# cerbos/cerbos

Measured on NVIDIA H100. Metric: checkresources_decisions_per_sec, higher is better.
Workload: dtype u64

## Files before the change

### cerbos_b200/csrc/cb_core.h

```cpp
#pragma once
#include <stdint.h>
#if !defined(__CUDACC_RTC__)
#include <math.h>
#endif

#include "cerbos_b200_format.h"

#if defined(__CUDACC__)
#define CB_HD __host__ __device__ __forceinline__
#define CB_HD_NOINLINE __host__ __device__ __noinline__
#else
#define CB_HD inline
#define CB_HD_NOINLINE
#endif

namespace cb {

struct alignas(16) U4 { uint32_t x, y, z, w; };

struct TableLayout {
    uint32_t off[32];
    uint32_t nV, nRP, nS, nP, nR, nAP, nT, n_slots, n_rows;
    uint32_t has_role_policies, has_parent_roles, has_principal_policies;
    uint32_t image_bytes;
    uint32_t uc_conds_off, uc_rows_off, uc_chain_off, n_uconds;
    uint32_t uc_n_rows;
    uint32_t uc_slots_off;
    uint32_t uc_deny_rows, uc_allow_rows;
    uint32_t theap_words;
    uint32_t uses_runtime;
};

struct TableView {
    const uint8_t *base;
    const TableLayout *L;
    template <typename T>
    CB_HD const T *sec(int id) const { return reinterpret_cast<const T *>(base + L->off[id]); }
    CB_HD const uint32_t *scope_parent() const { return sec<uint32_t>(CB_SEC_SCOPE_PARENT); }
    CB_HD const uint32_t *scope_flags() const { return sec<uint32_t>(CB_SEC_SCOPE_FLAGS); }
    CB_HD const uint32_t *res_block_map() const { return sec<uint32_t>(CB_SEC_RES_BLOCK_MAP); }
    CB_HD const uint8_t *res_exists() const { return sec<uint8_t>(CB_SEC_RES_EXISTS); }
    CB_HD const uint32_t *prin_block_map() const { return sec<uint32_t>(CB_SEC_PRIN_BLOCK_MAP); }
    CB_HD const uint8_t *prin_exists() const { return sec<uint8_t>(CB_SEC_PRIN_EXISTS); }
    CB_HD const uint32_t *prin_of_string() const { return sec<uint32_t>(CB_SEC_PRIN_OF_STRING); }
    CB_HD const cb_block *blocks() const { return sec<cb_block>(CB_SEC_BLOCKS); }
    CB_HD const cb_row *rows() const { return sec<cb_row>(CB_SEC_ROWS); }
    CB_HD const cb_cond *conds() const { return sec<cb_cond>(CB_SEC_CONDS); }
    CB_HD const cb_instr *code() const { return sec<cb_instr>(CB_SEC_CODE); }
    CB_HD const cb_const *consts() const { return sec<cb_const>(CB_SEC_CONSTS); }
    CB_HD const uint64_t *consts_v64() const { return sec<uint64_t>(CB_SEC_CONSTS_V64); }
    CB_HD const uint64_t *theap() const { return sec<uint64_t>(CB_SEC_THEAP); }
    CB_HD const uint32_t *str_off() const { return sec<uint32_t>(CB_SEC_STR_OFF); }
    CB_HD const uint8_t *str_bytes() const { return sec<uint8_t>(CB_SEC_STR_BYTES); }
    CB_HD const uint32_t *par_off() const { return sec<uint32_t>(CB_SEC_ROLE_PARENTS_OFF); }
    CB_HD const uint32_t *par_list() const { return sec<uint32_t>(CB_SEC_ROLE_PARENTS); }
    CB_HD const uint32_t *rp_off() const { return sec<uint32_t>(CB_SEC_ROLEPOL_OFF); }
    CB_HD const cb_rolepol_entry *rp_entries() const { return sec<cb_rolepol_entry>(CB_SEC_ROLEPOL_ENTRIES); }
    CB_HD const cb_rolepol_rule *rp_rules() const { return sec<cb_rolepol_rule>(CB_SEC_ROLEPOL_RULES); }
    CB_HD const uint32_t *rp_apats() const { return sec<uint32_t>(CB_SEC_ROLEPOL_APATS); }
    CB_HD const uint32_t *block_slots_off() const { return sec<uint32_t>(CB_SEC_BLOCK_SLOTS_OFF); }
    CB_HD const uint32_t *block_slots() const { return sec<uint32_t>(CB_SEC_BLOCK_SLOTS); }
    CB_HD const uint32_t *dr_off() const { return sec<uint32_t>(CB_SEC_DR_OFF); }
    CB_HD const uint32_t *dr_entries() const { return sec<uint32_t>(CB_SEC_DR_ENTRIES); }
    CB_HD const uint32_t *dr_parents() const { return sec<uint32_t>(CB_SEC_DR_PARENTS); }
    CB_HD const uint32_t *dr_name_str() const { return sec<uint32_t>(CB_SEC_DR_NAME_STR); }
    CB_HD const cb_cond *uconds() const { return reinterpret_cast<const cb_cond *>(base + L->uc_conds_off); }
    CB_HD const U4 *urows() const { return reinterpret_cast<const U4 *>(base + L->uc_rows_off); }
    CB_HD const uint32_t *uc_slots() const { return reinterpret_cast<const uint32_t *>(base + L->uc_slots_off); }
    CB_HD const U4 *uc_chain() const { return reinterpret_cast<const U4 *>(base + L->uc_chain_off); }
};

enum { CB_MAX_GATHER = 8 };
struct BatchView {
    const cb_hdr0 *hdr0;
    const cb_hdr1 *hdr1;
    const uint32_t *roles;
    const uint64_t *slots;
    const uint64_t *heap;
    const uint32_t *bstr_off;
    const uint8_t *bstr_bytes;
    const uint32_t *class_off, *class_pats, *aset_k;
    const uint64_t *aset_spread;
    const uint64_t *row_am;
    uint32_t n_rows;
    uint64_t stride;
    uint64_t first, count;
    uint32_t role_cols, n_asets, kc, n_pass, max_actions, kbytes, flags;
    uint32_t rcp, stride_pattern;
    int64_t now;
    const uint32_t *perm;
    uint32_t prefetch_slots;
    uint32_t *defer_list, *defer_count;
    uint32_t *count_dev;
    uint32_t *tile_counter;
    uint8_t *outs[CB_MAX_GATHER];
    uint32_t n_out;
    uint32_t *sig_flags[CB_MAX_GATHER];
    const uint32_t *wait_flags;
    uint32_t sig_rank, sig_step, wait_step;
    const uint32_t *strpred;
    const U4 *uc_rows_pk;
    uint32_t n_bstr;
    uint64_t heap_words;
};

#ifndef __CUDACC_RTC__
inline void finish_batch_view(BatchView &b) {
    b.perm = nullptr;
    b.prefetch_slots = 0;
    b.defer_list = nullptr; b.defer_count = nullptr; b.count_dev = nullptr; b.tile_counter = nullptr;
    b.n_out = 0;
    for (int i = 0; i < CB_MAX_GATHER; i++) { b.outs[i] = nullptr; b.sig_flags[i] = nullptr; }
    b.wait_flags = nullptr; b.sig_rank = 0; b.sig_step = 0; b.wait_step = 0;
    b.strpred = nullptr;
    b.uc_rows_pk = nullptr;
    b.rcp = 1;
    while (b.rcp < b.role_cols) b.rcp <<= 1;
    b.stride_pattern = 0;
    for (uint32_t j = 0; j * b.role_cols < 32; j++) b.stride_pattern |= 1u << (j * b.role_cols);
}
#endif

template <typename T>
CB_HD T ldg(const T *p) { return *p; }

CB_HD uint64_t ldcol64(const uint64_t *p) {
#if defined(__CUDA_ARCH__)
    uint64_t v;
    asm("ld.global.nc.L1::no_allocate.u64 %0, [%1];" : "=l"(v) : "l"(p));
    return v;
#else
    return *p;
#endif
}
CB_HD uint32_t ldcol32(const uint32_t *p) {
#if defined(__CUDA_ARCH__)
    uint32_t v;
    asm("ld.global.nc.L1::no_allocate.u32 %0, [%1];" : "=r"(v) : "l"(p));
    return v;
#else
    return *p;
#endif
}

CB_HD U4 ld16(const void *p) { return *reinterpret_cast<const U4 *>(p); }
CB_HD U4 ldcol128(const void *p) {
#if defined(__CUDA_ARCH__)
    U4 r;
    asm("ld.global.nc.L1::no_allocate.v4.u32 {%0, %1, %2, %3}, [%4];" : "=r"(r.x), "=r"(r.y), "=r"(r.z), "=r"(r.w) : "l"(p));
    return r;
#else
    return *reinterpret_cast<const U4 *>(p);
#endif
}
CB_HD cb_hdr0 load_hdr0(const cb_hdr0 *p) { U4 v = ldcol128(p); cb_hdr0 h; h.principal_id = v.x; h.kind_class = v.y; h.resource_scope = v.z; h.principal_scope = v.w; return h; }
CB_HD cb_hdr1 load_hdr1(const cb_hdr1 *p) {
    uint64_t v = ldcol64(reinterpret_cast<const uint64_t *>(p));
    cb_hdr1 h; h.resource_version = (uint16_t)(v & 0xFFFF); h.principal_version = (uint16_t)((v >> 16) & 0xFFFF); h.action_set_id = (uint32_t)(v >> 32); return h;
}
CB_HD cb_block load_block(const cb_block *p) { U4 v = ld16(p); cb_block b; b.row_start = v.x; b.n_rows = v.y; b.cond_base = v.z; b.n_conds = v.w; return b; }
CB_HD cb_row load_row(const cb_row *p) {
    U4 v = ld16(p);
    cb_row r; r.role = (uint16_t)(v.x & 0xFFFF); r.cond = (uint16_t)(v.x >> 16); r.drcond = (uint16_t)(v.y & 0xFFFF); r.respat = (uint16_t)(v.y >> 16);
    r.effect = (uint8_t)(v.z & 0xFF); r.flags = (uint8_t)((v.z >> 8) & 0xFF); r.n_pats = (uint16_t)(v.z >> 16); r.pat_start = v.w; return r;
}
CB_HD cb_rolepol_entry load_rp_entry(const cb_rolepol_entry *p) { U4 v = ld16(p); cb_rolepol_entry e; e.role = v.x; e.rule_start = v.y; e.n_rules = v.z; e.pad = v.w; return e; }
CB_HD cb_rolepol_rule load_rp_rule(const cb_rolepol_rule *p) { U4 v = ld16(p); cb_rolepol_rule e; e.respat = v.x; e.cond = v.y; e.apat_start = v.z; e.n_apats = v.w; return e; }

CB_HD double u2d(uint64_t u) {
#if defined(__CUDA_ARCH__)
    return __longlong_as_double((long long)u);
#else
    double d; __builtin_memcpy(&d, &u, 8); return d;
#endif
}
CB_HD uint64_t d2u(double d) {
#if defined(__CUDA_ARCH__)
    return (uint64_t)__double_as_longlong(d);
#else
    uint64_t u; __builtin_memcpy(&u, &d, 8); return u;
#endif
}

#if !defined(CB_LEAN_ONLY) || defined(CB_SPEC_PROGRAMS)
struct Val {
    uint32_t tag;
    uint64_t u;
};
static constexpr uint64_t kHeapBatch = 1ull << 63;
static constexpr uint64_t kHeapScratch = 1ull << 62;
static constexpr uint64_t kStrDyn = 1ull << 47;
static constexpr uint64_t kV64ScratchBit = 1ull << 46;
enum { CB_SCRATCH_WORDS = 192, CB_T_SKIP = 15 };

CB_HD Val mk(uint32_t tag, uint64_t u) { Val v; v.tag = tag; v.u = u; return v; }
CB_HD Val mk_err() { return mk(CB_T_ERR, 0); }
CB_HD Val mk_bool(bool b) { return mk(CB_T_BOOL, b ? 1u : 0u); }
CB_HD Val mk_int(int64_t i) { return mk(CB_T_INT, (uint64_t)i); }
CB_HD Val mk_double(double d) { return mk(CB_T_DOUBLE, d != d ? (uint64_t)CB_V64_CANON_NAN : d2u(d)); }

enum { SLOT_VALUE = 0, SLOT_ABSENT = 1, SLOT_ERROR = 2 };

CB_HD Val decode_v64(uint64_t bits, int *state) {
    const uint32_t top = (uint32_t)(bits >> 48);
    const bool boxed = (top & 0xFFF0u) == 0xFFF0u && (top & 0xFu) != 0;
    const uint32_t vt = top & 0xFu;
    const uint64_t pay = bits & 0xFFFFFFFFFFFFull;
    const uint64_t kTagOf = (uint64_t)CB_T_NULL << 4 | (uint64_t)CB_T_BOOL << 8 | (uint64_t)CB_T_STRING << 12 | (uint64_t)CB_T_LIST << 16 |
                            (uint64_t)CB_T_MAP << 20 | (uint64_t)CB_T_INT << 32;
    const uint32_t tag = boxed ? (uint32_t)(kTagOf >> (4 * vt)) & 0xFu : (uint32_t)CB_T_DOUBLE;
    uint64_t off = pay & (CB_V64_HEAP_BATCH_BIT - 1);
    off = (pay & CB_V64_HEAP_BATCH_BIT) ? off | kHeapBatch : (off & kV64ScratchBit) ? (off & ~kV64ScratchBit) | kHeapScratch : off;
    const uint64_t u = !boxed                                  ? bits
                       : vt == CB_V64_BOOL                     ? (uint64_t)(pay != 0)
                       : vt == CB_V64_STRING                   ? pay
                       : (vt == CB_V64_LIST || vt == CB_V64_MAP) ? off
                       : vt == CB_V64_INT                      ? (uint64_t)((int64_t)(pay << 16) >> 16)
                                                               : 0ull;
    *state = !boxed || tag != CB_T_ERR ? SLOT_VALUE : vt == CB_V64_ABSENT ? SLOT_ABSENT : SLOT_ERROR;
    return mk(tag, u);
}
CB_HD Val decode_elem(uint64_t bits) { int s; return decode_v64(bits, &s); }

struct Ctx {
    const TableView *t;
    const BatchView *b;
    uint64_t req;
    uint32_t pid;
    uint32_t unsupported;
    Val vars[CB_MAX_VARS];
    uint64_t edr;
    uint32_t scr_used;
    uint64_t scratch[CB_SCRATCH_WORDS];
};

CB_HD const uint64_t *heap_ptr(const Ctx &c, uint64_t ref) {
    return (ref & kHeapBatch) ? c.b->heap + (ref & ~kHeapBatch) : (ref & kHeapScratch) ? c.scratch + (ref & 0xFFFFu) : c.t->theap() + ref;
}
CB_HD void str_get(const Ctx &c, uint64_t id, const uint8_t *&p, uint32_t &len) {
    if (id & kStrDyn) {
        p = reinterpret_cast<const uint8_t *>(c.scratch) + ((id >> 16) & 0xFFFFu);
        len = (uint32_t)(id & 0xFFFFu);
    } else if (id < c.t->L->nT) {
        uint32_t o = ldg(c.t->str_off() + id);
        p = c.t->str_bytes() + o;
        len = ldg(c.t->str_off() + id + 1) - o;
    } else {
        uint64_t j = id - c.t->L->nT;
        uint32_t o = ldg(c.b->bstr_off + j);
        p = c.b->bstr_bytes + o;
        len = ldg(c.b->bstr_off + j + 1) - o;
    }
}

CB_HD bool is_num(const Val &v) { return v.tag == CB_T_INT || v.tag == CB_T_UINT || v.tag == CB_T_DOUBLE; }

CB_HD int num_cmp(const Val &a, const Val &b) {
    if (a.tag == CB_T_DOUBLE || b.tag == CB_T_DOUBLE) {
        if (a.tag == CB_T_DOUBLE && b.tag == CB_T_DOUBLE) {
            double x = u2d(a.u), y = u2d(b.u);
            if (x != x || y != y) return 2;
            return x < y ? -1 : (x > y ? 1 : 0);
        }
        int sign = 1;
        Val dv = a, iv = b;
        if (a.tag != CB_T_DOUBLE) { dv = b; iv = a; sign = -1; }
        double d = u2d(dv.u);
        if (d != d) return 2;
        int r;
        if (iv.tag == CB_T_UINT) {
            if (d < 0) r = -1;
            else if (d > 18446744073709551615.0) r = 1;
            else { double y = (double)iv.u; r = d < y ? -1 : (d > y ? 1 : 0); }
        } else {
            if (d < -9223372036854775808.0) r = -1;
            else if (d > 9223372036854775807.0) r = 1;
            else { double y = (double)(int64_t)iv.u; r = d < y ? -1 : (d > y ? 1 : 0); }
        }
        return r * sign;
    }
    if (a.tag == b.tag) {
        if (a.tag == CB_T_INT) { int64_t x = (int64_t)a.u, y = (int64_t)b.u; return x < y ? -1 : (x > y ? 1 : 0); }
        return a.u < b.u ? -1 : (a.u > b.u ? 1 : 0);
    }
    if (a.tag == CB_T_INT) {
        int64_t x = (int64_t)a.u;
        if (x < 0) return -1;
        return (uint64_t)x < b.u ? -1 : ((uint64_t)x > b.u ? 1 : 0);
    }
    int64_t y = (int64_t)b.u;
    if (y < 0) return 1;
    return a.u < (uint64_t)y ? -1 : (a.u > (uint64_t)y ? 1 : 0);
}

CB_HD bool str_equal(const Ctx &c, uint64_t a, uint64_t b) {
    if (a == b) return true;
    if (!((a | b) & kStrDyn)) return false;
    const uint8_t *pa, *pb;
    uint32_t la, lb;
    str_get(c, a, pa, la);
    str_get(c, b, pb, lb);
    if (la != lb) return false;
    for (uint32_t i = 0; i < la; i++)
        if (ldg(pa + i) != ldg(pb + i)) return false;
    return true;
}
CB_HD bool scalar_equal(const Ctx &c, const Val &a, const Val &b) {
    if (is_num(a) && is_num(b)) return num_cmp(a, b) == 0;
    if (a.tag != b.tag) return false;
    if (a.tag == CB_T_NULL) return true;
    if (a.tag == CB_T_STRING || a.tag == CB_T_BYTES) return str_equal(c, a.u, b.u);
    return a.u == b.u;
}
CB_HD bool is_container(const Val &v) { return v.tag == CB_T_LIST || v.tag == CB_T_MAP; }

CB_HD bool map_find(const Ctx &c, const Val &m, const Val &key, Val *out) {
    if (is_container(key) || key.tag == CB_T_ERR) return false;
    const uint64_t *p = heap_ptr(c, m.u);
    uint64_t n = ldg(p);
    for (uint64_t i = 0; i < n; i++) {
        Val k = decode_elem(ldg(p + 1 + i));
        if (scalar_equal(c, k, key)) {
            if (out) *out = decode_elem(ldg(p + 1 + n + i));
            return true;
        }
    }
    return false;
}

template <int DEPTH>
struct Eq {
    static CB_HD bool eq(Ctx &c, const Val &a, const Val &b) {
        if (!is_container(a) || !is_container(b)) {
            if (is_container(a) != is_container(b)) return false;
            return scalar_equal(c, a, b);
        }
        if (a.tag != b.tag) return false;
        const uint64_t *pa = heap_ptr(c, a.u), *pb = heap_ptr(c, b.u);
        uint64_t n = ldg(pa);
        if (n != ldg(pb)) return false;
        if (a.tag == CB_T_LIST) {
            for (uint64_t i = 0; i < n; i++)
                if (!Eq<DEPTH - 1>::eq(c, decode_elem(ldg(pa + 1 + i)), decode_elem(ldg(pb + 1 + i)))) return false;
            return true;
        }
        for (uint64_t i = 0; i < n; i++) {
            Val ov;
            if (!map_find(c, b, decode_elem(ldg(pa + 1 + i)), &ov)) return false;
            if (!Eq<DEPTH - 1>::eq(c, decode_elem(ldg(pa + 1 + n + i)), ov)) return false;
        }
        return true;
    }
};
template <>
struct Eq<0> {
    static CB_HD bool eq(Ctx &c, const Val &a, const Val &b) {
        if (is_container(a) && is_container(b)) { c.unsupported = 1; return false; }
        if (is_container(a) != is_container(b)) return false;
        return scalar_equal(c, a, b);
    }
};
CB_HD_NOINLINE bool container_equal(Ctx &c, const Val &a, const Val &b) { return Eq<3>::eq(c, a, b); }
CB_HD bool val_equal(Ctx &c, const Val &a, const Val &b) {
    if (!is_container(a) || !is_container(b)) { if (is_container(a) != is_container(b)) return false; return scalar_equal(c, a, b); }
    return container_equal(c, a, b);
}

CB_HD int str_cmp(const Ctx &c, uint64_t ia, uint64_t ib) {
    const uint8_t *pa, *pb;
    uint32_t la, lb;
    str_get(c, ia, pa, la);
    str_get(c, ib, pb, lb);
    uint32_t m = la < lb ? la : lb;
    for (uint32_t i = 0; i < m; i++) {
        uint8_t x = ldg(pa + i), y = ldg(pb + i);
        if (x != y) return x < y ? -1 : 1;
    }
    return la < lb ? -1 : (la > lb ? 1 : 0);
}

CB_HD int val_order(const Ctx &c, const Val &a, const Val &b) {
    if (is_num(a) && is_num(b)) { int r = num_cmp(a, b); return r == 2 ? 3 : r; }
    if (a.tag != b.tag) return 3;
    switch (a.tag) {
    case CB_T_BOOL: return a.u < b.u ? -1 : (a.u > b.u ? 1 : 0);
    case CB_T_STRING: return a.u == b.u ? 0 : str_cmp(c, a.u, b.u);
    case CB_T_TS:
    case CB_T_DUR: { int64_t x = (int64_t)a.u, y = (int64_t)b.u; return x < y ? -1 : (x > y ? 1 : 0); }
    default: return 3;
    }
}

CB_HD_NOINLINE int spiffe_equal(Ctx &c, const Val &a, const Val &b);
CB_HD Val do_cmp(Ctx &c, int ci, const Val &a, const Val &b) {
    if (a.tag == CB_T_ERR || b.tag == CB_T_ERR) return mk_err();
    if (ci <= 1 && (a.tag == CB_T_SPIFFE_ID || a.tag == CB_T_SPIFFE_TD)) {
        const int r = spiffe_equal(c, a, b);
        return r == 2 ? mk_err() : mk_bool((r == 1) == (ci == 0));
    }
    if (ci == 0) return mk_bool(val_equal(c, a, b));
    if (ci == 1) return mk_bool(!val_equal(c, a, b));
    int r = val_order(c, a, b);
    if (r == 3) return mk_err();
    switch (ci) {
    case 2: return mk_bool(r < 0);
    case 3: return mk_bool(r <= 0);
    case 4: return mk_bool(r > 0);
    default: return mk_bool(r >= 0);
    }
}

CB_HD Val do_in(Ctx &c, const Val &x, const Val &cont) {
    if (x.tag == CB_T_ERR || cont.tag == CB_T_ERR) return mk_err();
    if (cont.tag == CB_T_LIST) {
        const uint64_t *p = heap_ptr(c, cont.u);
        uint64_t n = ldg(p);
// ... 2906 lines not shown
        uint32_t k = 0;
        for (uint32_t i = 0; i < s.len; i++) k += (ldg(s.p + i) & 0xC0) != 0x80;
        return d2u((double)k);
    }
    return (uint64_t)(CB_V64_BOX_BASE | CB_V64_ERROR) << 48;
}
template <typename Cols>
CB_HD uint64_t term_operand(const TableView t, const BatchView &b, const Cols &cols, uint32_t pid, uint32_t kind, uint32_t v, uint32_t aux) {
    if (kind == CB_OPK_CONST) return ldg(t.consts_v64() + v);
    if (kind == CB_OPK_PID) return ((uint64_t)(CB_V64_BOX_BASE | CB_V64_STRING) << 48) | pid;
    uint64_t x = cols.slot(v);
    if (kind == CB_OPK_SLOT) return x;
    return kind == CB_OPK_SLOT_ELEM ? elem_operand(t, b, x, aux) : size_operand(t, b, x);
}
CB_HD bool v64_bad(uint64_t x) { return ((uint32_t)(x >> 48) & 0xFFFEu) == (CB_V64_BOX_BASE | CB_V64_ABSENT); }
CB_HD int eq_tri(uint64_t x, uint64_t y, bool &slow) {
    const uint32_t tx = v64_tag(x), ty = v64_tag(y);
    if (v64_bad(x) || v64_bad(y)) return TRI_E;
    if (tx == 0 && ty == 0) return u2d(x) == u2d(y);
    if (tx <= CB_V64_STRING && ty <= CB_V64_STRING) return x == y;
    slow = true;
    return TRI_E;
}
CB_HD int ord_tri(uint32_t ci, uint64_t x, uint64_t y, bool &slow) {
    const uint32_t tx = v64_tag(x), ty = v64_tag(y);
    if (v64_bad(x) || v64_bad(y)) return TRI_E;
    if (tx == 0 && ty == 0) {
        const double dx = u2d(x), dy = u2d(y);
        if (dx != dx || dy != dy) return TRI_E;
        return ci == 2 ? dx < dy : ci == 3 ? dx <= dy : ci == 4 ? dx > dy : dx >= dy;
    }
    if (tx != ty) return TRI_E;
    slow = true;
    return TRI_E;
}
CB_HD int in_tri(const TableView t, const BatchView &b, uint64_t x, uint64_t y, bool elems_scalar, bool &slow) {
    if (v64_bad(x) || v64_bad(y)) return TRI_E;
    if (v64_tag(y) != CB_V64_LIST || v64_tag(x) > CB_V64_STRING) { slow = true; return TRI_E; }
    const uint64_t *p = list_ptr(t, b, y);
    const uint32_t ln = (uint32_t)ldg(p);
    bool found = false;
    for (uint32_t j = 0; j < ln; j++) {
        const uint64_t e = ldg(p + 1 + j);
        if (!elems_scalar) slow |= v64_tag(e) > CB_V64_STRING;
        found |= scalar_eq64(x, e);
    }
    return found;
}
template <typename... E>
CB_HD int in_const_tri(uint64_t x, bool &slow, E... elems) {
    if (v64_bad(x)) return TRI_E;
    if (v64_tag(x) > CB_V64_STRING) { slow = true; return TRI_E; }
    bool found = false;
    ((found |= scalar_eq64(x, (uint64_t)elems)), ...);
    return found ? TRI_T : TRI_F;
}
CB_HD int has_tri(uint64_t x) {
    const uint32_t tx = v64_tag(x);
    return tx == CB_V64_ERROR ? TRI_E : (tx != CB_V64_ABSENT);
}
CB_HD int cmp_tri(uint32_t ci, uint64_t x, uint64_t y, bool &slow) {
    const uint32_t tx = v64_tag(x), ty = v64_tag(y);
    if (v64_bad(x) || v64_bad(y)) return TRI_E;
    if (tx == 0 && ty == 0) {
        const double dx = u2d(x), dy = u2d(y);
        if (ci == 0) return dx == dy;
        if (dx != dx || dy != dy) return TRI_E;
        return ci == 2 ? dx < dy : ci == 3 ? dx <= dy : ci == 4 ? dx > dy : dx >= dy;
    }
    if (ci == 0 && tx <= CB_V64_STRING && ty <= CB_V64_STRING) return x == y;
    if (ci != 0 && tx != ty) return TRI_E;
    slow = true;
    return TRI_E;
}
CB_HD int str_tri(const TableView t, const BatchView &b, uint32_t op, uint64_t x, uint64_t y) {
    if (v64_tag(x) != CB_V64_STRING || v64_tag(y) != CB_V64_STRING) return TRI_E;
    const StrRef a = str_ref(t, b, x), c = str_ref(t, b, y);
    if (c.len > a.len) return TRI_F;
    if (op == CB_TERM_CONTAINS) {
        bool hit = false;
        for (uint32_t o = 0; o + c.len <= a.len; o++) {
            bool eq = true;
            for (uint32_t j = 0; j < c.len; j++) eq &= ldg(a.p + o + j) == ldg(c.p + j);
            hit |= eq;
        }
        return hit;
    }
    const uint8_t *ap = op == CB_TERM_STARTS ? a.p : a.p + (a.len - c.len);
    bool eq = true;
    for (uint32_t j = 0; j < c.len; j++) eq &= ldg(ap + j) == ldg(c.p + j);
    return eq;
}
template <typename Cols>
CB_HD int term_tri(const TableView t, const BatchView &b, const Cols &cols, uint32_t pid, const U4 w, bool &slow) {
    const uint32_t op = w.x & 0xFF, flags = (w.x >> 8) & 0xFF, xk = (w.x >> 16) & 0xFF, yk = w.x >> 24;
    int tri = TRI_E;
    switch (w.x & 0xFF) {
    case CB_TERM_EQ_SS: tri = eq_tri(cols.slot(w.y), cols.slot(w.z), slow); break;
    case CB_TERM_EQ_SC: tri = eq_tri(cols.slot(w.y), ldg(t.consts_v64() + w.z), slow); break;
    case CB_TERM_EQ_SP: tri = eq_tri(cols.slot(w.y), ((uint64_t)(CB_V64_BOX_BASE | CB_V64_STRING) << 48) | pid, slow); break;
    case CB_TERM_ORD_SS: tri = ord_tri(flags & CB_TERM_CI_MASK, cols.slot(w.y), cols.slot(w.z), slow); break;
    case CB_TERM_ORD_SC: tri = ord_tri(flags & CB_TERM_CI_MASK, cols.slot(w.y), ldg(t.consts_v64() + w.z), slow); break;
    case CB_TERM_IN_SC: tri = in_tri(t, b, cols.slot(w.y), ldg(t.consts_v64() + w.z), true, slow); break;
    case CB_TERM_IN_CS: tri = in_tri(t, b, ldg(t.consts_v64() + w.y), cols.slot(w.z), false, slow); break;
    case CB_TERM_IN_SS: tri = in_tri(t, b, cols.slot(w.y), cols.slot(w.z), false, slow); break;
    default: {
        const uint64_t x = term_operand(t, b, cols, pid, xk, w.y, w.w & 0xFFFF);
        const uint64_t y = op == CB_TERM_HAS ? 0 : term_operand(t, b, cols, pid, yk, w.z, w.w >> 16);
        const uint32_t tx = v64_tag(x), ty = v64_tag(y);
        if (op == CB_TERM_HAS) {
            tri = has_tri(x);
        } else if (op == CB_TERM_CMP) {
            tri = cmp_tri(flags & CB_TERM_CI_MASK, x, y, slow);
        } else if (v64_bad(x) || v64_bad(y)) {
            tri = TRI_E;
        } else if (op == CB_TERM_IN) {
            if (ty != CB_V64_LIST || tx > CB_V64_STRING) slow = true;
            else {
                const uint64_t *p = list_ptr(t, b, y);
                const uint32_t ln = (uint32_t)ldg(p);
                bool found = false;
                for (uint32_t j = 0; j < ln; j++) {
                    const uint64_t e = ldg(p + 1 + j);
                    slow |= v64_tag(e) > CB_V64_STRING;
                    found |= scalar_eq64(x, e);
                }
                tri = found;
            }
        } else if (op == CB_TERM_STARTS || op == CB_TERM_ENDS || op == CB_TERM_CONTAINS) {
            tri = str_tri(t, b, op, x, y);
        } else {
            if (tx != CB_V64_LIST || ty != CB_V64_LIST) tri = TRI_E;
            else {
                const uint64_t *pa = list_ptr(t, b, x), *pb = list_ptr(t, b, y);
                const uint32_t na = (uint32_t)ldg(pa), nb = (uint32_t)ldg(pb);
                bool any_hit = false, all_hit = true;
                for (uint32_t i2 = 0; i2 < na; i2++) {
                    const uint64_t ea = ldg(pa + 1 + i2);
                    slow |= v64_tag(ea) > CB_V64_STRING;
                    bool hit = false;
                    for (uint32_t j = 0; j < nb; j++) {
                        const uint64_t eb = ldg(pb + 1 + j);
                        slow |= v64_tag(eb) > CB_V64_STRING;
                        hit |= scalar_eq64(ea, eb);
                    }
                    any_hit |= hit;
                    all_hit &= hit;
                }
                tri = op == CB_TERM_INTERSECTS ? any_hit : all_hit;
            }
        }
    }
    }
    return tri;
}
template <typename Cols>
CB_HD int uc_term_tri(const TableView t, const BatchView &b, const Cols &cols, uint32_t pid, const U4 w, bool &slow) {
#ifdef CB_UC_STUB_TERMS
    return (int)(cols.slot(w.y) & 1u);
#endif
    return term_tri(t, b, cols, pid, w, slow);
}
template <typename Cols>
CB_HD uint64_t uc_term_operand(const TableView t, const BatchView &b, const Cols &cols, uint32_t pid, uint32_t kind, uint32_t v, uint32_t aux) {
#ifdef CB_UC_STUB_TERMS
    return ((uint64_t)(CB_V64_BOX_BASE | CB_V64_STRING) << 48) | (uint32_t)cols.slot(v);
#endif
    return term_operand(t, b, cols, pid, kind, v, aux);
}
enum { CB_LC = 8 };
CB_HD uint32_t list_bound(uint32_t own) {
#if defined(__CUDA_ARCH__)
    return __reduce_max_sync(__activemask(), own);
#else
    return own;
#endif
}
#ifndef CB_LIST_KEYS64
struct ListRegs {
    uint32_t st, len;
    uint32_t bound;
    uint32_t e[CB_LC];
};
static constexpr uint32_t kListPad = 0xFFFFFFFEu;
static constexpr uint32_t kListNoKey = 0xFFFFFFFFu;
static constexpr uint32_t kStringTop = CB_V64_BOX_BASE | CB_V64_STRING;
CB_HD uint32_t list_key(uint64_t w) { return (uint32_t)w; }
CB_HD bool list_elem_odd(uint64_t w) { return (uint32_t)(w >> 48) != kStringTop; }
static constexpr uint64_t kListBeyondHeap = 0ull;
#else
struct ListRegs {
    uint32_t st, len;
    uint32_t bound;
    uint64_t e[CB_LC];
};
static constexpr uint64_t kListPad = 0xFFFE000000000001ull;
CB_HD uint64_t norm_scalar(uint64_t v) { return v == 0x8000000000000000ull ? 0ull : v; }
CB_HD uint64_t list_key(uint64_t w) { return norm_scalar(w); }
CB_HD bool list_elem_odd(uint64_t w) { return v64_tag(w) > CB_V64_STRING || w == CB_V64_CANON_NAN; }
static constexpr uint64_t kListBeyondHeap = kListPad;
#endif
CB_HD ListRegs list_load(const TableView t, const BatchView &b, uint64_t x) {
    ListRegs L;
    L.st = v64_bad(x) ? 1u : v64_tag(x) == CB_V64_LIST ? 0u : 3u;
    L.len = 0;
#ifdef CB_UC_STUB_LISTS
    L.len = (uint32_t)x & 7u;
    L.bound = CB_LC;
    for (int j = 0; j < CB_LC; j++) L.e[j] = (uint32_t)x + j;
    return L;
#endif
    const uint64_t *p = nullptr;
    uint64_t room = 0;
    if (L.st == 0) {
        const uint64_t pay = x & 0xFFFFFFFFFFFFull;
        const bool in_batch = (pay & CB_V64_HEAP_BATCH_BIT) != 0;
        const uint64_t off = in_batch ? pay & (CB_V64_HEAP_BATCH_BIT - 1) : pay;
        p = (in_batch ? b.heap : t.theap()) + off;
        room = (in_batch ? b.heap_words : (uint64_t)t.L->theap_words) - off;
        L.len = (uint32_t)ldg(p);
    }
    L.bound = list_bound(L.len < CB_LC ? L.len : CB_LC);
    const uint32_t lim = room > (uint64_t)L.bound ? L.bound : room != 0 ? (uint32_t)room - 1u : 0u;
    bool odd = L.len > CB_LC;
#if defined(__CUDA_ARCH__)
#pragma unroll
#endif
    for (int j = 0; j < CB_LC; j++) {
        const uint64_t w = (uint32_t)j < lim ? ldg(p + 1 + j) : kListBeyondHeap;
        const bool in = (uint32_t)j < L.len;
        odd |= in && list_elem_odd(w);
        L.e[j] = in ? list_key(w) : kListPad;
    }
    if (L.st == 0) L.st = odd ? 2u : 0u;
    return L;
}
CB_HD uint64_t list_size(const TableView t, const BatchView &b, uint64_t x, const ListRegs &L) {
    if (L.st == 0 || L.st == 2) return d2u((double)L.len);
    return size_operand(t, b, x);
}
CB_HD uint64_t list_elem(const TableView t, const BatchView &b, uint64_t x, const ListRegs &L, uint32_t i) {
    if (L.st == 2) return elem_operand(t, b, x, i);
    if (L.st != 0 || i >= L.len) return (uint64_t)(CB_V64_BOX_BASE | CB_V64_ERROR) << 48;
#ifndef CB_LIST_KEYS64
    return ((uint64_t)kStringTop << 48) | L.e[i];
#else
    return L.e[i];
#endif
}
#ifndef CB_LIST_KEYS64
typedef uint32_t ListKey;
CB_HD ListKey list_probe_key(uint64_t x) { return (uint32_t)(x >> 48) == kStringTop ? (uint32_t)x : kListNoKey; }
#else
typedef uint64_t ListKey;
CB_HD ListKey list_probe_key(uint64_t x) { return norm_scalar(x); }
#endif
template <int P>
CB_HD uint32_t list_probe(const ListRegs &L, const ListKey (&k)[P]) {
    static_assert(P >= 1 && P <= 32, "one bit per key");
#if defined(CB_UC_STUB_LISTS) || defined(CB_UC_STUB_LIST_PROBES)
    return ((uint32_t)(L.e[0] ^ k[0]) ^ L.len) & (uint32_t)((1ull << P) - 1u);
#endif
    uint32_t h = 0;
#if defined(__CUDA_ARCH__)
#pragma unroll
#endif
    for (int p = 0; p < P; p++) {
        bool hit = false;
#if defined(__CUDA_ARCH__)
#pragma unroll
#endif
        for (int j = 0; j < CB_LC; j++) hit |= k[p] == L.e[j];
        h |= (uint32_t)hit << p;
    }
    return h;
}
CB_HD int list_in_tri(uint64_t x, uint32_t st, uint32_t hit, bool &slow) {
#ifdef CB_UC_STUB_LISTS
    return hit ? TRI_T : TRI_F;
#endif
    if (v64_bad(x) || st == 1) return TRI_E;
    if (st != 0 || v64_tag(x) > CB_V64_STRING || x == CB_V64_CANON_NAN) { slow = true; return TRI_E; }
    return hit ? TRI_T : TRI_F;
}
CB_HD int list_in_tri(uint64_t x, const ListRegs &L, bool &slow) {
#ifdef CB_UC_STUB_LISTS
    return (uint32_t)x == L.e[0] ? TRI_T : TRI_F;
#endif
    const ListKey k[1] = {list_probe_key(x)};
    return list_in_tri(x, L.st, list_probe(L, k), slow);
}
CB_HD uint32_t list_mask(const ListRegs &A, const ListRegs &B) {
    return list_probe(B, A.e) & (A.len < CB_LC ? (1u << A.len) - 1u : (1u << CB_LC) - 1u);
}
CB_HD int list_set_tri(bool subset, const ListRegs &A, const ListRegs &B, uint32_t m, bool &slow) {
#ifdef CB_UC_STUB_LISTS
    return (A.e[0] == B.e[subset] + m) ? TRI_T : TRI_F;
#endif
    if (A.st == 1 || B.st == 1) return TRI_E;
    if (A.st == 3 || B.st == 3) return TRI_E;
    if (A.st == 2 || B.st == 2) { slow = true; return TRI_E; }
    return (subset ? m == (1u << A.len) - 1u : m != 0u) ? TRI_T : TRI_F;
}
CB_HD int strpred_tri(const BatchView &b, uint64_t x, uint32_t p) {
#ifdef CB_UC_STUB_STRPRED
    return (int)((x >> p) & 1u);
#endif
    if (v64_bad(x)) return TRI_E;
    if (v64_tag(x) != CB_V64_STRING) return TRI_E;
    return (int)((ldg(b.strpred + (uint32_t)(x & 0xFFFFFFFFu)) >> p) & 1u);
}
CB_HD bool typed_str(uint64_t x) { return (uint32_t)(x >> 32) == (uint32_t)(CB_V64_BOX_BASE | CB_V64_STRING) << 16; }
CB_HD bool typed_num(uint64_t x) { const double d = u2d(x); return v64_tag(x) == 0 && d == d; }
CB_HD bool typed_bool(uint64_t x) { return (x >> 1) == (uint64_t)(CB_V64_BOX_BASE | CB_V64_BOOL) << 47; }
CB_HD bool typed_list(const ListRegs &L, uint32_t need) {
    bool ok = L.st == 0 && L.len >= need;
#ifdef CB_LIST_KEYS64
    for (int j = 0; j < CB_LC; j++) ok &= (uint32_t)j >= L.len || (uint32_t)(L.e[j] >> 48) == (CB_V64_BOX_BASE | CB_V64_STRING);
#endif
    return ok;
}
CB_HD bool uc_typed(bool guard) {
#ifdef CB_UC_STUB_FALLBACK
    return guard || true;
#endif
    return guard;
}
CB_HD uint32_t typed_id(uint64_t key) { return (uint32_t)key; }
CB_HD uint64_t typed_box(uint32_t id) { return ((uint64_t)(CB_V64_BOX_BASE | CB_V64_STRING) << 48) | id; }
CB_HD bool typed_ord(uint32_t ci, double dx, double dy) { return ci == 2 ? dx < dy : ci == 3 ? dx <= dy : ci == 4 ? dx > dy : dx >= dy; }
CB_HD bool typed_strpred(const BatchView &b, uint32_t id, uint32_t p) {
#ifdef CB_UC_STUB_STRPRED
    return ((id >> p) & 1u) != 0;
#endif
    return ((ldg(b.strpred + id) >> p) & 1u) != 0;
}
template <typename Cols>
CB_HD ListKey list_elem_key(const TableView t, const BatchView &b, const Cols &cols, uint32_t v, const ListRegs &L, uint32_t i) {
    if (L.st == 2) return list_probe_key(elem_operand(t, b, cols.slot(v), i));
    return list_probe_key(list_elem(t, b, 0ull, L, i));
}

struct OneCols {
    uint64_t x;
    CB_HD uint64_t slot(uint32_t) const { return x; }
};
CB_HD bool term_lit(int tri, uint32_t flags) { return (flags & CB_TERM_LIT_F) ? tri == TRI_F : tri == TRI_T; }
template <typename Cols>
CB_HD uint32_t flat_dnf_inline(const TableView t, const BatchView &b, const Cols &cols, uint32_t pid, uint32_t flat_off, uint32_t info) {
    const uint32_t nt = info & 0xFFFF;
    const cb_instr *terms = t.code() + flat_off;
    bool any = false, group = true, slow = false;
    for (uint32_t i = 0; i < nt; i++) {
        const U4 w = ld16(terms + 2 * i);
        const uint32_t flags = (w.x >> 8) & 0xFF;
        group &= term_lit(term_tri(t, b, cols, pid, w, slow), flags);
        if (flags & CB_TERM_GROUP_END) { any |= group; group = true; }
    }
    if (slow) return 4u;
    return (uint32_t)(any != (bool)((info >> 24) & 1));
}
template <typename Cols>
CB_HD uint32_t cond_eval(const TableView t, const BatchView &b, const Cols &cols, uint32_t pid, uint32_t gid) {
    U4 cd = ld16(t.conds() + gid);
    if (cd.w) return flat_dnf_inline(t, b, cols, pid, cd.z, cd.w);
    return 4u;
}

CB_HD uint32_t chain_start(const TableView t, uint32_t scope, uint32_t kind_flag, bool lenient) {
    if (scope == CB_SCOPE_NONE) return CB_NONE32;
    uint32_t s = scope & ~CB_SCOPE_INEXACT_BIT;
    if (s >= t.L->nS) return CB_NONE32;
    if (!(ldg(t.scope_flags() + s) & kind_flag)) {
        if (!lenient) return CB_NONE32;
        do { s = ldg(t.scope_parent() + s); } while (s != CB_NONE32 && !(ldg(t.scope_flags() + s) & kind_flag));
    }
    return s;
}
CB_HD uint32_t chain_next(const TableView t, uint32_t s, uint32_t kind_flag) {
    do { s = ldg(t.scope_parent() + s); } while (s != CB_NONE32 && !(ldg(t.scope_flags() + s) & kind_flag));
    return s;
}

CB_HD void prefetch_l1(const void *p) {
#if defined(__CUDA_ARCH__)
    asm volatile("prefetch.global.L1 [%0];" ::"l"(p));
#else
    (void)p;
#endif
}

CB_HD void prefetch_request(const BatchView &b, uint64_t n) {
    prefetch_l1(b.hdr0 + n);
    prefetch_l1(b.hdr1 + n);
    const uint32_t *pr = b.roles + n;
    for (uint32_t i = 0; i < b.role_cols; i++, pr += b.stride) prefetch_l1(pr);
    const uint64_t *ps = b.slots + n;
    for (uint32_t q = 0; q < b.prefetch_slots; q++, ps += b.stride) prefetch_l1(ps);
}

#ifndef CB_LEAN_ONLY
CB_HD uint32_t kind_count(const BatchView &b, uint32_t kc) {
    if (kc == CB_KIND_NONE) return 0;
    if (!(kc & CB_KIND_CLASS_CSR_BIT)) return 1;
    uint32_t c = kc & ~CB_KIND_CLASS_CSR_BIT;
    return ldg(b.class_off + c + 1) - ldg(b.class_off + c);
}
CB_HD uint32_t kind_pat_at(const BatchView &b, uint32_t kc, uint32_t j) {
    if (!(kc & CB_KIND_CLASS_CSR_BIT)) return kc;
    return ldg(b.class_pats + ldg(b.class_off + (kc & ~CB_KIND_CLASS_CSR_BIT)) + j);
}
CB_HD bool kind_has(const BatchView &b, uint32_t kc, uint32_t pat) {
    if (!(kc & CB_KIND_CLASS_CSR_BIT)) return kc == pat;
    for (uint32_t j = 0, n = kind_count(b, kc); j < n; j++)
        if (kind_pat_at(b, kc, j) == pat) return true;
    return false;
}

template <typename M>
CB_HD_NOINLINE M role_cols_slow(const uint8_t *base, const TableLayout *L, const BatchView *b, uint64_t n, uint32_t n_roles, uint32_t rscope, uint32_t role) {
    TableView t; t.base = base; t.L = L;
    M m = 0;
    for (uint32_t i = 0; i < n_roles; i++) m |= (M)role_in_pr(t, role, ldcol32(b->roles + (uint64_t)i * b->stride + n), rscope) << i;
    return m;
}
struct U2x64 { uint64_t a, b; };
CB_HD_NOINLINE U2x64 role_tab_parents(const uint8_t *base, const TableLayout *L, const BatchView *b, uint64_t n, uint32_t n_roles, uint32_t rscope, uint32_t RCP,
                                     uint64_t rp0, uint64_t rp1) {
    TableView t; t.base = base; t.L = L;
    for (uint32_t i = 0; i < n_roles; i++) {
        uint32_t r = ldcol32(b->roles + (uint64_t)i * b->stride + n);
        if (r >= t.L->nR) continue;
        uint64_t idx = (uint64_t)rscope * t.L->nR + r;
        for (uint32_t j = ldg(t.par_off() + idx), e = ldg(t.par_off() + idx + 1); j < e; j++) {
            uint32_t pq = ldg(t.par_list() + j) * RCP + i;
            if (pq < 64) rp0 |= 1ull << pq; else if (pq < 128) rp1 |= 1ull << (pq - 64);
        }
    }
    U2x64 r; r.a = rp0; r.b = rp1; return r;
}

#endif
CB_HD uint32_t row_role(const U4 &r) { return r.x & 0xFFFF; }
CB_HD uint32_t row_cond(const U4 &r) { return r.x >> 16; }
CB_HD uint32_t row_drcond(const U4 &r) { return r.y & 0xFFFF; }
CB_HD uint32_t row_respat(const U4 &r) { return r.y >> 16; }
CB_HD uint32_t row_effect(const U4 &r) { return r.z & 0xFF; }
#ifndef CB_LEAN_ONLY

CB_HD_NOINLINE bool exists_check(const uint8_t *base, const TableLayout *L, const BatchView *b, uint32_t kc, uint32_t pscope, uint32_t r0,
                                 uint32_t pv, uint32_t rv, bool lenient) {
    TableView t; t.base = base; t.L = L;
    bool p_exists = false, r_exists = false;
    if (pv != CB_NONE16)
        for (uint32_t s = chain_start(t, pscope, CB_SCOPE_FLAG_PRINCIPAL, lenient); s != CB_NONE32; s = chain_next(t, s, CB_SCOPE_FLAG_PRINCIPAL))
            p_exists |= ldg(t.prin_exists() + (uint64_t)pv * t.L->nS + s) != 0;
    for (uint32_t s = r0; s != CB_NONE32; s = chain_next(t, s, CB_SCOPE_FLAG_RESOURCE))
        for (uint32_t j = 0, nk = kind_count(*b, kc); j < nk; j++)
            r_exists |= (ldg(t.res_exists() + ((uint64_t)rv * t.L->nRP + kind_pat_at(*b, kc, j)) * t.L->nS + s) & CB_EXISTS_RESOURCE_KIND) != 0;
    return p_exists || r_exists;
}

CB_HD void prefetch_block_slots(const TableView t, const BatchView &b, uint32_t bid, uint64_t n) {
    for (uint32_t q = ldg(t.block_slots_off() + bid), e = ldg(t.block_slots_off() + bid + 1); q < e; q++)
        prefetch_l1(b.slots + (uint64_t)ldg(t.block_slots() + q) * b.stride + n);
}

CB_HD_NOINLINE uint64_t compute_edr(const uint8_t *base, const TableLayout *L, const BatchView *b, uint64_t n, uint32_t pid, uint32_t bid, uint32_t n_roles,
                                    uint32_t rscope, uint32_t *unsupported) {
    TableView t; t.base = base; t.L = L;
    uint64_t mask = 0;
    for (uint32_t e = ldg(t.dr_off() + bid), ee = ldg(t.dr_off() + bid + 1); e < ee; e++) {
        const U4 en = ld16(t.dr_entries() + 4 * (uint64_t)e);
        bool hit = false;
        for (uint32_t q = 0; q < en.w && !hit; q++) {
            const uint32_t pr = ldg(t.dr_parents() + en.z + q);
            if (pr == CB_ROLE_ANY) { hit = true; break; }
            for (uint32_t i = 0; i < n_roles && !hit; i++) hit = role_in_pr(t, pr, ldcol32(b->roles + (uint64_t)i * b->stride + n), rscope);
        }
        if (!hit) continue;
        bool sat = true;
        if (en.y) { const uint32_t r = cond_sat(base, L, b, n, pid, en.y - 1); *unsupported |= r & 2; sat = r & 1; }
        if (sat) mask |= 1ull << (en.x & 63);
    }
    return mask;
}

template <typename M>
struct PairMasks { M deny, allow; uint32_t unsupported; };

template <typename M>
CB_HD_NOINLINE PairMasks<M> principal_walk(const uint8_t *base, const TableLayout *L, const BatchView *b, uint64_t n, uint32_t pid, uint32_t kc, uint32_t pidx,
                                           uint32_t p0, uint32_t rv, M amask, const uint64_t *row_am) {
    TableView t; t.base = base; t.L = L;
    PairMasks<M> out; out.deny = 0; out.allow = 0; out.unsupported = 0;
    M alive = amask;
    for (uint32_t s = p0; s != CB_NONE32 && alive; s = chain_next(t, s, CB_SCOPE_FLAG_PRINCIPAL)) {
        uint32_t bid = ldg(t.prin_block_map() + ((uint64_t)rv * t.L->nP + pidx) * t.L->nS + s);
        if (bid == CB_NONE32) continue;
        U4 bl = ld16(t.blocks() + bid);
        M D = 0, A = 0;
        for (uint32_t ri = bl.x, re = bl.x + bl.y; ri < re; ri++) {
            M m = (M)ldg(reinterpret_cast<const M *>(row_am + ri)) & alive;
            if (!m) continue;
            U4 row = ld16(t.rows() + ri);
            if (!kind_has(*b, kc, row_respat(row))) continue;
            if (row_effect(row) == CB_EFFECT_DENY ? (m & ~D) == 0 : (m & ~A) == 0) continue;
            bool sat = true;
            if (row_drcond(row)) { uint32_t r = cond_sat(t.base, t.L, b, n, pid, bl.z + row_drcond(row) - 1); out.unsupported |= r & 2; sat = r & 1; }
            if (sat && row_cond(row)) { uint32_t r = cond_sat(t.base, t.L, b, n, pid, bl.z + row_cond(row) - 1); out.unsupported |= r & 2; sat = r & 1; }
            if (!sat) continue;
            if (row_effect(row) == CB_EFFECT_DENY) D |= m; else A |= m;
        }
        out.deny |= D;
        alive &= ~D;
        uint32_t perm = (ldg(t.scope_flags() + s) >> CB_SCOPE_PERM_SHIFT) & 3;
        if (perm == 1) { M a = A & alive; out.allow |= a; alive &= ~a; }
    }
    return out;
}

template <typename M>
CB_HD_NOINLINE PairMasks<M> rolepol_denies(const uint8_t *base, const TableLayout *L, const BatchView *b, uint64_t n, uint32_t pid, uint32_t kc, uint32_t n_roles,
                                           uint32_t rscope, uint32_t RCP, uint64_t rp0, uint64_t rp1, bool packed, uint32_t rv, uint32_t s,
                                           uint32_t ps, uint32_t aset, M amask, M alive, M D) {
    TableView t; t.base = base; t.L = L;
    PairMasks<M> out; out.allow = 0; out.unsupported = 0;
    const M role_all = (M)(((M)1 << n_roles) - 1);
    const uint32_t nAP = t.L->nAP ? t.L->nAP : 1;
    const uint64_t *spread = b->aset_spread + ((uint64_t)ps * b->n_asets + aset) * nAP;
    uint64_t ro = (uint64_t)rv * t.L->nS + s;
    for (uint32_t e = ldg(t.rp_off() + ro), ee = ldg(t.rp_off() + ro + 1); e < ee; e++) {
        U4 en = ld16(t.rp_entries() + e);
        M rmask;
        if (packed) { uint32_t pos = en.x * RCP; rmask = (M)(pos < 64 ? rp0 >> pos : rp1 >> (pos - 64)) & role_all; }
        else rmask = role_cols_slow<M>(t.base, t.L, b, n, n_roles, rscope, en.x);
        if (!rmask) continue;
        M matched = 0;
        for (uint32_t q = 0; q < en.z; q++) {
            U4 ru = ld16(t.rp_rules() + en.y + q);
            if (!kind_has(*b, kc, ru.x)) continue;
            M am = 0;
            for (uint32_t a = 0; a < ru.w; a++) am |= (M)ldg(spread + ldg(t.rp_apats() + ru.z + a));
            if (!am) continue;
            matched |= am;
            if (ru.y && ((am * rmask) & alive & ~D)) {
                uint32_t r = cond_sat(t.base, t.L, b, n, pid, ru.y - 1);
                out.unsupported |= r & 2;
                if (!(r & 1)) D |= (am * rmask) & alive;
            }
        }
        D |= ((amask & ~matched) * rmask) & alive;
    }
    out.deny = D;
    return out;
}

template <typename M>
CB_HD void eval_request(const TableView t, const BatchView &b, uint64_t n, uint8_t *bitmap, uint8_t *effects, uint32_t *status) {
    constexpr M kOne = 1;
    const U4 h0 = ldcol128(b.hdr0 + n);
    const uint64_t h1 = ldcol64(reinterpret_cast<const uint64_t *>(b.hdr1 + n));
    const uint32_t pid = h0.x, kc = h0.y, rscope = h0.z, pscope = h0.w;
    const uint32_t rv = (uint32_t)(h1 & 0xFFFF), pv = (uint32_t)((h1 >> 16) & 0xFFFF), aset = (uint32_t)(h1 >> 32);
    const uint32_t RC = b.role_cols;
    const uint32_t K = aset < b.n_asets ? ldg(b.aset_k + aset) : 0;
    uint32_t unsupported = 0;

    uint32_t RCP = 1;
    while (RCP < RC) RCP <<= 1;
    const bool packed = (uint64_t)t.L->nR * RCP <= 128;
    uint64_t rp0 = 0, rp1 = 0;
    uint32_t n_roles = 0;
    for (uint32_t i = 0; i < RC; i++) {
        uint32_t rr = ldcol32(b.roles + (uint64_t)i * b.stride + n);
        if (rr != CB_ROLE_PAD) n_roles = i + 1;
        if (rr < t.L->nR) {
            uint32_t pos = rr * RCP + i;
            if (pos < 64) rp0 |= 1ull << pos; else if (pos < 128) rp1 |= 1ull << (pos - 64);
        }
    }

    uint64_t acc = 0;
    const bool wide = b.kbytes > 8;
    uint8_t *out = effects ? nullptr : bitmap + n * b.kbytes;
    uint8_t *eff = effects ? effects + n * (uint64_t)b.max_actions : nullptr;
    if (wide) {
        if (eff) for (uint32_t q = 0; q < b.max_actions; q++) eff[q] = (uint8_t)(q < K ? CB_EFFECT_DENY : 0);
        else for (uint32_t q = 0; q < b.kbytes; q++) out[q] = 0;
    }

    const bool lenient = (b.flags & CB_BATCH_FLAG_LENIENT) != 0;
    uint32_t p0 = CB_NONE32, r0 = CB_NONE32;
    bool live = n_roles != 0 && K != 0 && rv != CB_NONE16;
    if (live) {
        if (t.L->has_principal_policies) p0 = chain_start(t, pscope, CB_SCOPE_FLAG_PRINCIPAL, lenient);
        r0 = chain_start(t, rscope, CB_SCOPE_FLAG_RESOURCE, lenient);
        if (pv != rv && !exists_check(t.base, t.L, &b, kc, pscope, r0, pv, rv, lenient)) live = false;
        if (p0 == CB_NONE32 && r0 == CB_NONE32) live = false;
    }

    if (live) {
        const uint32_t pidx = (t.L->has_principal_policies && pid < t.L->nT) ? ldg(t.prin_of_string() + pid) : CB_NONE32;
        const M role_all = (M)((kOne << n_roles) - 1);
        if (t.L->has_parent_roles && packed && rscope != CB_SCOPE_NONE && !(rscope & CB_SCOPE_INEXACT_BIT) && rscope < t.L->nS) {
            U2x64 r = role_tab_parents(t.base, t.L, &b, n, n_roles, rscope, RCP, rp0, rp1);
            rp0 = r.a; rp1 = r.b;
        }
        const uint32_t nk = kind_count(b, kc);

        for (uint32_t ps = 0; ps < b.n_pass; ps++) {
            const uint32_t kbase = ps * b.kc;
            if (kbase >= K) break;
            const uint32_t kn = K - kbase < b.kc ? K - kbase : b.kc;
            const uint64_t *row_am = b.row_am + ((uint64_t)ps * b.n_asets + aset) * b.n_rows;
            M amask = 0;
            for (uint32_t kk = 0; kk < kn; kk++) amask |= kOne << (kk * RC);

            M p_allow = 0, p_deny = 0;
            if (pidx != CB_NONE32 && p0 != CB_NONE32) {
                PairMasks<M> pm = principal_walk<M>(t.base, t.L, &b, n, pid, kc, pidx, p0, rv, amask, row_am);
                p_allow = pm.allow; p_deny = pm.deny; unsupported |= pm.unsupported;
            }

            const M undecided = amask & ~(p_allow | p_deny);
            M r_allow_pairs = 0;
            if (undecided && r0 != CB_NONE32) {
                M alive = undecided * role_all;
                for (uint32_t s = r0; s != CB_NONE32 && alive; s = chain_next(t, s, CB_SCOPE_FLAG_RESOURCE)) {
                    M D = 0, A = 0;
                    bool any_row = false;
                    for (uint32_t j = 0; j < nk; j++) {
                        uint64_t mi = ((uint64_t)rv * t.L->nRP + kind_pat_at(b, kc, j)) * t.L->nS + s;
                        if (t.L->has_role_policies) any_row |= (ldg(t.res_exists() + mi) & CB_EXISTS_ANY_ROW) != 0;
                        uint32_t bid = ldg(t.res_block_map() + mi);
                        if (bid == CB_NONE32) continue;
                        prefetch_block_slots(t, b, bid, n);
                        const U4 bl = ld16(t.blocks() + bid);
// ... 691 lines not shown
```

### cerbos_b200/csrc/cb_specialize.h

```cpp
#pragma once
#include <stdint.h>

#include <cstdio>
#include <cstring>
#include <map>
#include <string>
#include <vector>

#include "cerbos_b200_format.h"

namespace cbspec {

struct Limits {
    uint32_t max_shapes = 8;
    uint32_t max_items = 96;
};

inline std::string hex(uint32_t v) {
    char buf[16];
    snprintf(buf, sizeof buf, "0x%xu", v);
    return buf;
}
inline std::string hex64(uint64_t v) {
    char buf[32];
// ... 76 lines not shown
        const uint32_t bid = shape_blocks[sh][0];
        const uint32_t *bl = blocks + 4 * bid;
        s += "template <typename Cols>\nCB_HD void spec_shape_" + std::to_string(sh) + "(" + args_decl + ") {\n";
        if (bs_off[bid + 1] > bs_off[bid]) {
            s += "    if (!cols.staged()) {";
            for (uint32_t q = bs_off[bid]; q < bs_off[bid + 1]; q++) s += " cols.prefetch_slot(" + std::to_string(bs[q]) + "u);";
            s += " }\n";
        }
        s += "    bool slow = false;\n    uint32_t val = 1u;\n";
        for (uint32_t c = 0; c < bl[3]; c++) {
            const uint32_t *cd = conds + 4 * (bl[2] + c);
            const uint32_t nt = cd[3] & 0xFFFFu, negate = (cd[3] >> 24) & 1u;
            s += "    {   // condition " + std::to_string(c + 1) + "\n        bool any = false, group = true;\n";
            for (uint32_t i = 0; i < nt; i++) {
                const uint32_t *w = code + 2 * (cd[2] + 2 * i);
                const uint32_t flags = (w[0] >> 8) & 0xFFu;
                s += "        group &= term_lit(" + term_expr(w, consts, theap) + ", " + hex(flags) + ");\n";
                if (flags & CB_TERM_GROUP_END) s += "        any |= group; group = true;\n";
            }
            s += std::string("        val |= (uint32_t)(any != ") + (negate ? "true" : "false") + ") << " + std::to_string(c + 1) + ";\n    }\n";
        }
        s += "    defer |= slow;\n";
        for (uint32_t r = 0; r < bl[1]; r++) {
            const uint32_t *row = rows + 4 * (bl[0] + r);
            s += "    row_apply(ldg(reinterpret_cast<const uint32_t *>(ram + " + std::to_string(r) + ")), U4{" + hex(row[0]) + ", " + hex(row[1] & 0xFFFFu) + ", " +
                 hex(row[2] & 0xFFu) + ", 0u}, rp, RCP, role_all, alive, val, D, A);\n";
        }
        s += "}\n";
    }
    s += "struct SpecBlocks {\n    template <typename Cols>\n    CB_HD void operator()(const TableView t, const BatchView &b, const Cols &cols, uint32_t pid, uint32_t bid, "
         "uint64_t rp, uint32_t RCP, uint32_t role_all, uint32_t alive, const uint64_t *row_am, uint32_t &D, uint32_t &A, bool &defer) const {\n";
    s += "        const uint64_t *ram = row_am + ldg(reinterpret_cast<const uint32_t *>(t.blocks() + bid));   // + row_start\n";
    s += "        switch (bid) {\n";
    for (uint32_t sh = 0; sh < shape_blocks.size(); sh++) {
        s += "       ";
        for (uint32_t bid : shape_blocks[sh]) s += " case " + std::to_string(bid) + ":";
        s += "\n            spec_shape_" + std::to_string(sh) + "(t, b, cols, pid, rp, RCP, role_all, alive, ram, D, A, defer);\n            break;\n";
    }
    s += "        default: defer = true; break;\n        }\n    }\n};\n}  // namespace cb\n";
    return s;
}

struct Ins { uint32_t op, ia, ib, ic; };
struct Atoms {
    std::map<std::vector<uint32_t>, uint32_t> ids;
    std::vector<std::string> src;
    std::vector<bool> slot_used;
    std::vector<uint32_t> only_slot;
    std::vector<bool> reads_pid;
};

inline bool is_jump(uint32_t op) {
    return op == CB_OP_JF_KEEP || op == CB_OP_JT_KEEP || op == CB_OP_JMP || op == CB_OP_TERN || op == CB_OP_LOOP_INIT || op == CB_OP_LOOP_NEXT || op == CB_OP_LOOP_PRED;
}

inline std::string atom_source(const std::vector<Ins> &P, uint32_t lo, uint32_t hi, const uint32_t *consts , uint32_t n_consts, uint32_t n_slots,
                               std::vector<bool> &slot_used, uint32_t *only_slot = nullptr, bool *reads_pid = nullptr) {
    std::vector<uint32_t> my_slots;
    bool my_pid = false;
    const uint32_t n = hi - lo;
    const int kUnset = -1000;
    std::vector<int> depth(n + 1, kUnset), ldep(n + 1, kUnset);
    std::vector<bool> target(n + 1, false);
    bool bad = false;
    auto set = [&](uint32_t k, int d, int l) {
        if (k > n) { bad = true; return; }
        if (depth[k] == kUnset) { depth[k] = d; ldep[k] = l; }
        else if (depth[k] != d || ldep[k] != l) bad = true;
    };
    auto rel = [&](uint32_t abs) -> uint32_t { if (abs < lo || abs > hi) { bad = true; return 0; } return abs - lo; };
    set(0, 0, 0);
    for (uint32_t k = 0; k < n && !bad; k++) {
        if (depth[k] == kUnset) { bad = true; break; }
        const Ins &I = P[lo + k];
        const int d = depth[k], l = ldep[k];
        int nd = d;
        bool falls = true;
        switch (I.op) {
        case CB_OP_CONST: case CB_OP_SLOT: case CB_OP_HAS_SLOT: case CB_OP_PID: case CB_OP_NOW: case CB_OP_VAR:
        case CB_OP_CMP_SLOT_CONST: case CB_OP_CMP_SLOT_SLOT: case CB_OP_CMP_SLOT_PID: case CB_OP_IN_SLOT_CONST: case CB_OP_IN_CONST_SLOT:
            nd = d + 1; break;
        case CB_OP_SELECT: case CB_OP_HAS: case CB_OP_NEG: case CB_OP_NOT: case CB_OP_SIZE: case CB_OP_NOERR: case CB_OP_INT: case CB_OP_UINT:
        case CB_OP_DOUBLE: case CB_OP_TIMESTAMP: case CB_OP_DURATION: case CB_OP_DYN: case CB_OP_IN_IP_RANGE: case CB_OP_HIER_SIZE: case CB_OP_TS_GET:
        case CB_OP_MATCHES:
            if (d < 1) bad = true;
            break;
        case CB_OP_INDEX: case CB_OP_EQ: case CB_OP_NE: case CB_OP_LT: case CB_OP_LE: case CB_OP_GT: case CB_OP_GE:
        case CB_OP_ADD: case CB_OP_SUB: case CB_OP_MUL: case CB_OP_DIV: case CB_OP_MOD: case CB_OP_IN:
        case CB_OP_STARTS_WITH: case CB_OP_ENDS_WITH: case CB_OP_CONTAINS: case CB_OP_AND: case CB_OP_OR:
        case CB_OP_HAS_INTERSECTION: case CB_OP_IS_SUBSET: case CB_OP_HIER_REL: case CB_OP_IN_SPLIT:
            if (d < 2) bad = true;
            nd = d - 1; break;
        case CB_OP_HIER_CA: nd = d - (I.ia == 0 ? 1 : 2); if (nd < 1) bad = true; break;
        case CB_OP_FN:
            if (I.ib < 1 || I.ib > (I.ia == CB_FN_FORMAT ? (uint32_t)CB_MAX_STACK : 4u) || d < (int)I.ib) bad = true;
            nd = d - ((int)I.ib - 1); break;
        case CB_OP_JF_KEEP: case CB_OP_JT_KEEP: if (d < 1) bad = true; set(rel(I.ic), d, l); target[rel(I.ic)] = true; break;
        case CB_OP_JMP: set(rel(I.ic), d, l); target[rel(I.ic)] = true; falls = false; break;
        case CB_OP_TERN:
            if (d < 1) bad = true;
            nd = d - 1;
            set(rel(I.ic), d - 1, l); target[rel(I.ic)] = true;
            set(rel(I.ib), d, l); target[rel(I.ib)] = true;
            break;
        case CB_OP_LOOP_INIT:
            if (d < 1 || (I.ib & 0xFF) >= CB_LOOP_MAP || l >= CB_MAX_LOOP_DEPTH) bad = true;
            set(rel(I.ic), d, l); target[rel(I.ic)] = true;
            set(k + 1, d - 1, l + 1);
            falls = false;
            break;
        case CB_OP_LOOP_NEXT:
            if (d < 1 || (I.ib & 0xFF) >= CB_LOOP_MAP || l < 1) bad = true;
            set(rel(I.ic), d - 1, l); target[rel(I.ic)] = true;
            set(k + 1, d, l - 1);
            falls = false;
            break;
        default: bad = true; break;
        }
        if (nd > CB_MAX_STACK) bad = true;
        if (falls && !bad) set(k + 1, nd, l);
    }
    if (bad || depth[n] != 1 || ldep[n] != 0) return "";
    auto S = [](int i) { return "s" + std::to_string(i); };
    auto lab = [](uint32_t k) { return "P" + std::to_string(k); };
    auto cst = [&](uint32_t k) -> std::string {
        if (k >= n_consts) { bad = true; return "mk_err()"; }
        const uint32_t *w = consts + 4 * k;
        return "mk(" + hex(w[0]) + ", " + hex64((uint64_t)w[2] | (uint64_t)w[3] << 32) + ")";
    };
    auto slot = [&](uint32_t v) -> std::string {
        if (v >= n_slots) { bad = true; return "0ull"; }
        slot_used[v] = true;
        bool seen = false;
        for (uint32_t q : my_slots) seen |= q == v;
        if (!seen) my_slots.push_back(v);
        return "cols.slot(" + std::to_string(v) + "u)";
    };
    int maxd = 1;
    for (uint32_t k = 0; k <= n; k++) if (depth[k] > maxd) maxd = depth[k];
    std::string s = "    Val";
    for (int i = 0; i < maxd; i++) s += std::string(i ? ", " : " ") + S(i);
    s += ";\n    Loop L0, L1; int st_; (void)st_; (void)L0; (void)L1;\n";
    for (uint32_t k = 0; k < n; k++) {
        const Ins &I = P[lo + k];
        const int d = depth[k], l = ldep[k];
        if (target[k]) s += lab(k) + ":;\n";
        const std::string a = S(d - 1), a2 = S(d - 2), top = S(d);
        s += "    ";
        switch (I.op) {
        case CB_OP_CONST: s += top + " = " + cst(I.ic) + ";"; break;
        case CB_OP_SLOT: s += top + " = decode_v64(" + slot(I.ic) + ", &st_);"; break;
        case CB_OP_HAS_SLOT: s += "decode_v64(" + slot(I.ic) + ", &st_); " + top + " = op_has_slot(st_);"; break;
        case CB_OP_PID: my_pid = true; s += top + " = mk(CB_T_STRING, c.pid);"; break;
        case CB_OP_NOW: s += top + " = mk(CB_T_TS, (uint64_t)c.b->now);"; break;
        case CB_OP_VAR: if (I.ia >= CB_MAX_VARS) bad = true; s += top + " = c.vars[" + std::to_string(I.ia) + "];"; break;
        case CB_OP_SELECT: s += a + " = op_select(c, " + a + ", " + hex(I.ic) + ");"; break;
        case CB_OP_HAS: s += a + " = op_has(c, " + a + ", " + hex(I.ic) + ");"; break;
        case CB_OP_INDEX: s += a2 + " = do_index(c, " + a2 + ", " + a + ");"; break;
        case CB_OP_EQ: case CB_OP_NE: case CB_OP_LT: case CB_OP_LE: case CB_OP_GT: case CB_OP_GE:
            s += a2 + " = do_cmp(c, " + std::to_string(I.op - CB_OP_EQ) + ", " + a2 + ", " + a + ");"; break;
        case CB_OP_ADD: case CB_OP_SUB: case CB_OP_MUL: case CB_OP_DIV: case CB_OP_MOD:
            s += a2 + " = do_arith(c, " + std::to_string(I.op) + ", " + a2 + ", " + a + ");"; break;
        case CB_OP_NEG: s += a + " = op_neg(" + a + ");"; break;
        case CB_OP_NOT: s += a + " = op_not(" + a + ");"; break;
        case CB_OP_IN: s += a2 + " = do_in(c, " + a2 + ", " + a + ");"; break;
        case CB_OP_SIZE: s += a + " = op_size(c, " + a + ");"; break;
        case CB_OP_STARTS_WITH: case CB_OP_ENDS_WITH: case CB_OP_CONTAINS:
            s += a2 + " = do_str2(c, " + std::to_string(I.op) + ", " + a2 + ", " + a + ");"; break;
        case CB_OP_JF_KEEP: s += "if (" + a + ".tag == CB_T_BOOL && " + a + ".u == 0) goto " + lab(I.ic - lo) + ";"; break;
        case CB_OP_JT_KEEP: s += "if (" + a + ".tag == CB_T_BOOL && " + a + ".u == 1) goto " + lab(I.ic - lo) + ";"; break;
        case CB_OP_AND: s += a2 + " = and_or(false, " + a2 + ", " + a + ");"; break;
        case CB_OP_OR: s += a2 + " = and_or(true, " + a2 + ", " + a + ");"; break;
        case CB_OP_JMP: s += "goto " + lab(I.ic - lo) + ";"; break;
        case CB_OP_TERN:
            s += "if (" + a + ".tag == CB_T_BOOL) { if (!" + a + ".u) goto " + lab(I.ic - lo) + "; } else { " + a + " = mk_err(); goto " + lab(I.ib - lo) + "; }";
            break;
        case CB_OP_HAS_INTERSECTION: s += a2 + " = do_set_pred(c, false, " + a2 + ", " + a + ");"; break;
        case CB_OP_IS_SUBSET: s += a2 + " = do_set_pred(c, true, " + a2 + ", " + a + ");"; break;
        case CB_OP_LOOP_INIT:
            s += "{ const Val r_ = " + a + "; if (!qloop_init(c, L" + std::to_string(l) + ", r_, " + std::to_string(I.ib & 0xFF) + ", " + (((I.ib >> 8) & 1) ? "true" : "false") +
                 ", " + std::to_string(I.ia) + ", &" + a + ")) goto " + lab(I.ic - lo) + "; }";
            break;
        case CB_OP_LOOP_NEXT:
            s += "{ const Val r_ = " + a + "; if (!qloop_next(c, L" + std::to_string(l - 1) + ", r_, " + std::to_string(I.ib & 0xFF) + ", " + (((I.ib >> 8) & 1) ? "true" : "false") +
                 ", " + std::to_string(I.ia) + ", &" + a + ")) goto " + lab(I.ic - lo) + "; }";
            break;
        case CB_OP_NOERR: s += a + " = mk_bool(" + a + ".tag != CB_T_ERR);"; break;
        case CB_OP_INT: s += a + " = conv_int(c, " + a + ");"; break;
        case CB_OP_UINT: s += a + " = conv_uint(c, " + a + ");"; break;
        case CB_OP_DOUBLE: s += a + " = op_double(c, " + a + ");"; break;
        case CB_OP_TIMESTAMP: s += a + " = op_timestamp(c, " + a + ");"; break;
        case CB_OP_DURATION: s += a + " = op_duration(c, " + a + ");"; break;
        case CB_OP_DYN: s += ";"; break;
        case CB_OP_CMP_SLOT_CONST: s += top + " = do_cmp(c, " + std::to_string(I.ia) + ", decode_v64(" + slot(I.ib) + ", &st_), " + cst(I.ic) + ");"; break;
        case CB_OP_CMP_SLOT_SLOT: s += "{ const Val x_ = decode_v64(" + slot(I.ib) + ", &st_); " + top + " = do_cmp(c, " + std::to_string(I.ia) + ", x_, decode_v64(" + slot(I.ic) + ", &st_)); }"; break;
        case CB_OP_CMP_SLOT_PID: my_pid = true; s += top + " = do_cmp(c, " + std::to_string(I.ia) + ", decode_v64(" + slot(I.ib) + ", &st_), mk(CB_T_STRING, c.pid));"; break;
        case CB_OP_IN_SLOT_CONST: s += top + " = do_in(c, decode_v64(" + slot(I.ib) + ", &st_), " + cst(I.ic) + ");"; break;
        case CB_OP_IN_CONST_SLOT: s += top + " = do_in(c, " + cst(I.ic) + ", decode_v64(" + slot(I.ib) + ", &st_));"; break;
        case CB_OP_IN_IP_RANGE: s += a + " = " + a + ".tag == CB_T_ERR ? mk_err() : do_in_ip_range(c, " + a + ", c.t->theap() + " + hex(I.ic) + ");"; break;
        case CB_OP_HIER_REL: s += a2 + " = op_hier_rel(c, " + hex(I.ia) + ", " + hex(I.ib) + ", " + hex(I.ic) + ", " + a2 + ", " + a + ");"; break;
        case CB_OP_TS_GET: s += a + " = op_ts_get(c, " + a + ", " + hex(I.ia) + ", " + hex(I.ib) + ", " + hex(I.ic) + ");"; break;
        case CB_OP_IN_SPLIT: s += a2 + " = op_in_split(c, " + a2 + ", " + a + ", " + hex(I.ib) + ");"; break;
        case CB_OP_HIER_SIZE: s += a + " = op_hier_size(c, " + a + ", " + hex(I.ib) + ");"; break;
        case CB_OP_HIER_CA:
            if (I.ia == 0) s += a2 + " = op_hier_ca2(c, " + a2 + ", " + a + ", " + hex(I.ib) + ", " + hex(I.ic) + ");";
            else s += S(d - 3) + " = op_hier_ca3(c, " + S(d - 3) + ", " + a2 + ", " + a + ", " + hex(I.ib) + ", " + hex(I.ic) + ");";
            break;
        case CB_OP_FN: {
            const int base = d - (int)I.ib;
            s += "{ Val a_[" + std::to_string(I.ib) + "] = {";
            for (uint32_t q = 0; q < I.ib; q++) s += std::string(q ? ", " : "") + S(base + (int)q);
            s += "}; " + S(base) + " = op_fn(c, " + hex(I.ia) + ", " + hex(I.ib) + ", a_); }";
            break;
        }
        case CB_OP_MATCHES: s += a + " = op_matches(c, " + a + ", " + hex(I.ic) + ");"; break;
        default: bad = true; break;
        }
        s += "\n";
    }
    if (target[n]) s += lab(n) + ":;\n";
    s += "    return cond_true(s0);\n";
    if (only_slot) *only_slot = my_slots.size() == 1 ? my_slots[0] : CB_NONE32;
    if (reads_pid) *reads_pid = my_pid;
    return bad ? std::string() : s;
}

inline std::string translate_program(const uint32_t *code_words, uint32_t code_off, uint32_t code_len, const uint32_t *consts, uint32_t n_consts, uint32_t n_slots, Atoms &at) {
    if (code_len == 0 || code_len > 4096) return "";
    std::vector<Ins> P(code_len);
    for (uint32_t i = 0; i < code_len; i++) {
        const uint32_t w0 = code_words[2 * (code_off + i)], w1 = code_words[2 * (code_off + i) + 1];
        P[i] = Ins{w0 & 0xFFu, (w0 >> 8) & 0xFFu, w0 >> 16, w1};
    }
    std::vector<std::string> st;
    uint32_t i = 0;
    bool ret = false;
    while (i < code_len && !ret) {
        const Ins &I = P[i];
        auto cond_level = [&](uint32_t op) { return op == CB_OP_AND || op == CB_OP_OR || op == CB_OP_COND_NOT || op == CB_OP_RET; };
        switch (I.op) {
        case CB_OP_RET: ret = true; continue;
        case CB_OP_AND: case CB_OP_OR: {
            if (st.size() < 2) return "";
            const std::string b = st.back(); st.pop_back();
            st.back() = "(" + st.back() + (I.op == CB_OP_AND ? " & " : " | ") + b + ")";
            i++;
            continue;
        }
        case CB_OP_COND_NOT: if (st.empty()) return ""; st.back() = "!" + st.back(); i++; continue;
        case CB_OP_JF_KEEP: case CB_OP_JT_KEEP:
            if (st.empty() || I.ic <= i || I.ic > code_len) return "";
            i++;
            continue;
        default: break;
        }
        uint32_t e = i;
        while (e < code_len && P[e].op != CB_OP_TO_COND) e++;
        bool literal = false;
        if (I.op == CB_OP_CONST && i + 1 < code_len) {
            const uint32_t nx = P[i + 1].op;
            if (cond_level(nx)) literal = true;
            if ((nx == CB_OP_JF_KEEP || nx == CB_OP_JT_KEEP) && (e >= code_len || P[i + 1].ic > e)) literal = true;
        }
        if (literal) {
            if (I.ic >= n_consts || consts[4 * I.ic] != CB_T_BOOL) return "";
            st.push_back(consts[4 * I.ic + 2] ? "true" : "false");
            i++;
            continue;
        }
        if (e >= code_len) return "";
        std::vector<uint32_t> key;
        for (uint32_t k = i; k < e; k++) {
            const Ins &J = P[k];
            const bool j = is_jump(J.op);
            key.push_back(J.op | J.ia << 8 | (J.op == CB_OP_TERN ? (J.ib - i) : J.ib) << 16);
            key.push_back(j ? J.ic - i : J.ic);
        }
        auto it = at.ids.find(key);
        if (it == at.ids.end()) {
            if (at.slot_used.size() < n_slots) at.slot_used.resize(n_slots, false);
            uint32_t one = CB_NONE32;
            bool pid = false;
            const std::string body = atom_source(P, i, e, consts, n_consts, n_slots, at.slot_used, &one, &pid);
            if (body.empty()) return "";
            const uint32_t id = (uint32_t)at.src.size();
            at.only_slot.push_back(one);
            at.reads_pid.push_back(pid);
            at.src.push_back("template <typename Cols>\nCB_HD bool uc_atom_" + std::to_string(id) + "(Ctx &c, const Cols &cols) {\n" + body + "}\n");
            it = at.ids.emplace(key, id).first;
        }
        st.push_back("a" + std::to_string(it->second));
        i = e + 1;
    }
    if (!ret || st.size() != 1) return "";
    return st[0];
}

struct UcLimits {
    uint32_t max_terms = 512;
};
struct UcSource {
    std::string src;
    uint32_t n_strpred = 0;
    uint32_t n_atoms = 0;
};
inline UcSource generate_uc(const uint8_t *uc_image, const uint32_t *off, uint32_t uc_conds_off, uint32_t n_uconds, uint32_t n_slots, uint32_t n_consts = 0,
                            const UcLimits lim = UcLimits()) {
    UcSource out;
    if (n_uconds == 0 || n_uconds > 127) return out;
    const uint32_t *const_words = reinterpret_cast<const uint32_t *>(uc_image + off[CB_SEC_CONSTS]);
    Atoms atoms;
    std::vector<std::string> formula(n_uconds + 1);
    const uint32_t *uconds = reinterpret_cast<const uint32_t *>(uc_image + uc_conds_off);
    const uint32_t scope_rows = uconds[0], deny_rows = uconds[1], allow_rows = uconds[2];
    const uint32_t *code = reinterpret_cast<const uint32_t *>(uc_image + off[CB_SEC_CODE]);
    const uint64_t *consts = reinterpret_cast<const uint64_t *>(uc_image + off[CB_SEC_CONSTS_V64]);
    const uint64_t *theap = reinterpret_cast<const uint64_t *>(uc_image + off[CB_SEC_THEAP]);
    const uint32_t kUseMask = ~((uint32_t)(CB_TERM_LIT_F | CB_TERM_GROUP_END) << 8);
    std::map<std::vector<uint32_t>, uint32_t> term_ids;
    std::vector<std::vector<uint32_t>> terms;
    const uint32_t ns = n_slots ? n_slots : 1;
    std::vector<bool> slot_used(ns, false), slot_list(ns, false);
    auto is_slot_kind = [](uint32_t kind) { return kind == CB_OPK_SLOT || kind == CB_OPK_SLOT_ELEM || kind == CB_OPK_SLOT_SIZE; };
    auto use_slot = [&](uint32_t kind, uint32_t v) { if (is_slot_kind(kind) && v < ns) slot_used[v] = true; };
    auto v64_tag = [](uint64_t b) { const uint32_t top = (uint32_t)(b >> 48); return (top & 0xFFF0u) == 0xFFF0u ? (top & 0xFu) : 0u; };
    for (uint32_t u = 1; u <= n_uconds; u++) {
        const uint32_t *cd = uconds + 4 * u;
        if (cd[3] == 0 || ((cd[3] >> 16) & 0xFF) != CB_FLAT_DNF) {
            formula[u] = translate_program(code, cd[0], cd[1], const_words, n_consts, ns, atoms);
            if (formula[u].empty()) return out;
            continue;
        }
        for (uint32_t i = 0, nt = cd[3] & 0xFFFFu; i < nt; i++) {
            const uint32_t *w = code + 2 * (cd[2] + 2 * i);
            std::vector<uint32_t> key = {w[0] & kUseMask, w[1], w[2], w[3]};
            if (term_ids.emplace(key, (uint32_t)terms.size()).second) terms.push_back(key);
        }
    }
    if (terms.size() > lim.max_terms) return out;
    std::vector<char> form(terms.size(), 'G');
    std::vector<uint32_t> pred_of(terms.size(), 0);
    std::vector<uint32_t> pred_terms;
    for (uint32_t q = 0; q < terms.size(); q++) {
        const uint32_t *w = terms[q].data();
        const uint32_t op = w[0] & 0xFF, xk = (w[0] >> 16) & 0xFF, yk = w[0] >> 24;
        switch (op) {
        case CB_TERM_EQ_SS: case CB_TERM_ORD_SS: use_slot(CB_OPK_SLOT, w[1]); use_slot(CB_OPK_SLOT, w[2]); break;
        case CB_TERM_EQ_SC: case CB_TERM_EQ_SP: case CB_TERM_ORD_SC: case CB_TERM_IN_SC: use_slot(CB_OPK_SLOT, w[1]); break;
        case CB_TERM_IN_SS: use_slot(CB_OPK_SLOT, w[1]); use_slot(CB_OPK_SLOT, w[2]); if (w[2] < ns) { slot_list[w[2]] = true; form[q] = 'L'; } break;
        case CB_TERM_IN_CS: use_slot(CB_OPK_SLOT, w[2]); if (w[2] < ns) { slot_list[w[2]] = true; form[q] = 'L'; } break;
        default:
            use_slot(xk, w[1]);
            if (op != CB_TERM_HAS) use_slot(yk, w[2]);
            if (xk == CB_OPK_SLOT_SIZE && w[1] < ns) slot_list[w[1]] = true;
            if (op != CB_TERM_HAS && yk == CB_OPK_SLOT_SIZE && w[2] < ns) slot_list[w[2]] = true;
            if (op == CB_TERM_IN && yk == CB_OPK_SLOT && w[2] < ns) { slot_list[w[2]] = true; form[q] = 'L'; }
            if ((op == CB_TERM_INTERSECTS || op == CB_TERM_SUBSET) && xk == CB_OPK_SLOT && yk == CB_OPK_SLOT && w[1] < ns && w[2] < ns) {
                slot_list[w[1]] = slot_list[w[2]] = true;
                form[q] = 'L';
            }
            if ((op == CB_TERM_STARTS || op == CB_TERM_ENDS || op == CB_TERM_CONTAINS) && xk == CB_OPK_SLOT && yk == CB_OPK_CONST &&
                v64_tag(consts[w[2]]) == CB_V64_STRING && pred_terms.size() < 32) {
                form[q] = 'P';
                pred_of[q] = (uint32_t)pred_terms.size();
                pred_terms.push_back(q);
            }
            break;
        }
    }
    std::vector<int> atom_pred(atoms.src.size(), -1);
    uint32_t n_pred_bits = (uint32_t)pred_terms.size();
    for (uint32_t a = 0; a < atoms.src.size(); a++)
        if (atoms.only_slot[a] != CB_NONE32 && !atoms.reads_pid[a] && n_pred_bits + 2 <= 32) { atom_pred[a] = (int)n_pred_bits; n_pred_bits += 2; }
    std::map<std::pair<uint32_t, uint32_t>, bool> masks;
    std::vector<std::pair<uint32_t, uint32_t>> mask_of(terms.size());
    for (int pass = 0; pass < 2; pass++)
        for (uint32_t q = 0; q < terms.size(); q++) {
            const uint32_t *w = terms[q].data();
            const uint32_t op = w[0] & 0xFF;
            if (form[q] != 'L' || (op != CB_TERM_SUBSET && op != CB_TERM_INTERSECTS) || (op == CB_TERM_SUBSET) != (pass == 0)) continue;
            std::pair<uint32_t, uint32_t> k(w[1], w[2]);
            if (op == CB_TERM_INTERSECTS && !masks.count(k) && masks.count({w[2], w[1]})) k = {w[2], w[1]};
            masks[k] = true;
            mask_of[q] = k;
        }
    auto sl = [](uint32_t v) { return "cols.slot(" + std::to_string(v) + "u)"; };
    auto operand = [&](uint32_t kind, uint32_t v, uint32_t aux) -> std::string {
        if (kind == CB_OPK_CONST) return hex64(consts[v]);
        if (kind == CB_OPK_PID) return "(((uint64_t)(CB_V64_BOX_BASE | CB_V64_STRING) << 48) | pid)";
        if (v >= ns) return "";
        if (kind == CB_OPK_SLOT) return sl(v);
        const std::string l = "cols.l" + std::to_string(v);
        if (kind == CB_OPK_SLOT_SIZE && slot_list[v]) return "list_size(t, b, " + sl(v) + ", " + l + ")";
        if (kind == CB_OPK_SLOT_ELEM && slot_list[v] && aux < 8) return "list_elem(t, b, " + sl(v) + ", " + l + ", " + std::to_string(aux) + "u)";
        return "";
    };
    struct Probe {
        uint32_t kind, v, aux;
        std::string value;
    };
    auto probe_operand = [&](uint32_t q) -> Probe {
        const uint32_t *w = terms[q].data();
        const uint32_t op = w[0] & 0xFF, xk = (w[0] >> 16) & 0xFF;
        if (op == CB_TERM_IN_CS) return Probe{CB_OPK_CONST, w[1], 0, hex64(consts[w[1]])};
        if (op == CB_TERM_IN_SS) return Probe{CB_OPK_SLOT, w[1], 0, sl(w[1])};
        const std::string x = operand(xk, w[1], w[3] & 0xFFFFu);
        if (!x.empty()) return Probe{xk, w[1], w[3] & 0xFFFFu, x};
        return Probe{CB_NONE32, 0, 0, "uc_term_operand(t, b, cols, pid, " + hex(xk) + ", " + hex(w[1]) + ", " + hex(w[3] & 0xFFFFu) + ")"};
    };
    std::map<uint32_t, std::vector<Probe>> probes;
    std::vector<uint32_t> probe_of(terms.size(), CB_NONE32);
    for (uint32_t q = 0; q < terms.size(); q++) {
        const uint32_t op = terms[q][0] & 0xFF;
        if (form[q] != 'L' || (op != CB_TERM_IN_CS && op != CB_TERM_IN_SS && op != CB_TERM_IN)) continue;
        std::vector<Probe> &ps = probes[terms[q][2]];
        const Probe x = probe_operand(q);
        uint32_t p = 0;
        while (p < ps.size() && ps[p].value != x.value) p++;
        if (p == ps.size() && p < 32) ps.push_back(x);
        if (p < ps.size()) probe_of[q] = p;
    }
    auto term_code = [&](uint32_t q) -> std::string {
        const uint32_t *w = terms[q].data();
        const uint32_t op = w[0] & 0xFF, flags = (w[0] >> 8) & 0xFF, xk = (w[0] >> 16) & 0xFF, yk = w[0] >> 24;
        const bool kinds = op <= CB_TERM_SUBSET;
        const std::string x = kinds ? operand(xk, w[1], w[3] & 0xFFFFu) : "", y = kinds && op != CB_TERM_HAS ? operand(yk, w[2], w[3] >> 16) : "";
        if (form[q] == 'P') return "strpred_tri(b, " + sl(w[1]) + ", " + std::to_string(pred_of[q]) + "u)";
        if (form[q] == 'L') {
            if (op == CB_TERM_IN_CS || op == CB_TERM_IN_SS || op == CB_TERM_IN) {
                const std::string v = std::to_string(w[2]);
                if (probe_of[q] == CB_NONE32) return "list_in_tri(" + probe_operand(q).value + ", cols.l" + v + ", slow)";
                const std::string xp = "x" + v + "_" + std::to_string(probe_of[q]);
                return "list_in_tri(" + xp + ", cols.l" + v + ".st, h" + v + " & " + hex(1u << probe_of[q]) + ", slow)";
            }
            const std::string a = std::to_string(mask_of[q].first), bb = std::to_string(mask_of[q].second);
            return std::string("list_set_tri(") + (op == CB_TERM_SUBSET ? "true" : "false") + ", cols.l" + a + ", cols.l" + bb + ", m" + a + "_" + bb + ", slow)";
        }
        if (w[1] < ns && w[2] < ns) {
            if (op == CB_TERM_EQ_SS) return "eq_tri(" + sl(w[1]) + ", " + sl(w[2]) + ", slow)";
            if (op == CB_TERM_ORD_SS) return "ord_tri(" + hex(flags & CB_TERM_CI_MASK) + ", " + sl(w[1]) + ", " + sl(w[2]) + ", slow)";
        }
        if (op == CB_TERM_EQ_SP && w[1] < ns) return "eq_tri(" + sl(w[1]) + ", " + operand(CB_OPK_PID, 0, 0) + ", slow)";
        if (op == CB_TERM_HAS && !x.empty()) return "has_tri(" + x + ")";
        if (op == CB_TERM_CMP && !x.empty() && !y.empty()) return "cmp_tri(" + hex(flags & CB_TERM_CI_MASK) + ", " + x + ", " + y + ", slow)";
        if ((op == CB_TERM_STARTS || op == CB_TERM_ENDS || op == CB_TERM_CONTAINS) && !x.empty() && !y.empty())
            return "str_tri(t, b, " + std::to_string(op) + "u, " + x + ", " + y + ")";
        const std::string e = term_expr(w, consts, theap);
        return e.compare(0, 9, "term_tri(") == 0 ? "uc_" + e : e;
    };
    const uint32_t kMaxRegSlots = 16;
    const bool have_atoms = !atoms.src.empty();
    atoms.slot_used.resize(ns, false);
    uint32_t n_reg = 0;
    for (uint32_t v = 0; v < ns; v++) n_reg += slot_used[v] || slot_list[v];
    if (n_reg > kMaxRegSlots)
        for (uint32_t v = 0; v < ns; v++) if (!slot_list[v]) slot_used[v] = false;
    std::vector<char> ty(ns, 0);
    std::vector<uint32_t> list_need(ns, 0);
    bool typed = n_reg > 0 && n_reg <= kMaxRegSlots;
    auto want = [&](uint32_t v, char k) {
        if (v >= ns || !k) { typed = false; return; }
        if (ty[v] && ty[v] != k) typed = false;
        ty[v] = k;
    };
    auto const_type = [&](uint64_t c) -> char {
        const uint32_t tag = v64_tag(c);
        double d;
        memcpy(&d, &c, sizeof d);
        if (tag == 0) return d == d ? 'N' : 0;
        if (tag == CB_V64_STRING) return (uint32_t)(c >> 32) == (uint32_t)(CB_V64_BOX_BASE | CB_V64_STRING) << 16 ? 'S' : 0;
        if (tag == CB_V64_BOOL) return (c >> 1) == (uint64_t)(CB_V64_BOX_BASE | CB_V64_BOOL) << 47 ? 'B' : 0;
        return 0;
    };
    auto operand_type = [&](uint32_t kind, uint32_t v, uint32_t aux) -> char {
        if (kind == CB_OPK_CONST) return const_type(consts[v]);
        if (kind == CB_OPK_PID) return 'S';
        if (v >= ns || !slot_list[v] || (kind == CB_OPK_SLOT_ELEM && aux >= 8)) return kind == CB_OPK_SLOT ? 0 : 'X';
        if (kind == CB_OPK_SLOT_SIZE) return 'N';
        if (kind == CB_OPK_SLOT_ELEM) { list_need[v] = aux + 1 > list_need[v] ? aux + 1 : list_need[v]; return 'S'; }
        return 0;
    };
    auto in_const_type = [&](uint32_t q) -> char {
        const uint64_t *p = theap + (consts[terms[q][2]] & 0xFFFFFFFFFFFFull);
        if (p[0] == 0 || p[0] > 16) return 0;
        char k = const_type(p[1]);
        for (uint32_t j = 1; j < (uint32_t)p[0]; j++) k = const_type(p[1 + j]) == k ? k : 0;
        return k == 'S' || k == 'N' ? k : 0;
    };
    for (uint32_t q = 0; q < terms.size() && typed; q++) {
        const uint32_t *w = terms[q].data();
        const uint32_t op = w[0] & 0xFF, xk = (w[0] >> 16) & 0xFF, yk = w[0] >> 24;
        switch (op) {
        case CB_TERM_EQ_SS: case CB_TERM_ORD_SS: break;
        case CB_TERM_EQ_SC: want(w[1], const_type(consts[w[2]])); break;
        case CB_TERM_ORD_SC: want(w[1], const_type(consts[w[2]]) == 'N' ? 'N' : 0); break;
        case CB_TERM_EQ_SP: want(w[1], 'S'); break;
        case CB_TERM_IN_SC: want(w[1], in_const_type(q)); break;
        case CB_TERM_IN_SS: want(w[1], 'S'); want(w[2], 'L'); break;
        case CB_TERM_IN_CS: want(w[2], 'L'); break;
        default: {
            if (op == CB_TERM_HAS) { if (xk != CB_OPK_SLOT) typed = false; break; }
            const char tx = operand_type(xk, w[1], w[3] & 0xFFFFu), tyy = operand_type(yk, w[2], w[3] >> 16);
            if (tx == 'X' || tyy == 'X') { typed = false; break; }
            if (form[q] == 'L') {
                if (op == CB_TERM_IN) { if (xk == CB_OPK_SLOT) want(w[1], 'S'); want(w[2], 'L'); }
                else { want(w[1], 'L'); want(w[2], 'L'); }
                break;
            }
            if (op == CB_TERM_STARTS || op == CB_TERM_ENDS || op == CB_TERM_CONTAINS) {
                if (xk == CB_OPK_SLOT) want(w[1], 'S');
                if (yk == CB_OPK_SLOT) want(w[2], 'S');
                break;
            }
            if (xk == CB_OPK_SLOT && yk != CB_OPK_SLOT) want(w[1], tyy);
            if (yk == CB_OPK_SLOT && xk != CB_OPK_SLOT) want(w[2], tx);
            break;
        }
        }
    }
    for (uint32_t v = 0; v < ns && typed; v++) {
        if (slot_list[v]) want(v, 'L');
        if ((slot_used[v] || slot_list[v]) && (!ty[v] || atoms.slot_used[v])) typed = false;
    }
    auto typed_operand = [&](uint32_t kind, uint32_t v, uint32_t aux, char &k) -> std::string {
        const std::string V = std::to_string(v);
        if (kind == CB_OPK_CONST) {
            const uint64_t c = consts[v];
            k = const_type(c);
            if (k == 'S') return hex((uint32_t)c);
            if (k == 'N') return "u2d(" + hex64(c) + ")";
            if (k == 'B') return c & 1u ? "true" : "false";
            return "";
        }
        if (kind == CB_OPK_PID) { k = 'S'; return "pid"; }
        if (kind == CB_OPK_SLOT_SIZE) { k = 'N'; return "(double)cols.l" + V + ".len"; }
        if (kind == CB_OPK_SLOT_ELEM) { k = 'S'; return "typed_id(cols.l" + V + ".e[" + std::to_string(aux) + "])"; }
        k = v < ns && (ty[v] == 'S' || ty[v] == 'N' || ty[v] == 'B') ? ty[v] : 0;
        return k == 'S' ? "typed_id(cols.k" + V + ")" : k == 'N' ? "cols.d" + V : k == 'B' ? "cols.b" + V : "";
    };
    auto typed_term = [&](uint32_t q) -> std::string {
        const uint32_t *w = terms[q].data();
        const uint32_t op = w[0] & 0xFF, flags = (w[0] >> 8) & 0xFF, xk = (w[0] >> 16) & 0xFF, yk = w[0] >> 24, ci = flags & CB_TERM_CI_MASK;
        if (form[q] == 'P') return "typed_strpred(b, typed_id(cols.k" + std::to_string(w[1]) + "), " + std::to_string(pred_of[q]) + "u)";
        if (form[q] == 'L') {
            if (op == CB_TERM_IN_CS || op == CB_TERM_IN_SS || op == CB_TERM_IN) {
                if (probe_of[q] == CB_NONE32) return "";
                if (op == CB_TERM_IN_CS && const_type(consts[w[1]]) == 0) return "";
                if (op == CB_TERM_IN && xk == CB_OPK_CONST && const_type(consts[w[1]]) == 0) return "";
                return "(h" + std::to_string(w[2]) + " & " + hex(1u << probe_of[q]) + ") != 0u";
            }
            const std::string a = std::to_string(mask_of[q].first), bb = std::to_string(mask_of[q].second);
            return op == CB_TERM_SUBSET ? "m" + a + "_" + bb + " == (1u << cols.l" + a + ".len) - 1u" : "m" + a + "_" + bb + " != 0u";
        }
        char kx = 0, ky = 0;
        std::string x, y;
        switch (op) {
        case CB_TERM_EQ_SS: case CB_TERM_ORD_SS:
            x = typed_operand(CB_OPK_SLOT, w[1], 0, kx); y = typed_operand(CB_OPK_SLOT, w[2], 0, ky);
            if (!kx || kx != ky) return "";
            if (op == CB_TERM_EQ_SS) return x + " == " + y;
            return kx == 'N' ? "typed_ord(" + hex(ci) + ", " + x + ", " + y + ")" : "";
        case CB_TERM_EQ_SC: case CB_TERM_ORD_SC:
            x = typed_operand(CB_OPK_SLOT, w[1], 0, kx); y = typed_operand(CB_OPK_CONST, w[2], 0, ky);
            if (!kx || kx != ky) return "";
            if (op == CB_TERM_EQ_SC) return x + " == " + y;
            return kx == 'N' ? "typed_ord(" + hex(ci) + ", " + x + ", " + y + ")" : "";
        case CB_TERM_EQ_SP: return "typed_id(cols.k" + std::to_string(w[1]) + ") == pid";
        case CB_TERM_IN_SC: {
            const uint64_t *p = theap + (consts[w[2]] & 0xFFFFFFFFFFFFull);
            x = typed_operand(CB_OPK_SLOT, w[1], 0, kx);
            if (!kx || kx != in_const_type(q)) return "";
            std::string e;
            for (uint32_t j = 0; j < (uint32_t)p[0]; j++)
                e += std::string(j ? " | " : "") + "(" + x + " == " + (kx == 'S' ? hex((uint32_t)p[1 + j]) : "u2d(" + hex64(p[1 + j]) + ")") + ")";
            return e;
        }
        case CB_TERM_HAS: return "true";
        case CB_TERM_CMP:
            x = typed_operand(xk, w[1], w[3] & 0xFFFFu, kx); y = typed_operand(yk, w[2], w[3] >> 16, ky);
            if (!kx || !ky) return "";
            if (ci == 0) return kx == ky ? x + " == " + y : "false";
            return kx == 'N' && ky == 'N' ? "typed_ord(" + hex(ci) + ", " + x + ", " + y + ")" : "";
        case CB_TERM_STARTS: case CB_TERM_ENDS: case CB_TERM_CONTAINS:
            x = typed_operand(xk, w[1], w[3] & 0xFFFFu, kx); y = typed_operand(yk, w[2], w[3] >> 16, ky);
            if (kx != 'S' || ky != 'S') return "";
            return "str_tri(t, b, " + std::to_string(op) + "u, typed_box(" + x + "), typed_box(" + y + ")) == TRI_T";
        default: return "";
        }
    };
    std::vector<std::string> tterm(terms.size());
    for (uint32_t q = 0; q < terms.size() && typed; q++) {
        tterm[q] = typed_term(q);
        typed = !tterm[q].empty();
    }
    auto probe_key = [&](const Probe &x) -> std::string {
        const std::string V = std::to_string(x.v);
        if (x.kind == CB_OPK_CONST || x.kind == CB_OPK_PID) return "list_probe_key(" + x.value + ")";
        if (x.kind == CB_OPK_SLOT) return x.v < ns && ty[x.v] == 'S' ? "cols.k" + V : "";
        if (x.kind == CB_OPK_SLOT_ELEM) return "list_elem_key(t, b, cols, " + V + "u, cols.l" + V + ", " + std::to_string(x.aux) + "u)";
        return "";
    };
    for (const auto &pl : probes)
        for (const Probe &x : pl.second) typed &= !probe_key(x).empty();
    std::string s;
    s += "// generated by cb_specialize.h (generate_uc) from the loaded table: every distinct condition, straight-line\n";
    s += "namespace cb {\n";
    for (const std::string &a : atoms.src) s += a;
    auto reg = [&](uint32_t v) { return slot_used[v] || slot_list[v]; };
    s += "struct SpecRegs {\n    CachedCols g;\n";
    for (uint32_t v = 0; v < ns; v++)
        if (reg(v)) s += "    uint64_t s" + std::to_string(v) + ";\n";
    if (typed) {
        s += "    bool typed;   // every slot below holds the type its terms compare it as (SpecConds::load)\n";
        for (uint32_t v = 0; v < ns; v++) {
            const std::string V = std::to_string(v);
            if (ty[v] == 'S') s += "    ListKey k" + V + ";   // string: its probe key (the id when typed)\n";
            if (ty[v] == 'N') s += "    double d" + V + ";\n";
            if (ty[v] == 'B') s += "    bool b" + V + ";\n";
        }
    }
    for (uint32_t v = 0; v < ns; v++)
        if (slot_list[v]) s += "    ListRegs l" + std::to_string(v) + ";\n";
    s += "    CB_HD uint64_t slot(uint32_t v) const {\n        switch (v) {\n";
    for (uint32_t v = 0; v < ns && !typed; v++)
        if (reg(v)) s += "        case " + std::to_string(v) + "u: return s" + std::to_string(v) + ";\n";
    s += "        default: return v < " + std::to_string(ns) + "u ? g.slot(v) : (uint64_t)(CB_V64_BOX_BASE | CB_V64_ERROR) << 48;\n        }\n    }\n};\n";
    s += "struct SpecConds {\n    static constexpr uint32_t n_strpred = " + std::to_string(n_pred_bits) + "u;\n";
    s += std::string("    static constexpr int kForm = ") + (n_uconds <= 31 ? "CB_UC_FORM_MASK32" : n_uconds <= 63 ? "CB_UC_FORM_MASK64" : "CB_UC_FORM_INDEX") + ";   // how the rows name their conditions\n";
    s += "    static constexpr uint32_t kScopeRows = " + std::to_string(scope_rows) + "u;   // rows the walk visits per scope (cb::uc_walk)\n";
    s += "    static constexpr uint32_t kDenyRows = " + std::to_string(deny_rows) + "u, kAllowRows = " + std::to_string(allow_rows) +
         "u;   // segment slots (0 / 0: row ranges)\n";
    s += std::string("    static constexpr bool kPrograms = ") + (have_atoms ? "true" : "false") + ";   // leaf programs: needs the value helpers of cb_core.h\n";
    s += "    template <typename Cols>\n    CB_HD SpecRegs load(const TableView t, const BatchView &b, const Cols &c) const {\n        SpecRegs r;\n        r.g.b = c.b; r.g.n = c.n;\n";
    for (uint32_t v = 0; v < ns; v++)
        if (reg(v)) s += "        r.s" + std::to_string(v) + " = c.slot(" + std::to_string(v) + "u);\n";
    if (typed) {
        std::string guard;
        for (uint32_t v = 0; v < ns; v++) {
            const std::string V = std::to_string(v);
            if (!reg(v)) continue;
            if (ty[v] == 'L') s += "        r.l" + V + " = list_load(t, b, r.s" + V + ");\n";
            if (ty[v] == 'S') s += "        r.k" + V + " = list_probe_key(r.s" + V + ");\n";
            if (ty[v] == 'N') s += "        r.d" + V + " = u2d(r.s" + V + ");\n";
            if (ty[v] == 'B') s += "        r.b" + V + " = (r.s" + V + " & 1u) != 0;\n";
            guard += std::string(guard.empty() ? "" : " & ") + (ty[v] == 'L' ? "typed_list(r.l" + V + ", " + std::to_string(list_need[v]) + "u)"
                                                                 : std::string(ty[v] == 'S' ? "typed_str" : ty[v] == 'N' ? "typed_num" : "typed_bool") + "(r.s" + V + ")");
        }
        s += "        r.typed = " + guard + ";\n";
    } else {
        for (uint32_t v = 0; v < ns; v++)
            if (slot_list[v]) s += "        r.l" + std::to_string(v) + " = list_load(t, b, r.s" + std::to_string(v) + ");\n";
    }
    s += "        return r;\n    }\n";
    s += "    // the predicate word of one string (pre-pass over the string dictionary; bit p = predicate p holds)\n";
    s += "    CB_HD uint32_t strpred(const TableView t, const BatchView &b, uint32_t id) const {\n";
    s += "        OneCols cols; cols.x = ((uint64_t)(CB_V64_BOX_BASE | CB_V64_STRING) << 48) | id;\n        bool slow = false; uint32_t bits = 0u; const uint32_t pid = 0u;\n";
    for (uint32_t p = 0; p < pred_terms.size(); p++) {
        const uint32_t *w = terms[pred_terms[p]].data();
        s += "        bits |= (uint32_t)(term_tri(t, b, cols, pid, U4{" + hex(w[0]) + ", 0x0u, " + hex(w[2]) + ", " + hex(w[3]) + "}, slow) == TRI_T) << " + std::to_string(p) + ";\n";
    }
    {
        bool any = false;
        for (int p : atom_pred) any |= p >= 0;
        if (any) {
            s += "        Ctx c; c.t = &t; c.b = &b; c.req = 0; c.pid = 0; c.edr = 0;\n";
            for (uint32_t a = 0; a < atoms.src.size(); a++)
                if (atom_pred[a] >= 0)
                    s += "        c.unsupported = 0; c.scr_used = 0; bits |= (uint32_t)uc_atom_" + std::to_string(a) + "(c, cols) << " + std::to_string(atom_pred[a]) +
                         "; bits |= (uint32_t)(c.unsupported != 0) << " + std::to_string(atom_pred[a] + 1) + ";\n";
        }
    }
    s += "        (void)slow; (void)pid;\n        return bits;\n    }\n";
    s += "    CB_HD CondWord operator()(const TableView t, const BatchView &b, const SpecRegs &cols, uint32_t pid, uint64_t n, bool &slow) const {\n";
    const std::string in = typed ? "            " : "        ";
    for (const auto &pl : probes) {
        const std::string v = std::to_string(pl.first);
        std::string keys;
        for (uint32_t p = 0; p < pl.second.size(); p++) {
            const std::string xp = "x" + v + "_" + std::to_string(p);
            if (!typed) s += "        const uint64_t " + xp + " = " + pl.second[p].value + ";\n";
            keys += std::string(p ? ", " : "") + (typed ? probe_key(pl.second[p]) : "list_probe_key(" + xp + ")");
        }
        s += "        const ListKey k" + v + "[" + std::to_string(pl.second.size()) + "] = {" + keys + "};\n";
        s += "        const uint32_t h" + v + " = list_probe(cols.l" + v + ", k" + v + ");   // bit p: x" + v + "_p is an element of slot " + v + "\n";
    }
    for (const auto &m : masks) {
        const std::string a = std::to_string(m.first.first), bb = std::to_string(m.first.second);
        s += "        const uint32_t m" + a + "_" + bb + " = list_mask(cols.l" + a + ", cols.l" + bb + ");   // elements of slot " + a + " in slot " + bb + "\n";
    }
    std::string tri;
    if (typed)
        for (const auto &pl : probes)
            for (uint32_t p = 0; p < pl.second.size(); p++)
                tri += in + "const uint64_t x" + std::to_string(pl.first) + "_" + std::to_string(p) + " = " + pl.second[p].value + ";\n";
    for (int list_terms = 1; list_terms >= 0; list_terms--)
        for (uint32_t q = 0; q < terms.size(); q++)
            if ((form[q] == 'L') == (list_terms == 1)) tri += in + "const int q" + std::to_string(q) + " = " + term_code(q) + ";\n";
    std::string atom_src;
    if (have_atoms) {
        atom_src += "        Ctx c; c.t = &t; c.b = &b; c.req = n; c.pid = pid; c.unsupported = 0; c.edr = 0; c.scr_used = 0;\n";
        for (uint32_t a = 0; a < atoms.src.size(); a++) {
            const std::string A = std::to_string(a);
            if (atom_pred[a] >= 0) {
                const std::string P = std::to_string(atom_pred[a]), V = sl(atoms.only_slot[a]);
                atom_src += "        bool a" + A + ";\n        {\n            const uint64_t x = " + V + ";\n            const uint32_t w = v64_tag(x) == CB_V64_STRING && !v64_bad(x) ? ldg(b.strpred + (uint32_t)(x & 0xFFFFFFFFu)) >> " + P + " : 2u;\n";
                atom_src += "            if (w & 2u) { c.scr_used = 0; a" + A + " = uc_atom_" + A + "(c, cols); } else a" + A + " = (w & 1u) != 0;\n        }\n";
            } else {
                atom_src += "        c.scr_used = 0; const bool a" + A + " = uc_atom_" + A + "(c, cols);\n";
            }
        }
        atom_src += "        slow |= c.unsupported != 0;   // a value the device forms cannot hold: the general kernel reports it\n";
    } else atom_src += "        (void)n;\n";
    std::string typed_src;
    std::vector<std::string> cond_src(n_uconds + 1);
    if (typed) {
        typed_src += "        if (uc_typed(cols.typed)) {   // every term a plain boolean: no error, no deferral\n";
        for (uint32_t q = 0; q < terms.size(); q++) typed_src += "            const bool t" + std::to_string(q) + " = " + tterm[q] + ";\n";
    }
    for (uint32_t u = 1; u <= n_uconds; u++) {
        const uint32_t *cd = uconds + 4 * u;
        const std::string word = u < 64 ? "val.lo" : "val.hi", sh = std::to_string(u & 63u);
        if (!formula[u].empty()) {
            cond_src[u] = "        " + word + " |= (uint64_t)(" + formula[u] + ") << " + sh + ";   // distinct condition " + std::to_string(u) + " (program)\n";
            continue;
        }
        const uint32_t nt = cd[3] & 0xFFFFu, negate = (cd[3] >> 24) & 1u;
        std::string &c = cond_src[u];
        c += in + "{   // distinct condition " + std::to_string(u) + "\n" + in + "    bool any = false, group = true;\n";
        std::string any, group;
        for (uint32_t i = 0; i < nt; i++) {
            const uint32_t *w = code + 2 * (cd[2] + 2 * i);
            const uint32_t flags = (w[0] >> 8) & 0xFFu;
            const uint32_t q = term_ids[{w[0] & kUseMask, w[1], w[2], w[3]}];
            c += in + "    group &= term_lit(q" + std::to_string(q) + ", " + hex(flags) + ");\n";
            group += std::string(group.empty() ? "" : " & ") + (flags & CB_TERM_LIT_F ? "!t" : "t") + std::to_string(q);
            if (flags & CB_TERM_GROUP_END) {
                c += in + "    any |= group; group = true;\n";
                any += std::string(any.empty() ? "" : " | ") + "(" + group + ")";
                group.clear();
            }
        }
        c += in + "    " + word + std::string(" |= (uint64_t)(any != ") + (negate ? "true" : "false") + ") << " + sh + ";\n" + in + "}\n";
        if (any.empty()) any = "false";
        typed_src += "            " + word + " |= (uint64_t)(" + (negate ? "!(" + any + ")" : any) + ") << " + sh + ";   // condition " + std::to_string(u) + "\n";
    }
    if (typed) {
        s += atom_src + "        CondWord val; val.lo = 1ull; val.hi = 0ull;\n" + typed_src + "        } else {   // the tri-state terms on the slot words, reloaded (cols.slot)\n" + tri;
        for (uint32_t u = 1; u <= n_uconds; u++) if (formula[u].empty()) s += cond_src[u];
        s += "        }\n";
        for (uint32_t u = 1; u <= n_uconds; u++) if (!formula[u].empty()) s += cond_src[u];
    } else {
        s += tri + atom_src + "        CondWord val; val.lo = 1ull; val.hi = 0ull;\n";
        for (uint32_t u = 1; u <= n_uconds; u++) s += cond_src[u];
    }
    s += "        return val;\n    }\n};\n}  // namespace cb\n";
    out.src = s;
    out.n_strpred = n_pred_bits;
    out.n_atoms = (uint32_t)atoms.src.size();
    return out;
}

}
```

### cerbos_b200/csrc/cerbos_b200.cu

```cuda
#include <cuda_runtime.h>
#include <dlfcn.h>
#include <sys/stat.h>
#include <unistd.h>

#include <atomic>
#include <cstdarg>
#include <cstdio>
#include <cstdlib>
#include <cstring>
#include <map>
#include <mutex>
#include <new>
#include <string>
#include <thread>
#include <vector>

#include "cb_core.h"
#include "cb_kernels.h"
#include "cb_specialize.h"
#include "cb_uc.h"
#include "cb_encode.h"
#include "cb_narrow.h"
#include "cb_host.h"
#include "cb_embed.inc"
// ... 24 lines not shown
    __shared__ __align__(8) uint64_t mbar_tab, mbar_col[4];
    cbk::check_tiles_body<cb::GenericBlocks>(td, bv, bitmap, effects, status, n_slots, smem_image, &mbar_tab, mbar_col);
}

__global__ void __launch_bounds__(kThreads, 2) check_meta_kernel(const __grid_constant__ TableDesc td, const __grid_constant__ cb::BatchView bv, uint8_t *effects,
                                                             uint32_t *action_meta, cb_request_meta *req_meta, uint32_t *status) {
    const uint64_t count = bv.count_dev ? (uint64_t)*bv.count_dev : bv.count;
    for (uint64_t i = (uint64_t)blockIdx.x * kThreads + threadIdx.x; i < count; i += (uint64_t)gridDim.x * kThreads)
        cb::eval_request_meta(td.base, &td.lay, &bv, bv.first + (bv.perm ? bv.perm[i] : i), effects, action_meta, req_meta, status);
    if (bv.count_dev) {
        __shared__ uint32_t last;
        __syncthreads();
        if (threadIdx.x == 0) {
            __threadfence();
            last = atomicAdd(bv.count_dev + 1, 1u) == gridDim.x - 1;
            if (blockIdx.x == 0) bv.count_dev[3] += (uint32_t)count;
        }
        __syncthreads();
        if (last && threadIdx.x == 0) { bv.count_dev[0] = 0; bv.count_dev[1] = 0; }
    }
}

constexpr uint32_t kMaxNarrowSlots = 64;
struct WidenParams {
    const uint32_t *pid; const uint16_t *hdr16; const uint8_t *versions; const uint8_t *roles;
    const void *slot_src[kMaxNarrowSlots];
    uint8_t slot_class[kMaxNarrowSlots];
    cb_hdr0 *hdr0; cb_hdr1 *hdr1; uint32_t *roles_out; uint64_t *slots_out;
    uint64_t first, count, stride;
    uint32_t role_cols, n_slots;
    uint32_t slot_base[kMaxNarrowSlots], slot_base2[kMaxNarrowSlots];
    const uint16_t *pid16; uint32_t pid_base;
    uint32_t hdr_const_mask, hdr_w; uint16_t hdr_const[4];
    uint32_t versions_const; uint8_t versions_value[2];
};
__device__ __forceinline__ uint64_t widen_special(uint32_t code) {
    return (uint64_t)(CB_V64_BOX_BASE | (code == 0 ? CB_V64_ABSENT : code == 1 ? CB_V64_ERROR : CB_V64_NULL)) << 48;
}
__global__ void __launch_bounds__(kThreads) widen_kernel(const __grid_constant__ WidenParams p) {
    for (uint64_t i = (uint64_t)blockIdx.x * kThreads + threadIdx.x; i < p.count; i += (uint64_t)gridDim.x * kThreads) {
        const uint64_t n = p.first + i;
        uint32_t f16[4];
        if (p.hdr_const_mask == 0) {
            const uint2 h = reinterpret_cast<const uint2 *>(p.hdr16)[n];
            f16[0] = h.x & 0xFFFF; f16[1] = h.x >> 16; f16[2] = h.y & 0xFFFF; f16[3] = h.y >> 16;
        } else {
            const uint16_t *hp = p.hdr16 + n * p.hdr_w;
            uint32_t q = 0;
            for (uint32_t f = 0; f < 4; f++) f16[f] = (p.hdr_const_mask >> f) & 1u ? p.hdr_const[f] : hp[q++];
        }
        const uint32_t k16 = f16[0], rs16 = f16[1], ps16 = f16[2], aset = f16[3];
        cb_hdr0 h0;
        h0.principal_id = p.pid16 ? p.pid_base + p.pid16[n] : p.pid[n];
        h0.kind_class = k16 == 0xFFFF ? CB_KIND_NONE : (k16 & 0x8000) ? ((k16 & 0x7FFF) | CB_KIND_CLASS_CSR_BIT) : k16;
        h0.resource_scope = rs16 == 0xFFFF ? CB_SCOPE_NONE : (rs16 & 0x8000) ? ((rs16 & 0x7FFF) | CB_SCOPE_INEXACT_BIT) : rs16;
        h0.principal_scope = ps16 == 0xFFFF ? CB_SCOPE_NONE : (ps16 & 0x8000) ? ((ps16 & 0x7FFF) | CB_SCOPE_INEXACT_BIT) : ps16;
        p.hdr0[n] = h0;
        const uint32_t rv = p.versions_const ? p.versions_value[0] : p.versions[2 * n], pv = p.versions_const ? p.versions_value[1] : p.versions[2 * n + 1];
        cb_hdr1 h1;
        h1.resource_version = (uint16_t)(rv == 0xFF ? CB_NONE16 : rv); h1.principal_version = (uint16_t)(pv == 0xFF ? CB_NONE16 : pv); h1.action_set_id = aset;
        p.hdr1[n] = h1;
        for (uint32_t c = 0; c < p.role_cols; c++) {
            const uint32_t r = p.roles[(uint64_t)c * p.stride + n];
            p.roles_out[(uint64_t)c * p.stride + n] = r == 0xFF ? CB_ROLE_PAD : r == 0xFE ? CB_ROLE_UNKNOWN : r;
        }
        for (uint32_t v = 0; v < p.n_slots; v++) {
            uint64_t out;
            switch (p.slot_class[v]) {
            case CGPU_SLOT_U32_ID: {
                const uint32_t w = static_cast<const uint32_t *>(p.slot_src[v])[n];
                if (w < 0xFFFFFFF0u) out = ((uint64_t)(CB_V64_BOX_BASE | CB_V64_STRING) << 48) | w;
                else if (w >= 0xFFFFFFFDu) out = widen_special(0xFFFFFFFFu - w);
                else out = ((uint64_t)(CB_V64_BOX_BASE | CB_V64_BOOL) << 48) | (w == 0xFFFFFFFBu ? 1u : 0u);
                break;
            }
            case CGPU_SLOT_U32_HEAP: {
                const uint32_t w = static_cast<const uint32_t *>(p.slot_src[v])[n];
                if (w >= 0xFFFFFFFDu) out = widen_special(0xFFFFFFFFu - w);
                else out = ((uint64_t)(CB_V64_BOX_BASE | ((w & 0x80000000u) ? CB_V64_MAP : CB_V64_LIST)) << 48) | CB_V64_HEAP_BATCH_BIT | (w & 0x7FFFFFFFu);
                break;
            }
            case CGPU_SLOT_F32: {
                const uint32_t w = static_cast<const uint32_t *>(p.slot_src[v])[n];
                if ((w & 0x7FC00000u) == 0x7FC00000u && (w & 0x3FFFFFu)) out = widen_special((w & 3u) - 1u);
                else if (w == 0x7FC00000u) out = CB_V64_CANON_NAN;
                else out = (uint64_t)__double_as_longlong((double)__uint_as_float(w));
                break;
            }
            case CGPU_SLOT_U8: {
                const uint32_t w = static_cast<const uint8_t *>(p.slot_src[v])[n];
                out = w <= 1 ? (((uint64_t)(CB_V64_BOX_BASE | CB_V64_BOOL) << 48) | w) : widen_special(w == 3 ? 0u : w == 4 ? 1u : 2u);
                break;
            }
            case CGPU_SLOT_U16_ID: {
                const uint32_t w = static_cast<const uint16_t *>(p.slot_src[v])[n];
                if (w < 0xFFF0u) out = ((uint64_t)(CB_V64_BOX_BASE | CB_V64_STRING) << 48) | (uint64_t)(w < 0x8000u ? p.slot_base[v] + w : p.slot_base2[v] + (w - 0x8000u));
                else if (w >= 0xFFFDu) out = widen_special(0xFFFFu - w);
                else out = ((uint64_t)(CB_V64_BOX_BASE | CB_V64_BOOL) << 48) | (w == 0xFFFBu ? 1u : 0u);
                break;
            }
            case CGPU_SLOT_U8_NUM: {
                const uint32_t w = static_cast<const uint8_t *>(p.slot_src[v])[n];
                out = w >= 0xFDu ? widen_special(0xFFu - w) : (uint64_t)__double_as_longlong((double)w);
                break;
            }
            default: out = static_cast<const uint64_t *>(p.slot_src[v])[n]; break;
            }
            p.slots_out[(uint64_t)v * p.stride + n] = out;
        }
    }
}
__global__ void __launch_bounds__(kThreads) widen_heap_kernel(const uint32_t *src, uint64_t *dst, uint64_t n) {
    for (uint64_t i = (uint64_t)blockIdx.x * kThreads + threadIdx.x; i < n; i += (uint64_t)gridDim.x * kThreads) {
        const uint32_t w = src[i];
        dst[i] = (w & 0x80000000u) ? (((uint64_t)(CB_V64_BOX_BASE | CB_V64_STRING) << 48) | (w & 0x7FFFFFFFu)) : (uint64_t)w;
    }
}

__global__ void __launch_bounds__(kThreads) widen_heap16_kernel(const uint16_t *src, uint64_t *dst, uint64_t n, uint32_t base, uint32_t base2) {
    for (uint64_t i = (uint64_t)blockIdx.x * kThreads + threadIdx.x; i < n; i += (uint64_t)gridDim.x * kThreads) {
        const uint32_t w = src[i];
        dst[i] = (w & 0x8000u) ? (((uint64_t)(CB_V64_BOX_BASE | CB_V64_STRING) << 48) | (uint64_t)(((w & 0x4000u) ? base2 : base) + (w & 0x3FFFu))) : (uint64_t)w;
    }
}

template <bool kStaged>
__global__ void __launch_bounds__(kThreads, CB_MIN_BLOCKS) check_uc(const __grid_constant__ TableDesc td, const __grid_constant__ cb::BatchView bv, uint8_t *bitmap,
                                                                  uint8_t *effects, uint32_t *status, const uint32_t) {
    extern __shared__ __align__(128) uint8_t smem_image[];
    __shared__ __align__(8) uint64_t mbar;
    (void)status;
    cbk::check_uc_body<cb::GenericConds, cb::CachedCols, kStaged>(td, bv, bitmap, effects, smem_image, &mbar);
}
template <bool kStaged>
__global__ void __launch_bounds__(kThreads, CB_MIN_BLOCKS) check_uc_meta(const __grid_constant__ TableDesc td, const __grid_constant__ cb::BatchView bv, uint8_t *effects,
                                                                       uint32_t *action_meta, cb_request_meta *req_meta, const cb::U4 *side) {
    extern __shared__ __align__(128) uint8_t smem_image[];
    __shared__ __align__(8) uint64_t mbar;
    cbk::check_uc_body<cb::GenericConds, cb::CachedCols, kStaged>(td, bv, nullptr, effects, smem_image, &mbar, cbk::UcMeta{action_meta, req_meta, side});
}

struct SignalParams { uint32_t *flags[cb::CB_MAX_GATHER]; const uint32_t *wait_flags; uint32_t n_ranks, my_rank, step, wait_step; };
__global__ void __launch_bounds__(kThreads) uc_merge_rows(const __grid_constant__ TableDesc td, const __grid_constant__ cb::BatchView bv, cb::U4 *out, const uint32_t n_pk) {
    const uint32_t j = blockIdx.x * kThreads + threadIdx.x;
    if (j >= n_pk) return;
    cb::TableView tv;
    tv.base = td.base; tv.L = &td.lay;
    const uint32_t n_u = td.lay.uc_n_rows;
    cb::UcRowsGlobal g; g.urows = tv.urows(); g.row_am = bv.row_am; g.RCP = bv.rcp; g.nR = td.lay.nR;
    out[j] = g.aset(tv, bv, j / n_u).merged(tv, j % n_u);
}

__global__ void gather_signal(const __grid_constant__ SignalParams p) {
    asm volatile("griddepcontrol.wait;" ::: "memory");
    __threadfence_system();
    if (threadIdx.x < p.n_ranks) asm volatile("red.release.sys.global.max.u32 [%0], %1;" ::"l"(p.flags[threadIdx.x] + p.my_rank), "r"(p.step) : "memory");
    if (p.wait_step) cbk::gather_wait_flags(p.wait_flags, p.n_ranks, p.wait_step);
}
__global__ void gather_wait(const uint32_t *flags, uint32_t n_ranks, uint32_t step) {
    if (threadIdx.x < n_ranks) {
        uint32_t v;
        do {
            asm volatile("ld.acquire.sys.global.u32 %0, [%1];" : "=r"(v) : "l"(flags + threadIdx.x) : "memory");
        } while ((int32_t)(v - step) < 0);
    }
}

constexpr uint32_t kClusterChunk = 2048;
constexpr uint32_t kMaxBuckets = 4096;

struct ClusterParams {
    const cb_hdr0 *hdr0;
    const cb_hdr1 *hdr1;
    uint64_t first;
    uint32_t count, window, nb;
    uint32_t nV, nRP, nS;
    uint16_t *keys;
    uint32_t *hist;
    uint32_t *perm;
};

__device__ __forceinline__ uint32_t cluster_key(const ClusterParams &p, uint64_t n) {
    const cb::U4 h0 = cb::ldcol128(p.hdr0 + n);
    const uint64_t h1 = cb::ldcol64(reinterpret_cast<const uint64_t *>(p.hdr1 + n));
    uint32_t kc = h0.y & ~CB_KIND_CLASS_CSR_BIT, rs = h0.z & ~CB_SCOPE_INEXACT_BIT, rv = (uint32_t)(h1 & 0xFFFF);
    kc = kc < p.nRP ? kc : p.nRP;
    rs = rs < p.nS ? rs : p.nS;
    rv = rv < p.nV ? rv : p.nV;
    return ((rv * (p.nRP + 1) + kc) * (p.nS + 1) + rs) & (p.nb - 1);
}

__global__ void __launch_bounds__(kThreads) cluster_count(const __grid_constant__ ClusterParams p) {
    __shared__ uint32_t hist[kMaxBuckets];
    for (uint32_t j = threadIdx.x; j < p.nb; j += kThreads) hist[j] = 0;
    __syncthreads();
    const uint32_t c0 = blockIdx.x * kClusterChunk;
    for (uint32_t q = 0; q < kClusterChunk / kThreads; q++) {
        const uint32_t i = c0 + q * kThreads + threadIdx.x;
        if (i < p.count) {
            const uint32_t k = cluster_key(p, p.first + i);
            p.keys[i] = (uint16_t)k;
            atomicAdd(&hist[k], 1u);
        }
    }
    __syncthreads();
    uint32_t *g = p.hist + (uint64_t)(c0 / p.window) * p.nb;
    for (uint32_t j = threadIdx.x; j < p.nb; j += kThreads)
        if (hist[j]) atomicAdd(g + j, hist[j]);
}

__global__ void __launch_bounds__(kThreads) cluster_scan(const __grid_constant__ ClusterParams p) {
    __shared__ uint32_t part[kThreads];
    uint32_t *g = p.hist + (uint64_t)blockIdx.x * p.nb;
    const uint32_t per = (p.nb + kThreads - 1) / kThreads;
    const uint32_t j0 = threadIdx.x * per;
    uint32_t sum = 0;
    for (uint32_t j = j0; j < j0 + per && j < p.nb; j++) sum += g[j];
    part[threadIdx.x] = sum;
    __syncthreads();
    for (uint32_t d = 1; d < kThreads; d <<= 1) {
        uint32_t v = threadIdx.x >= d ? part[threadIdx.x - d] : 0;
        __syncthreads();
        part[threadIdx.x] += v;
        __syncthreads();
    }
    uint32_t run = part[threadIdx.x] - sum;
    for (uint32_t j = j0; j < j0 + per && j < p.nb; j++) { uint32_t c = g[j]; g[j] = run; run += c; }
}

__global__ void __launch_bounds__(kThreads) cluster_scatter(const __grid_constant__ ClusterParams p) {
    __shared__ uint32_t hist[kMaxBuckets];
    for (uint32_t j = threadIdx.x; j < p.nb; j += kThreads) hist[j] = 0;
    __syncthreads();
    const uint32_t c0 = blockIdx.x * kClusterChunk;
    uint32_t key[kClusterChunk / kThreads], rank[kClusterChunk / kThreads];
#pragma unroll
    for (uint32_t q = 0; q < kClusterChunk / kThreads; q++) {
        const uint32_t i = c0 + q * kThreads + threadIdx.x;
        key[q] = 0; rank[q] = 0;
        if (i < p.count) { key[q] = p.keys[i]; rank[q] = atomicAdd(&hist[key[q]], 1u); }
    }
    __syncthreads();
    uint32_t *g = p.hist + (uint64_t)(c0 / p.window) * p.nb;
    for (uint32_t j = threadIdx.x; j < p.nb; j += kThreads)
        if (hist[j]) hist[j] = atomicAdd(g + j, hist[j]);
    __syncthreads();
    const uint32_t wbase = (c0 / p.window) * p.window;
#pragma unroll
    for (uint32_t q = 0; q < kClusterChunk / kThreads; q++) {
        const uint32_t i = c0 + q * kThreads + threadIdx.x;
        if (i < p.count) p.perm[wbase + hist[key[q]] + rank[q]] = i;
    }
}

thread_local std::string g_err;

int fail(int code, const char *fmt, ...) {
    char buf[512];
    va_list ap;
    va_start(ap, fmt);
    vsnprintf(buf, sizeof(buf), fmt, ap);
    va_end(ap);
    g_err = buf;
    return code;
}
#define CUDA_TRY(expr)                                                                                   \
    do {                                                                                                 \
        cudaError_t e__ = (expr);                                                                        \
        if (e__ != cudaSuccess) return fail(CGPU_ERR_CUDA, "%s failed: %s", #expr, cudaGetErrorString(e__)); \
    } while (0)

struct Slot {
    cudaStream_t stream = nullptr;
    cudaStream_t h2d = nullptr, d2h = nullptr;
    std::vector<cudaEvent_t> ev;
    void *dev = nullptr;
    size_t dev_cap = 0;
    uint32_t *h_status = nullptr;
    uint32_t *d_status = nullptr;
    bool busy = false;
};

enum class Kernel : uint8_t {
    General, GeneralGlobal,
    Lean, LeanGlobal, LeanTiles,
    Uc, UcGlobal,
    SpecTiles, SpecDirect,
    SpecUc, SpecUcGlobal,
    UcMeta, UcMetaGlobal, SpecUcMeta, SpecUcMetaGlobal,
};
constexpr int kKernels = (int)Kernel::SpecUcMetaGlobal + 1;

struct LaunchPlan {
    Kernel kernel = Kernel::General;
    uint32_t smem = 0;
    uint32_t last_arg = 0;
    bool stage = false;
    bool lean = false;
    bool uc = false;
    bool uc_staged = false;
    bool col_tiles = false;
    bool cluster = false;
    bool spec = false;
    bool strpred = false;
    bool merge_rows = false;
    bool serialise = false;
};

template <class T> struct LaneBuf {
    T *ptr = nullptr;
    size_t cap = 0;
    cudaError_t fit(size_t n, size_t min_cap, cudaStream_t stream) {
        if (cap >= n) return cudaSuccess;
        size_t c = min_cap;
        while (c < n) c <<= 1;
        T *fresh = nullptr;
        const cudaError_t e = cudaMallocAsync(reinterpret_cast<void **>(&fresh), c * sizeof(T), stream);
        if (e != cudaSuccess) return e;
        T *old = ptr;
        ptr = fresh;
        cap = c;
        return old ? cudaFreeAsync(old, stream) : cudaSuccess;
    }
};

}

struct cgpu_ctx {
    int device = 0;
    int sm_count = 0;
    uint32_t *d_status = nullptr;
    std::atomic<uint64_t> launches{0};
    std::mutex mu;
    std::vector<Slot> slots;
    LaunchPlan last_plan;
    uint32_t last_grid = 0, last_window = 0, last_buckets = 0;
    int force_no_stage = 0;
    int force_general = 0;
    int cluster_mode = -1;
    int force_no_tiles = 0;
    int force_no_jit = 0;
    struct DeferLane {
        uint32_t seq = 0;
        uint32_t *cells = nullptr;
        struct Bufs {
            LaneBuf<uint32_t> list;
            LaneBuf<uint32_t> strpred;
            LaneBuf<cb::U4> pk;
        } q[4];
    };
    std::map<cudaStream_t, DeferLane> defer_lanes;
    std::mutex defer_mu;
    cudaStream_t copy_stream = nullptr;
    cudaEvent_t copy_ev[16] = {};
    uint32_t copy_seq = 0;
    struct SliceUse { const void *ptr; cudaEvent_t done; uint8_t *stage; size_t stage_bytes; };
    std::vector<SliceUse> slice_uses;
    std::mutex copy_mu;
    std::vector<cgpu_ctx *> peers;
    int uc_mode = -1;
    bool profiling = false;
    cudaEvent_t ev0 = nullptr, ev1 = nullptr;
    double prof_ms = 0;
    uint64_t prof_n = 0;
    bool prof_pending = false;
};

struct cgpu_encoder { cbenc::Encoder enc; };
struct cgpu_encoded {
    cbenc::Columns cols;
    void *pinned = nullptr;
    size_t pinned_cap = 0;
    const void *ptrs[CGPU_N_COLUMNS] = {};
    size_t bytes[CGPU_N_COLUMNS] = {};
    uint32_t flags = 0;
    uint32_t n_slots = 0, role_cols = 1;
};
struct cgpu_narrowed {
    cbnarrow::Narrowed nb;
    const cgpu_encoded *enc = nullptr;
    void *pinned = nullptr;
    bool pinned_is_malloc = false;
    size_t pinned_cap = 0;
    const void *pid = nullptr, *hdr16 = nullptr, *versions = nullptr, *roles = nullptr, *heap = nullptr;
    std::vector<const void *> slot_ptrs;
    size_t heap_bytes = 0;
    const void *cols[CGPU_N_COLUMNS] = {};
    size_t col_bytes[CGPU_N_COLUMNS] = {};
};

struct cgpu_table {
    cgpu_ctx *ctx = nullptr;
    std::atomic<int> refs{1};
    uint8_t *d_image = nullptr;
    TableDesc desc{};
    uint32_t meta[CB_META_WORDS]{};
    mutable std::atomic<uint64_t> occ[kKernels]{};
    std::vector<uint8_t> host_image;
    std::mutex spec_mu;
    std::atomic<int> spec_state{0};
    cudaLibrary_t spec_lib = nullptr;
    cudaKernel_t spec_tiles = nullptr, spec_direct = nullptr, spec_uc = nullptr, spec_uc_global = nullptr, spec_strpred = nullptr;
    cudaKernel_t spec_uc_meta = nullptr, spec_uc_meta_global = nullptr;
    uint32_t spec_n_strpred = 0;
    std::string spec_note;
    uint64_t sec_len[cbhost::kMaxSec]{};
    std::vector<cgpu_table *> peer_tables;
    cbuc::Image uc;
    uint8_t *d_uc_image = nullptr;
    TableDesc uc_desc{};
    cbuc::MetaSide uc_meta;
    cb::U4 *d_uc_meta = nullptr;
    std::thread spec_thread;
    std::mutex join_mu;
};

namespace {

int invalid(const std::string &why) { return why.empty() ? CGPU_OK : fail(CGPU_ERR_INVALID, "%s", why.c_str()); }

struct Nvrtc {
    void *h = nullptr;
    int (*create)(void **, const char *, const char *, int, const char *const *, const char *const *) = nullptr;
    int (*compile)(void *, int, const char *const *) = nullptr;
    int (*log_size)(void *, size_t *) = nullptr;
    int (*log)(void *, char *) = nullptr;
    int (*cubin_size)(void *, size_t *) = nullptr;
    int (*cubin)(void *, char *) = nullptr;
    int (*destroy)(void **) = nullptr;
    bool ok = false;
};
Nvrtc &nvrtc() {
    static Nvrtc n;
    static std::once_flag once;
    std::call_once(once, [] {
        for (const char *name : {"libnvrtc.so.12", "libnvrtc.so"}) {
            n.h = dlopen(name, RTLD_NOW | RTLD_LOCAL);
            if (n.h) break;
        }
        if (!n.h) return;
        n.create = reinterpret_cast<decltype(n.create)>(dlsym(n.h, "nvrtcCreateProgram"));
        n.compile = reinterpret_cast<decltype(n.compile)>(dlsym(n.h, "nvrtcCompileProgram"));
        n.log_size = reinterpret_cast<decltype(n.log_size)>(dlsym(n.h, "nvrtcGetProgramLogSize"));
        n.log = reinterpret_cast<decltype(n.log)>(dlsym(n.h, "nvrtcGetProgramLog"));
        n.cubin_size = reinterpret_cast<decltype(n.cubin_size)>(dlsym(n.h, "nvrtcGetCUBINSize"));
        n.cubin = reinterpret_cast<decltype(n.cubin)>(dlsym(n.h, "nvrtcGetCUBIN"));
        n.destroy = reinterpret_cast<decltype(n.destroy)>(dlsym(n.h, "nvrtcDestroyProgram"));
        n.ok = n.create && n.compile && n.log_size && n.log && n.cubin_size && n.cubin && n.destroy;
    });
    return n;
}

const char kSpecPrelude[] =
    "#define CB_LEAN_ONLY 1\n"
    "#ifndef CB_SPEC_MIN_BLOCKS\n#define CB_SPEC_MIN_BLOCKS 5\n#endif\n"
    "typedef unsigned char uint8_t; typedef unsigned short uint16_t; typedef unsigned int uint32_t; typedef unsigned long long uint64_t;\n"
    "typedef signed char int8_t; typedef short int16_t; typedef int int32_t; typedef long long int64_t; typedef unsigned long long uintptr_t;\n";
const char kSpecKernels[] =
    "\nextern \"C\" __global__ void __launch_bounds__(256, CB_SPEC_MIN_BLOCKS) cb_spec_tiles(const __grid_constant__ cbk::TableDesc td, const __grid_constant__ cb::BatchView bv,\n"
    "        uint8_t *bitmap, uint8_t *effects, uint32_t *status, const uint32_t n_slots) {\n"
    "    extern __shared__ __align__(128) uint8_t smem_image[];\n"
    "    __shared__ __align__(8) uint64_t mbar_tab, mbar_col[4];\n"
    "    cbk::check_tiles_body<cb::SpecBlocks>(td, bv, bitmap, effects, status, n_slots, smem_image, &mbar_tab, mbar_col);\n"
    "}\n"
    "extern \"C\" __global__ void __launch_bounds__(256, CB_SPEC_MIN_BLOCKS) cb_spec_direct(const __grid_constant__ cbk::TableDesc td, const __grid_constant__ cb::BatchView bv,\n"
    "        uint8_t *bitmap, uint8_t *effects, uint32_t *status, const uint32_t stage_rt) {\n"
    "    extern __shared__ __align__(128) uint8_t smem_image[];\n"
    "    __shared__ __align__(8) uint64_t mbar;\n"
    "    cbk::check_body<true, 1, cb::SpecBlocks>(td, bv, bitmap, effects, status, stage_rt, smem_image, &mbar);\n"
    "}\n";
const char kSpecUcStaged[] =
    "\nextern \"C\" __global__ void __launch_bounds__(256, CB_SPEC_UC_MIN_BLOCKS) cb_spec_uc(const __grid_constant__ cbk::TableDesc td, const __grid_constant__ cb::BatchView bv,\n"
    "        uint8_t *bitmap, uint8_t *effects, uint32_t *status, const uint32_t) {\n"
    "    extern __shared__ __align__(128) uint8_t smem_image[];\n"
    "    __shared__ __align__(8) uint64_t mbar;\n"
    "    cbk::check_uc_body<cb::SpecConds, cb::GlobalCols, true>(td, bv, bitmap, effects, smem_image, &mbar);\n"
    "}\n";
const char kSpecUcGlobal[] =
    "\nextern \"C\" __global__ void __launch_bounds__(256, CB_SPEC_UC_MIN_BLOCKS) cb_spec_uc_global(const __grid_constant__ cbk::TableDesc td, const __grid_constant__ cb::BatchView bv,\n"
    "        uint8_t *bitmap, uint8_t *effects, uint32_t *status, const uint32_t) {\n"
    "    cbk::check_uc_body<cb::SpecConds, cb::GlobalCols, false>(td, bv, bitmap, effects, nullptr, nullptr);\n"
    "}\n";
const char kSpecUcMetaStaged[] =
    "\nextern \"C\" __global__ void __launch_bounds__(256, CB_SPEC_UC_MIN_BLOCKS) cb_spec_uc_meta(const __grid_constant__ cbk::TableDesc td, const __grid_constant__ cb::BatchView bv,\n"
    "        uint8_t *effects, uint32_t *action_meta, cb_request_meta *req_meta, const cb::U4 *side) {\n"
    "    extern __shared__ __align__(128) uint8_t smem_image[];\n"
    "    __shared__ __align__(8) uint64_t mbar;\n"
    "    cbk::check_uc_body<cb::SpecConds, cb::GlobalCols, true>(td, bv, nullptr, effects, smem_image, &mbar, cbk::UcMeta{action_meta, req_meta, side});\n"
    "}\n";
const char kSpecUcMetaGlobal[] =
    "\nextern \"C\" __global__ void __launch_bounds__(256, CB_SPEC_UC_MIN_BLOCKS) cb_spec_uc_meta_global(const __grid_constant__ cbk::TableDesc td, const __grid_constant__ cb::BatchView bv,\n"
    "        uint8_t *effects, uint32_t *action_meta, cb_request_meta *req_meta, const cb::U4 *side) {\n"
    "    cbk::check_uc_body<cb::SpecConds, cb::GlobalCols, false>(td, bv, nullptr, effects, nullptr, nullptr, cbk::UcMeta{action_meta, req_meta, side});\n"
    "}\n";
const char kSpecUcStrpred[] =
    "\nextern \"C\" __global__ void __launch_bounds__(256) cb_spec_strpred(const __grid_constant__ cbk::TableDesc td, const __grid_constant__ cb::BatchView bv, uint32_t *out, const uint32_t n) {\n"
    "    const uint32_t id = blockIdx.x * 256u + threadIdx.x;\n"
    "    cb::TableView tv; tv.base = td.base; tv.L = &td.lay;\n"
    "    if (id < n) out[id] = cb::SpecConds().strpred(tv, bv, id);\n"
    "}\n";

uint64_t fnv1a(const void *p, size_t n, uint64_t h = 1469598103934665603ull) {
    const uint8_t *b = static_cast<const uint8_t *>(p);
    for (size_t i = 0; i < n; i++) { h ^= b[i]; h *= 1099511628211ull; }
    return h;
}
std::string cache_path(uint64_t key) {
    const char *d = getenv("CERBOS_B200_CACHE_DIR");
    std::string dir;
    if (d) { if (!d[0]) return ""; dir = d; }
    else { const char *home = getenv("HOME"); if (!home || !home[0]) return ""; dir = std::string(home) + "/.cache/cerbos_b200"; }
    char name[64];
    snprintf(name, sizeof name, "/spec_%016llx.cubin", (unsigned long long)key);
    return dir + name;
}
bool cache_read(const std::string &path, std::vector<char> *out) {
    if (path.empty()) return false;
    FILE *f = fopen(path.c_str(), "rb");
    if (!f) return false;
    fseek(f, 0, SEEK_END);
    const long n = ftell(f);
    fseek(f, 0, SEEK_SET);
    bool ok = n > 0;
    if (ok) { out->resize((size_t)n); ok = fread(out->data(), 1, (size_t)n, f) == (size_t)n; }
    fclose(f);
    return ok;
}
void cache_write(const std::string &path, const std::vector<char> &data) {
    if (path.empty()) return;
    const std::string dir = path.substr(0, path.rfind('/'));
    for (size_t i = 1; i <= dir.size(); i++)
        if (i == dir.size() || dir[i] == '/') mkdir(dir.substr(0, i).c_str(), 0755);
    const std::string tmp = path + ".tmp" + std::to_string((unsigned long long)getpid());
    FILE *f = fopen(tmp.c_str(), "wb");
    if (!f) return;
    const bool ok = fwrite(data.data(), 1, data.size(), f) == data.size();
    fclose(f);
    if (ok) rename(tmp.c_str(), path.c_str()); else remove(tmp.c_str());
}

enum SpecForm { SPEC_NONE = 0, SPEC_SHAPES = 1, SPEC_UC = 2 };
constexpr uint32_t kUcMaxSmem = 72 * 1024;

uint64_t uc_smem_bytes(const cbuc::Image &uc, uint64_t n_pk) { return (((uint64_t)uc.lay.image_bytes + 127) & ~127ull) + 16 * n_pk; }
bool uc_stageable(const cbuc::Image &uc, uint64_t n_pk = 1) { return uc_smem_bytes(uc, n_pk) <= kUcMaxSmem; }

SpecForm spec_generate(const uint8_t *image, const cb::TableLayout &lay, const uint32_t *meta, const cbuc::Image &uc, std::string *gen, std::string *why, uint32_t *n_strpred,
                       uint32_t *n_atoms = nullptr) {
    *n_strpred = 0;
    if (n_atoms) *n_atoms = 0;
    if (!cbhost::lean_table(lay, meta)) {
        *why = "table is not lean-eligible (principal / role policies, parent roles or resource globs): general kernel only";
        return SPEC_NONE;
    }
    if (lay.image_bytes <= kMaxStageBytes) {
        *gen = cbspec::generate(image, lay.off, meta);
        if (!gen->empty()) return SPEC_SHAPES;
    }
    if (uc.ok) {
        cbspec::UcSource us = cbspec::generate_uc(uc.bytes.data(), uc.lay.off, uc.lay.uc_conds_off, uc.n_uconds, lay.n_slots, meta[CB_META_N_CONSTS]);
        *gen = us.src;
        *n_strpred = us.n_strpred;
        if (n_atoms) *n_atoms = us.n_atoms;
        if (!gen->empty()) return SPEC_UC;
    }
    *why = "table does not qualify (too many block shapes and: more than 127 distinct conditions, or a condition program the translator does not take -- "
           "list / map literals, collecting comprehensions, runtime.effectiveDerivedRoles)";
    return SPEC_NONE;
}

SpecForm spec_compile(const uint8_t *image, const cb::TableLayout &lay, const uint32_t *meta, const cbuc::Image &uc, std::vector<char> *cubin, std::string *why, uint32_t *n_strpred) {
    std::string gen;
    uint32_t n_atoms = 0;
    const SpecForm form = spec_generate(image, lay, meta, uc, &gen, why, n_strpred, &n_atoms);
    if (form == SPEC_NONE) return SPEC_NONE;
    std::string src = kSpecPrelude;
    if (n_atoms) src += "#define CB_SPEC_PROGRAMS 1\n";
    for (const char *const *p = kEmbedFormat; *p; p++) src += *p;
    for (const char *const *p = kEmbedCore; *p; p++) src += *p;
    src += gen;
    for (const char *const *p = kEmbedKernels; *p; p++) src += *p;
    if (form == SPEC_UC) {
        if (uc_stageable(uc)) { src += kSpecUcStaged; src += kSpecUcMetaStaged; }
        src += kSpecUcGlobal;
        src += kSpecUcMetaGlobal;
        src += kSpecUcStrpred;
    } else src += kSpecKernels;
    const char *mb = getenv("CERBOS_B200_SPEC_BLOCKS");
    const std::string mbopt = std::string("-DCB_SPEC_MIN_BLOCKS=") + (mb && mb[0] >= '1' && mb[0] <= '8' && !mb[1] ? mb : "5");
    const char *ub = getenv("CERBOS_B200_SPEC_UC_BLOCKS");
    const std::string ubopt = std::string("-DCB_SPEC_UC_MIN_BLOCKS=") + (ub && ub[0] >= '1' && ub[0] <= '8' && !ub[1] ? ub : n_atoms ? "2" : "3");
    if (const char *dump = getenv("CERBOS_B200_SPEC_DUMP")) {
        if (FILE *f = fopen(dump, "w")) { fwrite(src.data(), 1, src.size(), f); fclose(f); }
    }
    std::vector<std::string> defs;
    if (const char *xd = getenv("CERBOS_B200_SPEC_DEFS")) {
        std::string cur;
        for (const char *c = xd;; c++) {
            if (*c == ' ' || *c == 0) { if (!cur.empty()) defs.push_back(cur); cur.clear(); if (!*c) break; }
            else cur += *c;
        }
    }
    uint64_t key = fnv1a(ubopt.data(), ubopt.size(), fnv1a(mbopt.data(), mbopt.size(), fnv1a(src.data(), src.size())));
    for (const std::string &d : defs) key = fnv1a(d.data(), d.size(), key);
    const std::string cpath = cache_path(key);
    if (cache_read(cpath, cubin)) return form;
    Nvrtc &n = nvrtc();
    if (!n.ok) { *why = "libnvrtc not available"; return SPEC_NONE; }
    void *prog = nullptr;
    if (n.create(&prog, src.c_str(), "cerbos_b200_spec.cu", 0, nullptr, nullptr) != 0) { *why = "nvrtcCreateProgram failed"; return SPEC_NONE; }
    std::vector<const char *> opts = {"--gpu-architecture=sm_90a", "-std=c++17", "-lineinfo", mbopt.c_str(), ubopt.c_str()};
    for (const std::string &d : defs) opts.push_back(d.c_str());
    if (n_atoms) opts.push_back("--device-int128");
    const int rc = n.compile(prog, (int)opts.size(), opts.data());
    if (rc != 0) {
        size_t ls = 0;
        n.log_size(prog, &ls);
        std::string log(ls, '\0');
        if (ls) n.log(prog, &log[0]);
        n.destroy(&prog);
        *why = "NVRTC compile failed: " + log.substr(0, 600);
        return SPEC_NONE;
    }
    size_t cs = 0;
    n.cubin_size(prog, &cs);
    cubin->resize(cs);
    n.cubin(prog, cubin->data());
    n.destroy(&prog);
    cache_write(cpath, *cubin);
    return form;
}

bool ensure_spec(cgpu_ctx *ctx, cgpu_table *t) {
    int st = t->spec_state.load(std::memory_order_acquire);
    if (st != 0) return st > 0;
    std::lock_guard<std::mutex> g(t->spec_mu);
    st = t->spec_state.load(std::memory_order_acquire);
    if (st != 0) return st > 0;
    auto give_up = [&](const std::string &why) { t->spec_note = why; t->spec_state.store(-1, std::memory_order_release); return false; };
    if (ctx->force_no_jit) return give_up("disabled (CERBOS_B200_NO_JIT)");
    std::vector<char> cubin;
    std::string why;
    const SpecForm form = spec_compile(t->host_image.data(), t->desc.lay, t->meta, t->uc, &cubin, &why, &t->spec_n_strpred);
    if (form == SPEC_NONE) return give_up(why);
    if (cudaLibraryLoadData(&t->spec_lib, cubin.data(), nullptr, nullptr, 0, nullptr, nullptr, 0) != cudaSuccess) { cudaGetLastError(); return give_up("cudaLibraryLoadData failed"); }
    bool got = form == SPEC_UC ? (!uc_stageable(t->uc) || (cudaLibraryGetKernel(&t->spec_uc, t->spec_lib, "cb_spec_uc") == cudaSuccess &&
                                                            cudaLibraryGetKernel(&t->spec_uc_meta, t->spec_lib, "cb_spec_uc_meta") == cudaSuccess)) &&
                                     cudaLibraryGetKernel(&t->spec_uc_global, t->spec_lib, "cb_spec_uc_global") == cudaSuccess &&
                                     cudaLibraryGetKernel(&t->spec_uc_meta_global, t->spec_lib, "cb_spec_uc_meta_global") == cudaSuccess &&
                                     cudaLibraryGetKernel(&t->spec_strpred, t->spec_lib, "cb_spec_strpred") == cudaSuccess
                               : cudaLibraryGetKernel(&t->spec_tiles, t->spec_lib, "cb_spec_tiles") == cudaSuccess &&
                                     cudaLibraryGetKernel(&t->spec_direct, t->spec_lib, "cb_spec_direct") == cudaSuccess;
    if (!got) {
        cudaGetLastError();
        cudaLibraryUnload(t->spec_lib);
        t->spec_lib = nullptr;
        t->spec_tiles = t->spec_direct = t->spec_uc = t->spec_uc_global = t->spec_strpred = nullptr;
        t->spec_uc_meta = t->spec_uc_meta_global = nullptr;
        return give_up("cudaLibraryGetKernel failed");
    }
    t->spec_note = "ok";
    t->spec_state.store(1, std::memory_order_release);
    return true;
}

constexpr uint64_t kClusterMinRequests = 32768;
constexpr uint64_t kClusterWindowBytes = 12u << 20;

int launch_cluster(cgpu_ctx *ctx, const cgpu_table *t, const cb::BatchView &bv, uint32_t **perm_out, cudaStream_t stream) {
    const cb::TableLayout &lay = t->desc.lay;
    ClusterParams p{};
    p.hdr0 = bv.hdr0; p.hdr1 = bv.hdr1; p.first = bv.first; p.count = (uint32_t)bv.count;
    p.nV = lay.nV; p.nRP = lay.nRP; p.nS = lay.nS;
    const uint64_t nkeys = (uint64_t)(lay.nV + 1) * (lay.nRP + 1) * (lay.nS + 1);
    p.nb = 32;
    while (p.nb < nkeys && p.nb < kMaxBuckets) p.nb <<= 1;
    const uint64_t per_req = 24 + 4ull * bv.role_cols + 8ull * lay.n_slots + 16;
    uint64_t w = kClusterChunk;
    while (w * 2 * per_req <= kClusterWindowBytes) w <<= 1;
    while (w < 64ull * p.nb && w < (1ull << 22)) w <<= 1;
    p.window = (uint32_t)w;
    const uint32_t n_win = (uint32_t)((bv.count + w - 1) / w);
    const uint32_t n_chunks = (uint32_t)((bv.count + kClusterChunk - 1) / kClusterChunk);
    const size_t perm_bytes = ((size_t)bv.count * 4 + 255) & ~(size_t)255, keys_bytes = ((size_t)bv.count * 2 + 255) & ~(size_t)255;
    const size_t hist_bytes = (size_t)n_win * p.nb * 4;
    uint8_t *scratch = nullptr;
    CUDA_TRY(cudaMallocAsync(reinterpret_cast<void **>(&scratch), perm_bytes + keys_bytes + hist_bytes, stream));
    p.perm = reinterpret_cast<uint32_t *>(scratch);
    p.keys = reinterpret_cast<uint16_t *>(scratch + perm_bytes);
    p.hist = reinterpret_cast<uint32_t *>(scratch + perm_bytes + keys_bytes);
    CUDA_TRY(cudaMemsetAsync(p.hist, 0, hist_bytes, stream));
    cluster_count<<<n_chunks, kThreads, 0, stream>>>(p);
    cluster_scan<<<n_win, kThreads, 0, stream>>>(p);
    cluster_scatter<<<n_chunks, kThreads, 0, stream>>>(p);
    CUDA_TRY(cudaGetLastError());
    ctx->launches.fetch_add(3, std::memory_order_relaxed);
    ctx->last_window = p.window; ctx->last_buckets = p.nb;
    *perm_out = p.perm;
    return CGPU_OK;
}

int acquire_defer(cgpu_ctx *ctx, cudaStream_t stream, uint64_t count, uint32_t **list, uint32_t **cell, size_t n_strpred, uint32_t **strpred,
                  size_t n_pk, cb::U4 **pk) {
    std::lock_guard<std::mutex> g(ctx->defer_mu);
    cgpu_ctx::DeferLane &ln = ctx->defer_lanes[stream];
    if (!ln.cells) {
        CUDA_TRY(cudaMalloc(reinterpret_cast<void **>(&ln.cells), 4 * 16));
        CUDA_TRY(cudaMemset(ln.cells, 0, 4 * 16));
    }
    const uint32_t q = ln.seq++ & 3;
    cgpu_ctx::DeferLane::Bufs &b = ln.q[q];
    CUDA_TRY(b.list.fit(count, 1024, stream));
    if (n_strpred) CUDA_TRY(b.strpred.fit(n_strpred, 4096, stream));
    if (n_pk) CUDA_TRY(b.pk.fit(n_pk, 4096, stream));
    *list = b.list.ptr;
    *cell = ln.cells + 4 * q;
    *strpred = n_strpred ? b.strpred.ptr : nullptr;
    *pk = n_pk ? b.pk.ptr : nullptr;
    return CGPU_OK;
}

LaunchPlan plan_launch(const cgpu_ctx &ctx, const cgpu_table &t, const cb::BatchView &bv) {
    const cb::TableLayout &lay = t.desc.lay;
    LaunchPlan p;
    p.stage = !ctx.force_no_stage && lay.image_bytes <= kMaxStageBytes;
    const bool spec_ready = t.spec_state.load(std::memory_order_acquire) == 1;
    const bool uc_spec_ready = spec_ready && t.spec_uc_global != nullptr;
    const bool mostly_programs = t.uc.ok && !uc_spec_ready && 2 * (uint64_t)t.uc.n_gids_flat < t.uc.n_gids;
    p.lean = !ctx.force_general && !mostly_programs && cbhost::lean_eligible(lay, t.meta, bv);
    const uint64_t n_pk = (uint64_t)bv.n_asets * t.uc.lay.uc_n_rows;
    p.uc = p.lean && cbhost::uc_eligible(lay, t.uc, bv) && (uc_spec_ready || !t.uc.needs_spec()) && t.d_uc_image &&
           (ctx.uc_mode == 1 || (ctx.uc_mode != 0 && ctx.cluster_mode != 1 && t.meta[CB_META_BLOCK_SHAPES] > 1));
    p.cluster = !p.uc && bv.count < (1ull << 32) &&
                (ctx.cluster_mode == 1 || (ctx.cluster_mode != 0 && bv.count >= kClusterMinRequests && t.meta[CB_META_BLOCK_SHAPES] > 1));
    const uint32_t tile_bytes = cb::tile_cols_bytes(bv.role_cols, lay.n_slots);
    const uint64_t small_tabs = (uint64_t)bv.n_asets * lay.n_rows * 8 + (((uint64_t)bv.n_asets + 1) & ~1ull) * 4 + 16 + 2 * kThreads;
    const uint32_t tiles_smem = ((lay.image_bytes + 127u) & ~127u) + 2 * tile_bytes + (uint32_t)(small_tabs < 65536 ? small_tabs : 65536);
    auto al16 = [](const void *ptr) { return (reinterpret_cast<uintptr_t>(ptr) & 15) == 0; };
    p.col_tiles = !p.uc && p.lean && p.stage && !p.cluster && !ctx.force_no_tiles && tiles_smem <= kMaxTilesSmem && bv.stride % 4 == 0 &&
                  bv.first % 4 == 0 && al16(bv.hdr0) && al16(bv.hdr1) && al16(bv.roles) && al16(bv.slots);
    p.uc_staged = p.uc && !ctx.force_no_stage && uc_stageable(t.uc, n_pk) && (!uc_spec_ready || t.spec_uc != nullptr);
    p.spec = p.uc ? uc_spec_ready : p.lean && p.stage && bv.count < (1ull << 32) && spec_ready && t.spec_tiles != nullptr;
    p.kernel = p.uc        ? (p.spec ? (p.uc_staged ? Kernel::SpecUc : Kernel::SpecUcGlobal) : p.uc_staged ? Kernel::Uc : Kernel::UcGlobal)
             : p.spec      ? (p.col_tiles ? Kernel::SpecTiles : Kernel::SpecDirect)
             : p.col_tiles ? Kernel::LeanTiles
             : p.lean      ? (p.stage ? Kernel::Lean : Kernel::LeanGlobal)
                           : (p.stage ? Kernel::General : Kernel::GeneralGlobal);
    p.smem = p.uc ? (p.uc_staged ? (uint32_t)uc_smem_bytes(t.uc, n_pk) : 0) : p.col_tiles ? tiles_smem : p.stage ? lay.image_bytes : 0;
    p.last_arg = p.col_tiles ? lay.n_slots : p.stage ? 1u : 0u;
    p.serialise = p.spec && !p.uc && !ctx.profiling;
    p.strpred = p.uc && p.spec && t.spec_n_strpred;
    p.merge_rows = p.uc && !p.uc_staged && n_pk <= (1u << 19);
    return p;
}

const void *kernel_fn(const cgpu_table &t, Kernel k) {
    switch (k) {
    case Kernel::General:
    case Kernel::GeneralGlobal: return (const void *)check_kernel<false, 2>;
    case Kernel::Lean: return (const void *)check_kernel<true, 1>;
    case Kernel::LeanGlobal: return (const void *)check_kernel<true, 0>;
    case Kernel::LeanTiles: return (const void *)check_kernel_tiles;
    case Kernel::Uc: return (const void *)check_uc<true>;
    case Kernel::UcGlobal: return (const void *)check_uc<false>;
    case Kernel::SpecTiles: return (const void *)t.spec_tiles;
    case Kernel::SpecDirect: return (const void *)t.spec_direct;
    case Kernel::SpecUc: return (const void *)t.spec_uc;
    case Kernel::SpecUcGlobal: return (const void *)t.spec_uc_global;
    case Kernel::UcMeta: return (const void *)check_uc_meta<true>;
    case Kernel::UcMetaGlobal: return (const void *)check_uc_meta<false>;
    case Kernel::SpecUcMeta: return (const void *)t.spec_uc_meta;
    case Kernel::SpecUcMetaGlobal: return (const void *)t.spec_uc_meta_global;
    }
    return nullptr;
}
Kernel meta_kernel(Kernel k) {
    return k == Kernel::Uc ? Kernel::UcMeta : k == Kernel::UcGlobal ? Kernel::UcMetaGlobal : k == Kernel::SpecUc ? Kernel::SpecUcMeta : Kernel::SpecUcMetaGlobal;
}

struct MetaDev {
    uint32_t *action_meta;
    cb_request_meta *req_meta;
};

int resident_ctas(const cgpu_table &t, Kernel k, uint32_t smem) {
    std::atomic<uint64_t> &entry = t.occ[(int)k];
    const uint64_t e = entry.load(std::memory_order_relaxed);
    if ((uint32_t)e != 0 && (uint32_t)(e >> 32) == smem) return (int)(uint32_t)e;
    const void *fn = kernel_fn(t, k);
    int occ = 0;
    if (cudaFuncSetAttribute(fn, cudaFuncAttributeMaxDynamicSharedMemorySize, (int)kMaxStageBytes) != cudaSuccess ||
        cudaOccupancyMaxActiveBlocksPerMultiprocessor(&occ, fn, kThreads, smem) != cudaSuccess) {
        if (k < Kernel::SpecTiles || k == Kernel::UcMeta || k == Kernel::UcMetaGlobal) return fail(CGPU_ERR_CUDA, "kernel attribute / occupancy query failed: %s", cudaGetErrorString(cudaGetLastError()));
        cudaGetLastError();
        occ = CB_MIN_BLOCKS;
    }
    if (occ < 1) occ = 1;
    entry.store((uint64_t)smem << 32 | (uint32_t)occ, std::memory_order_relaxed);
    return occ;
}

cudaError_t launch_serialised(const void *fn, uint32_t grid, uint32_t block, uint32_t smem, cudaStream_t stream, void **args) {
    cudaLaunchConfig_t cfg = {};
    cfg.gridDim = dim3(grid); cfg.blockDim = dim3(block); cfg.dynamicSmemBytes = smem; cfg.stream = stream;
    cudaLaunchAttribute pdl[1];
    pdl[0].id = cudaLaunchAttributeProgrammaticStreamSerialization;
    pdl[0].val.programmaticStreamSerializationAllowed = 1;
    cfg.attrs = pdl; cfg.numAttrs = 1;
    return cudaLaunchKernelExC(&cfg, fn, args);
}

int launch_check(cgpu_ctx *ctx, const cgpu_table *t, const LaunchPlan &plan_in, const cb::BatchView &bv, uint8_t *d_bitmap, uint8_t *d_effects,
                 uint32_t *d_status, cudaStream_t stream, const MetaDev *md = nullptr) {
    LaunchPlan plan = plan_in;
    if (md) plan.kernel = meta_kernel(plan.kernel);
    const cb::TableLayout &lay = t->desc.lay;
    const uint64_t tiles = (bv.count + kThreads - 1) / kThreads;
    const int occ = resident_ctas(*t, plan.kernel, plan.smem);
    if (occ < 0) return occ;
    const uint64_t max_ctas = (uint64_t)ctx->sm_count * (uint64_t)occ;
    uint32_t grid = (uint32_t)(tiles < max_ctas ? tiles : max_ctas);
    if (grid == 0) grid = 1;
    TableDesc td = plan.uc ? t->uc_desc : t->desc;
    cb::BatchView bvv = bv;
    bvv.perm = nullptr;
    bvv.prefetch_slots = lay.n_slots <= 8 ? lay.n_slots : 0;
    uint32_t *perm = nullptr;
    if (plan.cluster) {
        int rc = launch_cluster(ctx, t, bv, &perm, stream);
        if (rc != CGPU_OK) return rc;
        bvv.perm = perm;
    }
    uint32_t last_arg = plan.last_arg;
    uint32_t *defer = nullptr;
    if (plan.lean) {
        uint32_t *cell = nullptr, *strpred = nullptr;
        cb::U4 *pk = nullptr;
        const uint32_t n_str = lay.nT + bv.n_bstr;
        const uint64_t n_pk = (uint64_t)bv.n_asets * t->uc.lay.uc_n_rows;
        int rc = acquire_defer(ctx, stream, bv.count, &defer, &cell, plan.strpred ? (size_t)n_str + 1 : 0, &strpred, plan.merge_rows ? (size_t)n_pk : 0, &pk);
        if (rc != CGPU_OK) return rc;
        if (plan.merge_rows) {
            uc_merge_rows<<<(unsigned)((n_pk + kThreads - 1) / kThreads), kThreads, 0, stream>>>(t->uc_desc, bvv, pk, (uint32_t)n_pk);
            CUDA_TRY(cudaGetLastError());
            ctx->launches.fetch_add(1, std::memory_order_relaxed);
            bvv.uc_rows_pk = pk;
        }
        bvv.defer_count = cell;
        bvv.tile_counter = plan.col_tiles ? cell + 2 : nullptr;
        bvv.defer_list = defer;
        if (plan.strpred && n_str) {
            TableDesc ptd = t->uc_desc;
            uint32_t n_arg = n_str;
            void *pargs[] = {&ptd, &bvv, &strpred, &n_arg};
            CUDA_TRY(cudaLaunchKernel((const void *)t->spec_strpred, dim3((n_str + 255) / 256), dim3(256), pargs, 0, stream));
            ctx->launches.fetch_add(1, std::memory_order_relaxed);
        }
        bvv.strpred = strpred;
    }
    const void *fn = kernel_fn(*t, plan.kernel);
    void *args[] = {&td, &bvv, &d_bitmap, &d_effects, &d_status, &last_arg};
    uint32_t *d_am = md ? md->action_meta : nullptr;
    cb_request_meta *d_rm = md ? md->req_meta : nullptr;
    const cb::U4 *d_side = t->d_uc_meta;
    void *margs[] = {&td, &bvv, &d_effects, &d_am, &d_rm, &d_side};
    if (ctx->profiling) {
        if (ctx->prof_pending && cudaEventSynchronize(ctx->ev1) == cudaSuccess) {
            float ms = 0;
            if (cudaEventElapsedTime(&ms, ctx->ev0, ctx->ev1) == cudaSuccess) { ctx->prof_ms += ms; ctx->prof_n++; }
            ctx->prof_pending = false;
        }
        CUDA_TRY(cudaEventRecord(ctx->ev0, stream));
    }
    if (plan.serialise) {
        CUDA_TRY(launch_serialised(fn, grid, kThreads, plan.smem, stream, args));
    } else {
        CUDA_TRY(cudaLaunchKernel(fn, dim3(grid), dim3(kThreads), md ? margs : args, plan.smem, stream));
    }
    CUDA_TRY(cudaGetLastError());
    if (ctx->profiling) { CUDA_TRY(cudaEventRecord(ctx->ev1, stream)); ctx->prof_pending = true; }
    if (md) {
        cb::BatchView dv = bv;
        dv.perm = defer;
        dv.count_dev = bvv.defer_count;
        const uint64_t gmax = (uint64_t)ctx->sm_count * 4;
        check_meta_kernel<<<(unsigned)(tiles < gmax ? tiles : gmax), kThreads, 0, stream>>>(t->desc, dv, d_effects, d_am, d_rm, d_status);
        CUDA_TRY(cudaGetLastError());
        ctx->launches.fetch_add(1, std::memory_order_relaxed);
    } else if (plan.lean) {
        cb::BatchView dv = bv;
        dv.perm = defer;
        dv.count_dev = bvv.defer_count;
        dv.prefetch_slots = 0;
        const Kernel gk = plan.stage ? Kernel::General : Kernel::GeneralGlobal;
        const uint32_t gsmem = plan.stage ? lay.image_bytes : 0;
        const int gocc = resident_ctas(*t, gk, gsmem);
        if (gocc < 0) return gocc;
        const uint64_t gmax = (uint64_t)ctx->sm_count;
        const uint32_t ggrid = (uint32_t)(tiles < gmax ? tiles : gmax);
        uint32_t stage_arg = plan.stage ? 1u : 0u;
        TableDesc gtd = t->desc;
        void *gargs[] = {&gtd, &dv, &d_bitmap, &d_effects, &d_status, &stage_arg};
        CUDA_TRY(launch_serialised(kernel_fn(*t, gk), ggrid ? ggrid : 1, kThreads, gsmem, stream, gargs));
        CUDA_TRY(cudaGetLastError());
        ctx->launches.fetch_add(1, std::memory_order_relaxed);
    }
    if (perm) CUDA_TRY(cudaFreeAsync(perm, stream));
    ctx->launches.fetch_add(1, std::memory_order_relaxed);
    ctx->last_plan = plan;
    ctx->last_grid = grid;
    return CGPU_OK;
}

}

extern "C" {

const char *cgpu_last_error(void) { return g_err.c_str(); }

int cgpu_init(const int *device_ids, int n_devices, cgpu_ctx **out) {
    if (!out) return fail(CGPU_ERR_INVALID, "cgpu_init: out is null");
    *out = nullptr;
    if (n_devices < 1 || !device_ids) return fail(CGPU_ERR_INVALID, "cgpu_init: at least one device; got %d", n_devices);
    if (n_devices > 1) {
        for (int i = 0; i < n_devices; i++)
            for (int j = 0; j < i; j++)
                if (device_ids[i] == device_ids[j]) return fail(CGPU_ERR_INVALID, "cgpu_init: device %d listed twice", device_ids[i]);
        cgpu_ctx *head = nullptr;
        int rc = cgpu_init(device_ids, 1, &head);
        if (rc != CGPU_OK) return rc;
        for (int i = 1; i < n_devices; i++) {
            cgpu_ctx *c = nullptr;
            rc = cgpu_init(device_ids + i, 1, &c);
            if (rc != CGPU_OK) { const std::string why = g_err; cgpu_shutdown(head); return fail(rc, "%s", why.c_str()); }
            head->peers.push_back(c);
        }
        *out = head;
        return CGPU_OK;
    }
    int count = 0;
    cudaError_t e = cudaGetDeviceCount(&count);
    if (e != cudaSuccess || count == 0) return fail(CGPU_ERR_NO_DEVICE, "no CUDA device available (%s); cerbos_b200 has no CPU fallback", e == cudaSuccess ? "device count 0" : cudaGetErrorString(e));
    if (device_ids[0] < 0 || device_ids[0] >= count) return fail(CGPU_ERR_INVALID, "cgpu_init: device %d out of range (0..%d)", device_ids[0], count - 1);
    cgpu_ctx *ctx = new (std::nothrow) cgpu_ctx();
    if (!ctx) return fail(CGPU_ERR_INVALID, "out of memory");
    ctx->device = device_ids[0];
    {
        cudaDeviceProp prop;
        cudaError_t ie = cudaSetDevice(ctx->device);
        if (ie == cudaSuccess) ie = cudaGetDeviceProperties(&prop, ctx->device);
        if (ie == cudaSuccess) { ctx->sm_count = prop.multiProcessorCount; ie = cudaMalloc(&ctx->d_status, sizeof(uint32_t)); }
        if (ie == cudaSuccess) ie = cudaMemset(ctx->d_status, 0, sizeof(uint32_t));
        if (ie != cudaSuccess) {
            if (ctx->d_status) cudaFree(ctx->d_status);
            delete ctx;
            return fail(CGPU_ERR_CUDA, "cgpu_init: %s", cudaGetErrorString(ie));
        }
    }
    const char *ns = getenv("CERBOS_B200_NO_STAGE");
    ctx->force_no_stage = ns && ns[0] == '1';
    const char *fg = getenv("CERBOS_B200_FORCE_GENERAL");
    ctx->force_general = fg && fg[0] == '1';
    const char *nj = getenv("CERBOS_B200_NO_JIT");
    ctx->force_no_jit = nj && nj[0] == '1';
    const char *nt = getenv("CERBOS_B200_NO_TILES");
    ctx->force_no_tiles = nt && nt[0] == '1';
    const char *um = getenv("CERBOS_B200_UC");
    ctx->uc_mode = um && (um[0] == '0' || um[0] == '1') ? um[0] - '0' : -1;
    const char *cm = getenv("CERBOS_B200_CLUSTER");
    ctx->cluster_mode = cm && (cm[0] == '0' || cm[0] == '1') ? cm[0] - '0' : -1;
    cudaMemPool_t pool;
    if (cudaDeviceGetDefaultMemPool(&pool, ctx->device) == cudaSuccess) {
        uint64_t keep = ~0ull;
        cudaMemPoolSetAttribute(pool, cudaMemPoolAttrReleaseThreshold, &keep);
    }
    ctx->slots.resize(4);
    *out = ctx;
    return CGPU_OK;
}

void cgpu_shutdown(cgpu_ctx *ctx) {
    if (!ctx) return;
    for (cgpu_ctx *p : ctx->peers) cgpu_shutdown(p);
    ctx->peers.clear();
    cudaSetDevice(ctx->device);
    cudaDeviceSynchronize();
    for (auto &s : ctx->slots) {
        if (s.stream) cudaStreamDestroy(s.stream);
        if (s.h2d) cudaStreamDestroy(s.h2d);
        if (s.d2h) cudaStreamDestroy(s.d2h);
        for (auto e : s.ev) cudaEventDestroy(e);
        if (s.dev) cudaFree(s.dev);
        if (s.h_status) cudaFreeHost(s.h_status);
        if (s.d_status) cudaFree(s.d_status);
    }
    if (ctx->d_status) cudaFree(ctx->d_status);
    for (auto &kv : ctx->defer_lanes) {
        for (auto &b : kv.second.q) { cudaFree(b.list.ptr); cudaFree(b.strpred.ptr); cudaFree(b.pk.ptr); }
        if (kv.second.cells) cudaFree(kv.second.cells);
    }
    if (ctx->copy_stream) cudaStreamDestroy(ctx->copy_stream);
    for (auto e : ctx->copy_ev) if (e) cudaEventDestroy(e);
    for (auto &u : ctx->slice_uses) { if (u.done) cudaEventDestroy(u.done); if (u.stage) cudaFree(u.stage); }
    if (ctx->ev0) cudaEventDestroy(ctx->ev0);
    if (ctx->ev1) cudaEventDestroy(ctx->ev1);
    delete ctx;
}

int cgpu_table_load(cgpu_ctx *ctx, const void *blob, size_t len, cgpu_table **out) {
    if (!ctx || !out) return fail(CGPU_ERR_INVALID, "cgpu_table_load: null argument");
    *out = nullptr;
    cgpu_table *t = new (std::nothrow) cgpu_table();
    if (!t) return fail(CGPU_ERR_INVALID, "out of memory");
    t->ctx = ctx;
    int rc = invalid(cbhost::parse_blob(blob, len, &t->desc.lay, t->meta, t->sec_len));
    if (rc != CGPU_OK) { delete t; return rc; }
    t->uc = cbuc::build(static_cast<const uint8_t *>(blob), t->desc.lay.off, t->sec_len, t->meta, t->desc.lay);
    cudaError_t e = cudaSetDevice(ctx->device);
    if (e == cudaSuccess) e = cudaMalloc(reinterpret_cast<void **>(&t->d_image), t->desc.lay.image_bytes);
    if (e == cudaSuccess) e = cudaMemcpy(t->d_image, blob, t->desc.lay.image_bytes, cudaMemcpyHostToDevice);
    if (e == cudaSuccess && t->uc.ok) {
        e = cudaMalloc(reinterpret_cast<void **>(&t->d_uc_image), t->uc.bytes.size());
        if (e == cudaSuccess) e = cudaMemcpy(t->d_uc_image, t->uc.bytes.data(), t->uc.bytes.size(), cudaMemcpyHostToDevice);
        t->uc_meta = cbuc::build_meta(static_cast<const uint8_t *>(blob), t->desc.lay.off, t->sec_len, t->meta, t->desc.lay, t->uc);
        if (e == cudaSuccess && t->uc_meta.ok) {
            e = cudaMalloc(reinterpret_cast<void **>(&t->d_uc_meta), t->uc_meta.words.size() * 4);
            if (e == cudaSuccess) e = cudaMemcpy(t->d_uc_meta, t->uc_meta.words.data(), t->uc_meta.words.size() * 4, cudaMemcpyHostToDevice);
        }
    }
    if (e != cudaSuccess) {
        if (t->d_image) cudaFree(t->d_image);
        if (t->d_uc_image) cudaFree(t->d_uc_image);
        if (t->d_uc_meta) cudaFree(t->d_uc_meta);
        delete t;
        return fail(CGPU_ERR_CUDA, "table upload failed: %s", cudaGetErrorString(e));
    }
    t->desc.base = t->d_image;
    t->uc_desc.base = t->d_uc_image;
    t->uc_desc.lay = t->uc.lay;
    t->host_image.assign(static_cast<const uint8_t *>(blob), static_cast<const uint8_t *>(blob) + t->desc.lay.image_bytes);
    t->spec_thread = std::thread([ctx, t] {
        cudaSetDevice(ctx->device);
        ensure_spec(ctx, t);
    });
    for (cgpu_ctx *p : ctx->peers) {
        cgpu_table *pt = nullptr;
        rc = cgpu_table_load(p, blob, len, &pt);
        if (rc != CGPU_OK) { const std::string why = g_err; cgpu_table_release(t); return fail(rc, "%s", why.c_str()); }
        t->peer_tables.push_back(pt);
    }
    *out = t;
    return CGPU_OK;
}

void cgpu_table_retain(cgpu_table *t) { if (t) t->refs.fetch_add(1); }
int cgpu_device_count(const cgpu_ctx *ctx) { return ctx ? 1 + (int)ctx->peers.size() : 0; }

void cgpu_table_release(cgpu_table *t) {
    if (!t) return;
    if (t->refs.fetch_sub(1) == 1) {
        for (cgpu_table *pt : t->peer_tables) cgpu_table_release(pt);
        t->peer_tables.clear();
        { std::lock_guard<std::mutex> g(t->join_mu); if (t->spec_thread.joinable()) t->spec_thread.join(); }
        cudaSetDevice(t->ctx->device);
        cudaDeviceSynchronize();
        cudaFree(t->d_image);
        if (t->d_uc_image) cudaFree(t->d_uc_image);
        if (t->d_uc_meta) cudaFree(t->d_uc_meta);
        if (t->spec_lib) cudaLibraryUnload(t->spec_lib);
        delete t;
    }
}

int cgpu_table_compile_check(const void *blob, size_t len, size_t *cubin_bytes) {
    if (!blob || !cubin_bytes) return fail(CGPU_ERR_INVALID, "cgpu_table_compile_check: null argument");
    *cubin_bytes = 0;
    cb::TableLayout lay;
    uint32_t meta[CB_META_WORDS];
    uint64_t sec_len[cbhost::kMaxSec] = {0};
    int rc = invalid(cbhost::parse_blob(blob, len, &lay, meta, sec_len));
    if (rc != CGPU_OK) return rc;
    const cbuc::Image uc = cbuc::build(static_cast<const uint8_t *>(blob), lay.off, sec_len, meta, lay);
    std::vector<char> cubin;
    std::string why;
    uint32_t n_strpred = 0;
    const SpecForm form = spec_compile(static_cast<const uint8_t *>(blob), lay, meta, uc, &cubin, &why, &n_strpred);
    if (form == SPEC_NONE) {
        g_err = why;
        return why.rfind("NVRTC compile failed", 0) == 0 ? CGPU_ERR_CUDA : CGPU_OK;
    }
    g_err = form == SPEC_UC ? "unique-condition form" : "block-shape form";
    *cubin_bytes = cubin.size();
    return CGPU_OK;
}

int cgpu_table_wait_ready(cgpu_table *t, int *specialised) {
    if (!t) return fail(CGPU_ERR_INVALID, "cgpu_table_wait_ready: null table");
    for (cgpu_table *pt : t->peer_tables) cgpu_table_wait_ready(pt, nullptr);
    { std::lock_guard<std::mutex> g(t->join_mu); if (t->spec_thread.joinable()) t->spec_thread.join(); }
    if (specialised) *specialised = t->spec_state.load(std::memory_order_acquire) == 1 ? 1 : 0;
    g_err = t->spec_note;
    return CGPU_OK;
}

int cgpu_table_info(const cgpu_table *t, uint32_t *meta_out, uint32_t n_words) {
    if (!t || !meta_out) return fail(CGPU_ERR_INVALID, "cgpu_table_info: null argument");
    if (n_words > CB_META_WORDS) n_words = CB_META_WORDS;
    memcpy(meta_out, t->meta, n_words * 4);
    return CGPU_OK;
}

uint64_t cgpu_launch_count(const cgpu_ctx *ctx) { return ctx ? ctx->launches.load() : 0; }

int cgpu_deferred_count(cgpu_ctx *ctx, uint64_t *total) {
    if (!ctx || !total) return fail(CGPU_ERR_INVALID, "cgpu_deferred_count: null argument");
    *total = 0;
    struct RestoreDevice {
        int dev = -1;
        RestoreDevice() { if (cudaGetDevice(&dev) != cudaSuccess) { cudaGetLastError(); dev = -1; } }
        ~RestoreDevice() { if (dev >= 0) cudaSetDevice(dev); }
    } restore;
    std::vector<cgpu_ctx *> all{ctx};
    all.insert(all.end(), ctx->peers.begin(), ctx->peers.end());
    for (cgpu_ctx *c : all) {
        CUDA_TRY(cudaSetDevice(c->device));
        CUDA_TRY(cudaDeviceSynchronize());
        std::lock_guard<std::mutex> g(c->defer_mu);
        for (auto &kv : c->defer_lanes) {
            if (!kv.second.cells) continue;
            uint32_t w[16];
            CUDA_TRY(cudaMemcpy(w, kv.second.cells, sizeof(w), cudaMemcpyDeviceToHost));
            for (int q = 0; q < 4; q++) *total += w[4 * q + 3];
        }
    }
    return CGPU_OK;
}

int cgpu_last_kernel_config(const cgpu_ctx *ctx, uint32_t *grid, uint32_t *block, uint32_t *smem_bytes) {
    if (!ctx) return fail(CGPU_ERR_INVALID, "null ctx");
    if (grid) *grid = ctx->last_grid;
    if (block) *block = ctx->last_grid ? kThreads : 0;
    if (smem_bytes) *smem_bytes = ctx->last_plan.smem | (uint32_t)ctx->last_plan.lean << 31;
    return CGPU_OK;
}

int cgpu_last_cluster_config(const cgpu_ctx *ctx, uint32_t *clustered, uint32_t *window, uint32_t *buckets) {
    if (!ctx) return fail(CGPU_ERR_INVALID, "null ctx");
    const LaunchPlan &p = ctx->last_plan;
    if (clustered) *clustered = (uint32_t)p.cluster | (uint32_t)p.col_tiles << 1 | (uint32_t)p.spec << 2 | (uint32_t)p.uc << 3;
    if (window) *window = ctx->last_window;
    if (buckets) *buckets = ctx->last_buckets;
    return CGPU_OK;
}

int cgpu_profile(cgpu_ctx *ctx, int enable, double *kernel_ms_sum, uint64_t *n_launches) {
    if (!ctx) return fail(CGPU_ERR_INVALID, "null ctx");
    CUDA_TRY(cudaSetDevice(ctx->device));
    if (ctx->prof_pending) {
        CUDA_TRY(cudaEventSynchronize(ctx->ev1));
        float ms = 0;
        CUDA_TRY(cudaEventElapsedTime(&ms, ctx->ev0, ctx->ev1));
        ctx->prof_ms += ms; ctx->prof_n++;
        ctx->prof_pending = false;
    }
    if (kernel_ms_sum) *kernel_ms_sum = ctx->prof_ms;
    if (n_launches) *n_launches = ctx->prof_n;
    ctx->prof_ms = 0; ctx->prof_n = 0;
    if (enable && !ctx->ev0) { CUDA_TRY(cudaEventCreate(&ctx->ev0)); CUDA_TRY(cudaEventCreate(&ctx->ev1)); }
    ctx->profiling = enable != 0;
    return CGPU_OK;
}

int cgpu_check_device(cgpu_ctx *ctx, const cgpu_table *t, const cgpu_batch *dev_batch, void *dev_bitmap_out, void *cuda_stream) {
    if (!ctx || !t || !dev_batch || !dev_bitmap_out) return fail(CGPU_ERR_INVALID, "cgpu_check_device: null argument");
    if (t->ctx != ctx) return fail(CGPU_ERR_INVALID, "table belongs to another context");
    cb::BatchView bv;
    int rc = invalid(cbhost::make_batch_view(t->desc.lay, dev_batch, 0, dev_batch->n_requests, &bv));
    if (rc != CGPU_OK) return rc;
    CUDA_TRY(cudaSetDevice(ctx->device));
    cudaStream_t s = static_cast<cudaStream_t>(cuda_stream);
    return launch_check(ctx, t, plan_launch(*ctx, *t, bv), bv, static_cast<uint8_t *>(dev_bitmap_out), nullptr, ctx->d_status, s);
}

int cgpu_peer_alloc(cgpu_ctx *ctx, size_t bytes, void **dev_ptr, void *ipc_handle_out) {
    if (!ctx || !dev_ptr || !ipc_handle_out || bytes == 0) return fail(CGPU_ERR_INVALID, "cgpu_peer_alloc: bad argument");
    CUDA_TRY(cudaSetDevice(ctx->device));
    void *p = nullptr;
    CUDA_TRY(cudaMalloc(&p, bytes));
    CUDA_TRY(cudaMemset(p, 0, bytes));
    cudaIpcMemHandle_t h;
    cudaError_t e = cudaIpcGetMemHandle(&h, p);
    if (e != cudaSuccess) { cudaFree(p); return fail(CGPU_ERR_CUDA, "cudaIpcGetMemHandle failed: %s", cudaGetErrorString(e)); }
    static_assert(sizeof(h) == CGPU_IPC_HANDLE_BYTES, "IPC handle size");
    memcpy(ipc_handle_out, &h, sizeof(h));
    *dev_ptr = p;
    return CGPU_OK;
}

int cgpu_peer_open(cgpu_ctx *ctx, const void *ipc_handle, void **dev_ptr) {
    if (!ctx || !ipc_handle || !dev_ptr) return fail(CGPU_ERR_INVALID, "cgpu_peer_open: null argument");
    CUDA_TRY(cudaSetDevice(ctx->device));
    cudaIpcMemHandle_t h;
    memcpy(&h, ipc_handle, sizeof(h));
    CUDA_TRY(cudaIpcOpenMemHandle(dev_ptr, h, cudaIpcMemLazyEnablePeerAccess));
    return CGPU_OK;
}

int cgpu_peer_close(cgpu_ctx *ctx, void *dev_ptr) {
    if (!ctx || !dev_ptr) return fail(CGPU_ERR_INVALID, "cgpu_peer_close: null argument");
    CUDA_TRY(cudaSetDevice(ctx->device));
    CUDA_TRY(cudaIpcCloseMemHandle(dev_ptr));
    return CGPU_OK;
}

int cgpu_peer_free(cgpu_ctx *ctx, void *dev_ptr) {
    if (!ctx || !dev_ptr) return fail(CGPU_ERR_INVALID, "cgpu_peer_free: null argument");
    CUDA_TRY(cudaSetDevice(ctx->device));
    CUDA_TRY(cudaFree(dev_ptr));
    return CGPU_OK;
}

int cgpu_peer_read(cgpu_ctx *ctx, const void *dev_ptr, void *host_out, size_t bytes) {
    if (!ctx || !dev_ptr || !host_out) return fail(CGPU_ERR_INVALID, "cgpu_peer_read: null argument");
    CUDA_TRY(cudaSetDevice(ctx->device));
    CUDA_TRY(cudaMemcpy(host_out, dev_ptr, bytes, cudaMemcpyDeviceToHost));
    return CGPU_OK;
}

int cgpu_check_device_gather(cgpu_ctx *ctx, const cgpu_table *t, const cgpu_batch *dev_batch, const cgpu_gather *g, void *cuda_stream) {
    if (!ctx || !t || !dev_batch || !g || !g->gather_bufs || !g->flags) return fail(CGPU_ERR_INVALID, "cgpu_check_device_gather: null argument");
    if (t->ctx != ctx) return fail(CGPU_ERR_INVALID, "table belongs to another context");
    if (g->n_ranks == 0 || g->n_ranks > cb::CB_MAX_GATHER || g->my_rank >= g->n_ranks || g->step == 0)
        return fail(CGPU_ERR_INVALID, "cgpu_check_device_gather: 1..%d ranks, my_rank < n_ranks, step > 0", cb::CB_MAX_GATHER);
    cb::BatchView bv;
    int rc = invalid(cbhost::make_batch_view(t->desc.lay, dev_batch, 0, dev_batch->n_requests, &bv));
    if (rc != CGPU_OK) return rc;
    if (bv.kbytes > 8) return fail(CGPU_ERR_UNSUPPORTED, "fused gather supports up to 64 actions per request");
    if ((uint64_t)bv.count * bv.kbytes > g->slice_bytes) return fail(CGPU_ERR_INVALID, "gather slice too small");
    SignalParams sp{};
    for (uint32_t r = 0; r < g->n_ranks; r++) {
        if (!g->gather_bufs[r] || !g->flags[r]) return fail(CGPU_ERR_INVALID, "gather buffer / flags of rank %u missing", r);
        bv.outs[r] = static_cast<uint8_t *>(g->gather_bufs[r]) + (uint64_t)g->my_rank * g->slice_bytes;
        sp.flags[r] = g->flags[r];
    }
    sp.n_ranks = g->n_ranks; sp.my_rank = g->my_rank; sp.step = g->step;
    sp.wait_flags = g->wait_flags ? g->wait_flags : g->flags[g->my_rank]; sp.wait_step = g->wait_step;
    CUDA_TRY(cudaSetDevice(ctx->device));
    cudaStream_t s = static_cast<cudaStream_t>(cuda_stream);
    const uint64_t slice_used = (uint64_t)bv.count * bv.kbytes;
    const char *ce = getenv("CERBOS_B200_CE_GATHER");
    const bool ce_gather = g->n_ranks > 1 && (ce ? ce[0] == '1' : slice_used >= (1u << 20));
    if (ce_gather) {
        std::lock_guard<std::mutex> lk(ctx->copy_mu);
        if (!ctx->copy_stream) CUDA_TRY(cudaStreamCreateWithFlags(&ctx->copy_stream, cudaStreamNonBlocking));
        uint8_t *own = bv.outs[g->my_rank];
        cgpu_ctx::SliceUse *use = nullptr;
        for (auto &u : ctx->slice_uses) if (u.ptr == own) use = &u;
        if (use) CUDA_TRY(cudaStreamWaitEvent(s, use->done, 0));
        else {
            cgpu_ctx::SliceUse nu{own, nullptr, nullptr, 0};
            CUDA_TRY(cudaEventCreateWithFlags(&nu.done, cudaEventDisableTiming));
            ctx->slice_uses.push_back(nu);
            use = &ctx->slice_uses.back();
        }
        if (use->stage_bytes < slice_used) {
            if (use->stage) { CUDA_TRY(cudaStreamSynchronize(ctx->copy_stream)); CUDA_TRY(cudaFree(use->stage)); use->stage = nullptr; use->stage_bytes = 0; }
            CUDA_TRY(cudaMalloc(reinterpret_cast<void **>(&use->stage), slice_used));
            use->stage_bytes = slice_used;
        }
        rc = launch_check(ctx, t, plan_launch(*ctx, *t, bv), bv, use->stage, nullptr, ctx->d_status, s);
        if (rc != CGPU_OK) return rc;
        cudaEvent_t &ev = ctx->copy_ev[ctx->copy_seq++ & 15];
        if (!ev) CUDA_TRY(cudaEventCreateWithFlags(&ev, cudaEventDisableTiming));
        CUDA_TRY(cudaEventRecord(ev, s));
        CUDA_TRY(cudaStreamWaitEvent(ctx->copy_stream, ev, 0));
        for (uint32_t q = 0; q < g->n_ranks; q++) {
            const uint32_t r = (g->my_rank + 1 + q) % g->n_ranks;
            CUDA_TRY(cudaMemcpyAsync(bv.outs[r], use->stage, slice_used, cudaMemcpyDeviceToDevice, ctx->copy_stream));
        }
        SignalParams sp2 = sp;
        sp2.wait_step = 0;
        void *args[] = {&sp2};
        CUDA_TRY(cudaLaunchKernel((const void *)gather_signal, dim3(1), dim3(32), args, 0, ctx->copy_stream));
        CUDA_TRY(cudaEventRecord(use->done, ctx->copy_stream));
        ctx->launches.fetch_add(1, std::memory_order_relaxed);
        if (g->wait_step) {
            gather_wait<<<1, 32, 0, s>>>(sp.wait_flags, g->n_ranks, g->wait_step);
            CUDA_TRY(cudaGetLastError());
            ctx->launches.fetch_add(1, std::memory_order_relaxed);
        }
        return CGPU_OK;
    }
    bv.n_out = g->n_ranks;
    for (uint32_t r = 0; r < g->n_ranks; r++) bv.sig_flags[r] = g->flags[r];
    bv.sig_rank = g->my_rank; bv.sig_step = g->step;
    bv.wait_flags = sp.wait_flags; bv.wait_step = g->wait_step;
    const LaunchPlan plan = plan_launch(*ctx, *t, bv);
    rc = launch_check(ctx, t, plan, bv, bv.outs[g->my_rank], nullptr, ctx->d_status, s);
    if (rc != CGPU_OK) return rc;
    if (!plan.lean) {
        void *args[] = {&sp};
        CUDA_TRY(launch_serialised((const void *)gather_signal, 1, 32, 0, s, args));
        ctx->launches.fetch_add(1, std::memory_order_relaxed);
    }
    return CGPU_OK;
}

int cgpu_gather_wait(cgpu_ctx *ctx, const uint32_t *local_flags, uint32_t n_ranks, uint32_t step, void *cuda_stream) {
    if (!ctx || !local_flags || n_ranks == 0 || n_ranks > cb::CB_MAX_GATHER) return fail(CGPU_ERR_INVALID, "cgpu_gather_wait: bad argument");
    CUDA_TRY(cudaSetDevice(ctx->device));
    gather_wait<<<1, 32, 0, static_cast<cudaStream_t>(cuda_stream)>>>(local_flags, n_ranks, step);
    CUDA_TRY(cudaGetLastError());
    ctx->launches.fetch_add(1, std::memory_order_relaxed);
    return CGPU_OK;
}

int cgpu_sync(cgpu_ctx *ctx, void *cuda_stream) {
    if (!ctx) return fail(CGPU_ERR_INVALID, "null ctx");
    CUDA_TRY(cudaSetDevice(ctx->device));
    cudaStream_t s = static_cast<cudaStream_t>(cuda_stream);
    uint32_t st = 0;
    CUDA_TRY(cudaMemcpyAsync(&st, ctx->d_status, 4, cudaMemcpyDeviceToHost, s));
    CUDA_TRY(cudaStreamSynchronize(s));
    if (st) {
        CUDA_TRY(cudaMemsetAsync(ctx->d_status, 0, 4, s));
        CUDA_TRY(cudaStreamSynchronize(s));
        return fail(CGPU_ERR_UNSUPPORTED, "a request produced a run-time value the device cannot represent exactly (e.g. timestamp outside 1678..2262, string->double, concatenation)");
    }
    return CGPU_OK;
}

struct HostBlock { void *p = nullptr; size_t cap = 0; bool is_malloc = false; };
struct HostBlockPool {
    std::mutex mu;
    std::vector<HostBlock> free_list;
    HostBlock take(size_t bytes, bool allow_malloc) {
        size_t cap = 1u << 20;
        while (cap < bytes && cap < (64u << 20)) cap <<= 1;
        if (cap < bytes) cap = (bytes + (64u << 20) - 1) / (64u << 20) * (64u << 20);
        {
            std::lock_guard<std::mutex> g(mu);
            size_t best = free_list.size();
            for (size_t i = 0; i < free_list.size(); i++)
                if (free_list[i].cap >= bytes && (allow_malloc || !free_list[i].is_malloc) && (best == free_list.size() || free_list[i].cap < free_list[best].cap)) best = i;
            if (best != free_list.size()) { HostBlock b = free_list[best]; free_list.erase(free_list.begin() + (long)best); return b; }
        }
        HostBlock b;
        if (cudaHostAlloc(&b.p, cap, cudaHostAllocDefault) == cudaSuccess) { b.cap = cap; return b; }
        cudaGetLastError();
        b.p = nullptr;
        if (allow_malloc) { b.p = malloc(cap); b.cap = b.p ? cap : 0; b.is_malloc = b.p != nullptr; }
        return b;
    }
    void give(HostBlock b) {
        if (!b.p) return;
        {
            std::lock_guard<std::mutex> g(mu);
            if (free_list.size() < 8) { free_list.push_back(b); return; }
        }
        if (b.is_malloc) free(b.p); else cudaFreeHost(b.p);
    }
};
static HostBlockPool &host_pool() { static HostBlockPool *p = new HostBlockPool(); return *p; }

int cgpu_encoder_create(const void *blob, size_t len, const char *default_version, const char *default_scope, int lenient_scope_search, cgpu_encoder **out) {
    if (!blob || !out) return fail(CGPU_ERR_INVALID, "cgpu_encoder_create: null argument");
    *out = nullptr;
    cgpu_encoder *e = new (std::nothrow) cgpu_encoder();
    if (!e) return fail(CGPU_ERR_INVALID, "out of memory");
    cbenc::Conf conf;
    if (default_version && default_version[0]) conf.default_version = default_version;
    if (default_scope) conf.default_scope = default_scope;
    conf.lenient = lenient_scope_search != 0;
    if (!e->enc.init(blob, len, conf)) { const std::string why = e->enc.error; delete e; return fail(CGPU_ERR_INVALID, "%s", why.c_str()); }
    *out = e;
    return CGPU_OK;
}
void cgpu_encoder_destroy(cgpu_encoder *e) { delete e; }

int cgpu_encode(const cgpu_encoder *e, const void *const *inputs, const size_t *input_bytes, uint64_t n, cgpu_encoded **out) {
    if (!e || !inputs || !input_bytes || !out || n == 0) return fail(CGPU_ERR_INVALID, "cgpu_encode: null argument or empty batch");
    *out = nullptr;
    cgpu_encoded *r = new (std::nothrow) cgpu_encoded();
    if (!r) return fail(CGPU_ERR_INVALID, "out of memory");
    std::string enc_err;
    unsigned threads = std::thread::hardware_concurrency();
    if (threads > 32) threads = 32;
    if (const char *et = getenv("CERBOS_B200_ENCODE_THREADS")) { const long v = strtol(et, nullptr, 10); if (v >= 1 && v <= 256) threads = (unsigned)v; }
    if (!e->enc.encode(inputs, input_bytes, n, &r->cols, threads ? threads : 1, &enc_err)) { delete r; return fail(CGPU_ERR_INVALID, "cgpu_encode: %s", enc_err.c_str()); }
// ... 406 lines not shown
```

Before: 89.71 billion.

## Precompute per-string records to resolve startsWith/endsWith pairs in registers

The per-batch pre-pass now builds a 16- or 32-byte record per string: predicate bits, length, first 8 bytes and last 8 bytes. The generated condition code loads these records once per slot. startsWith/endsWith between two slot strings is then decided with mask compares, and only suffixes longer than 8 bytes fall back to the full byte comparison. This is meant to avoid repeated heap byte walks in the decision kernel, at the cost of a larger pre-pass buffer and more registers per thread.

```diff
diff --git a/cerbos_b200/csrc/cb_core.h b/cerbos_b200/csrc/cb_core.h
--- a/cerbos_b200/csrc/cb_core.h
+++ b/cerbos_b200/csrc/cb_core.h
@@ -98,6 +98,7 @@
     uint32_t *sig_flags[CB_MAX_GATHER];
     const uint32_t *wait_flags;
     uint32_t sig_rank, sig_step, wait_step;
+    const U4 *strrec;
     const uint32_t *strpred;
     const U4 *uc_rows_pk;
     uint32_t n_bstr;
@@ -112,6 +113,7 @@
     b.n_out = 0;
     for (int i = 0; i < CB_MAX_GATHER; i++) { b.outs[i] = nullptr; b.sig_flags[i] = nullptr; }
     b.wait_flags = nullptr; b.sig_rank = 0; b.sig_step = 0; b.wait_step = 0;
+    b.strrec = nullptr;
     b.strpred = nullptr;
     b.uc_rows_pk = nullptr;
     b.rcp = 1;
@@ -3624,13 +3626,60 @@
     if (A.st == 2 || B.st == 2) { slow = true; return TRI_E; }
     return (subset ? m == (1u << A.len) - 1u : m != 0u) ? TRI_T : TRI_F;
 }
-CB_HD int strpred_tri(const BatchView &b, uint64_t x, uint32_t p) {
+struct StrRec { uint32_t pred, len; uint64_t head, tail; };
+CB_HD StrRec str_rec_make(const TableView t, const BatchView &b, uint32_t id, uint32_t pred) {
+    const StrRef s = str_ref(t, b, ((uint64_t)(CB_V64_BOX_BASE | CB_V64_STRING) << 48) | id);
+    const uint32_t n = s.len < 8 ? s.len : 8;
+    StrRec r;
+    r.pred = pred; r.len = s.len; r.head = 0; r.tail = 0;
+    for (uint32_t i = 0; i < n; i++) {
+        r.head |= (uint64_t)ldg(s.p + i) << (8 * i);
+        r.tail |= (uint64_t)ldg(s.p + (s.len - n) + i) << (8 * i);
+    }
+    return r;
+}
+CB_HD void str_rec_store(U4 *out, const StrRec &r, uint32_t halves) {
+    out[0] = U4{r.pred, r.len, (uint32_t)r.head, (uint32_t)(r.head >> 32)};
+    if (halves == 2) out[1] = U4{(uint32_t)r.tail, (uint32_t)(r.tail >> 32), 0u, 0u};
+}
+CB_HD StrRec str_rec(const TableView t, const BatchView &b, uint64_t x, uint32_t halves) {
+    StrRec r;
+    r.pred = 0; r.len = 0; r.head = 0; r.tail = 0;
+    if (v64_tag(x) != CB_V64_STRING) return r;
+    const uint32_t id = (uint32_t)x;
+#if defined(__CUDA_ARCH__)
+    const U4 *p = b.strrec + (size_t)id * halves;
+    const U4 h = ldg(p);
+    r.pred = h.x; r.len = h.y; r.head = h.z | (uint64_t)h.w << 32;
+    if (halves == 2) { const U4 h2 = ldg(p + 1); r.tail = h2.x | (uint64_t)h2.y << 32; }
+#else
+    r = str_rec_make(t, b, id, b.strpred ? b.strpred[id] : 0u);
+#endif
+    return r;
+}
+CB_HD int strpred_tri(uint64_t x, uint32_t pred, uint32_t p) {
 #ifdef CB_UC_STUB_STRPRED
     return (int)((x >> p) & 1u);
 #endif
     if (v64_bad(x)) return TRI_E;
     if (v64_tag(x) != CB_V64_STRING) return TRI_E;
-    return (int)((ldg(b.strpred + (uint32_t)(x & 0xFFFFFFFFu)) >> p) & 1u);
+    return (int)((pred >> p) & 1u);
+}
+CB_HD bool str_rec_match(uint32_t op, const StrRec &x, const StrRec &y) {
+    const uint32_t k = y.len, n = x.len < 8 ? x.len : 8;
+    const uint64_t w = op == CB_TERM_STARTS ? x.head : x.tail >> ((8 * (n - k)) & 63);
+    const uint64_t m = k >= 8 ? ~0ull : (1ull << (8 * k)) - 1ull;
+    return x.len >= k && ((w ^ y.head) & m) == 0;
+}
+CB_HD uint32_t str_pair_match(uint32_t op, const StrRec &x, const StrRec &y) { return y.len > 8 ? 2u : (uint32_t)str_rec_match(op, x, y); }
+CB_HD_NOINLINE int str_tri_long(const TableView t, const BatchView &b, uint32_t op, uint64_t x, uint64_t y) { return str_tri(t, b, op, x, y); }
+CB_HD int str_tri(const TableView t, const BatchView &b, uint32_t op, uint64_t x, uint64_t y, uint32_t m) {
+#ifdef CB_UC_STUB_STR_PAIRS
+    return (int)((x ^ y) & 1u);
+#endif
+    if (v64_tag(x) != CB_V64_STRING || v64_tag(y) != CB_V64_STRING) return TRI_E;
+    if (m & 2u) return str_tri_long(t, b, op, x, y);
+    return (int)(m & 1u);
 }
 CB_HD bool typed_str(uint64_t x) { return (uint32_t)(x >> 32) == (uint32_t)(CB_V64_BOX_BASE | CB_V64_STRING) << 16; }
 CB_HD bool typed_num(uint64_t x) { const double d = u2d(x); return v64_tag(x) == 0 && d == d; }
@@ -3651,11 +3700,18 @@
 CB_HD uint32_t typed_id(uint64_t key) { return (uint32_t)key; }
 CB_HD uint64_t typed_box(uint32_t id) { return ((uint64_t)(CB_V64_BOX_BASE | CB_V64_STRING) << 48) | id; }
 CB_HD bool typed_ord(uint32_t ci, double dx, double dy) { return ci == 2 ? dx < dy : ci == 3 ? dx <= dy : ci == 4 ? dx > dy : dx >= dy; }
-CB_HD bool typed_strpred(const BatchView &b, uint32_t id, uint32_t p) {
+CB_HD bool typed_strpred(uint32_t id, uint32_t pred, uint32_t p) {
 #ifdef CB_UC_STUB_STRPRED
     return ((id >> p) & 1u) != 0;
 #endif
-    return ((ldg(b.strpred + id) >> p) & 1u) != 0;
+    return ((pred >> p) & 1u) != 0;
+}
+CB_HD bool typed_str_pair(const TableView t, const BatchView &b, uint32_t op, uint32_t x, uint32_t y, uint32_t m) {
+#ifdef CB_UC_STUB_STR_PAIRS
+    return ((x ^ y) & 1u) != 0;
+#endif
+    if (m & 2u) return str_tri_long(t, b, op, typed_box(x), typed_box(y)) == TRI_T;
+    return (m & 1u) != 0;
 }
 template <typename Cols>
 CB_HD ListKey list_elem_key(const TableView t, const BatchView &b, const Cols &cols, uint32_t v, const ListRegs &L, uint32_t i) {
diff --git a/cerbos_b200/csrc/cb_specialize.h b/cerbos_b200/csrc/cb_specialize.h
--- a/cerbos_b200/csrc/cb_specialize.h
+++ b/cerbos_b200/csrc/cb_specialize.h
@@ -402,6 +402,7 @@
 struct UcSource {
     std::string src;
     uint32_t n_strpred = 0;
+    uint32_t str_rec = 0;
     uint32_t n_atoms = 0;
 };
 inline UcSource generate_uc(const uint8_t *uc_image, const uint32_t *off, uint32_t uc_conds_off, uint32_t n_uconds, uint32_t n_slots, uint32_t n_consts = 0,
@@ -465,6 +466,7 @@
                 pred_of[q] = (uint32_t)pred_terms.size();
                 pred_terms.push_back(q);
             }
+            if ((op == CB_TERM_STARTS || op == CB_TERM_ENDS) && xk == CB_OPK_SLOT && yk == CB_OPK_SLOT && w[1] < ns && w[2] < ns) form[q] = 'R';
             break;
         }
     }
@@ -485,6 +487,24 @@
             mask_of[q] = k;
         }
     auto sl = [](uint32_t v) { return "cols.slot(" + std::to_string(v) + "u)"; };
+    uint32_t str_halves = n_pred_bits ? 1u : 0u;
+    std::vector<bool> rec_slot(ns, false);
+    for (uint32_t q = 0; q < terms.size(); q++) {
+        const uint32_t *w = terms[q].data();
+        if (form[q] == 'P') rec_slot[w[1]] = true;
+        if (form[q] == 'R') {
+            rec_slot[w[1]] = rec_slot[w[2]] = true;
+            if (str_halves < 2u) str_halves = (w[0] & 0xFF) == CB_TERM_ENDS ? 2u : 1u;
+        }
+    }
+    auto rec = [&](uint32_t v) { return rec_slot[v] ? "cols.q" + std::to_string(v) : "str_rec(t, b, " + sl(v) + ", kStrRec)"; };
+    auto pair_match = [&](uint32_t q, bool in_load) {
+        const uint32_t *w = terms[q].data();
+        if (in_load != (rec_slot[w[1]] && rec_slot[w[2]])) return std::string();
+        const std::string r1 = in_load ? "r.q" + std::to_string(w[1]) : rec(w[1]), r2 = in_load ? "r.q" + std::to_string(w[2]) : rec(w[2]);
+        return "str_pair_match(" + std::to_string(w[0] & 0xFF) + "u, " + r1 + ", " + r2 + ")";
+    };
+    auto match_of = [&](uint32_t q) { const std::string e = pair_match(q, false); return e.empty() ? "cols.m" + std::to_string(q) : e; };
     auto operand = [&](uint32_t kind, uint32_t v, uint32_t aux) -> std::string {
         if (kind == CB_OPK_CONST) return hex64(consts[v]);
         if (kind == CB_OPK_PID) return "(((uint64_t)(CB_V64_BOX_BASE | CB_V64_STRING) << 48) | pid)";
@@ -525,7 +545,8 @@
         const uint32_t op = w[0] & 0xFF, flags = (w[0] >> 8) & 0xFF, xk = (w[0] >> 16) & 0xFF, yk = w[0] >> 24;
         const bool kinds = op <= CB_TERM_SUBSET;
         const std::string x = kinds ? operand(xk, w[1], w[3] & 0xFFFFu) : "", y = kinds && op != CB_TERM_HAS ? operand(yk, w[2], w[3] >> 16) : "";
-        if (form[q] == 'P') return "strpred_tri(b, " + sl(w[1]) + ", " + std::to_string(pred_of[q]) + "u)";
+        if (form[q] == 'P') return "strpred_tri(" + sl(w[1]) + ", " + rec(w[1]) + ".pred, " + std::to_string(pred_of[q]) + "u)";
+        if (form[q] == 'R') return "str_tri(t, b, " + std::to_string(op) + "u, " + sl(w[1]) + ", " + sl(w[2]) + ", " + match_of(q) + ")";
         if (form[q] == 'L') {
             if (op == CB_TERM_IN_CS || op == CB_TERM_IN_SS || op == CB_TERM_IN) {
                 const std::string v = std::to_string(w[2]);
@@ -555,6 +576,7 @@
     for (uint32_t v = 0; v < ns; v++) n_reg += slot_used[v] || slot_list[v];
     if (n_reg > kMaxRegSlots)
         for (uint32_t v = 0; v < ns; v++) if (!slot_list[v]) slot_used[v] = false;
+    for (uint32_t v = 0; v < ns; v++) rec_slot[v] = rec_slot[v] && (slot_used[v] || slot_list[v]);
     std::vector<char> ty(ns, 0);
     std::vector<uint32_t> list_need(ns, 0);
     bool typed = n_reg > 0 && n_reg <= kMaxRegSlots;
@@ -641,7 +663,9 @@
     auto typed_term = [&](uint32_t q) -> std::string {
         const uint32_t *w = terms[q].data();
         const uint32_t op = w[0] & 0xFF, flags = (w[0] >> 8) & 0xFF, xk = (w[0] >> 16) & 0xFF, yk = w[0] >> 24, ci = flags & CB_TERM_CI_MASK;
-        if (form[q] == 'P') return "typed_strpred(b, typed_id(cols.k" + std::to_string(w[1]) + "), " + std::to_string(pred_of[q]) + "u)";
+        if (form[q] == 'P') return "typed_strpred(typed_id(cols.k" + std::to_string(w[1]) + "), " + rec(w[1]) + ".pred, " + std::to_string(pred_of[q]) + "u)";
+        if (form[q] == 'R')
+            return "typed_str_pair(t, b, " + std::to_string(op) + "u, typed_id(cols.k" + std::to_string(w[1]) + "), typed_id(cols.k" + std::to_string(w[2]) + "), " + match_of(q) + ")";
         if (form[q] == 'L') {
             if (op == CB_TERM_IN_CS || op == CB_TERM_IN_SS || op == CB_TERM_IN) {
                 if (probe_of[q] == CB_NONE32) return "";
@@ -721,11 +745,16 @@
     }
     for (uint32_t v = 0; v < ns; v++)
         if (slot_list[v]) s += "    ListRegs l" + std::to_string(v) + ";\n";
+    for (uint32_t v = 0; v < ns; v++)
+        if (rec_slot[v]) s += "    StrRec q" + std::to_string(v) + ";   // the string's record (str_rec)\n";
+    for (uint32_t q = 0; q < terms.size(); q++)
+        if (form[q] == 'R' && !pair_match(q, true).empty()) s += "    uint32_t m" + std::to_string(q) + ";   // str_pair_match() of term " + std::to_string(q) + "\n";
     s += "    CB_HD uint64_t slot(uint32_t v) const {\n        switch (v) {\n";
     for (uint32_t v = 0; v < ns && !typed; v++)
         if (reg(v)) s += "        case " + std::to_string(v) + "u: return s" + std::to_string(v) + ";\n";
     s += "        default: return v < " + std::to_string(ns) + "u ? g.slot(v) : (uint64_t)(CB_V64_BOX_BASE | CB_V64_ERROR) << 48;\n        }\n    }\n};\n";
     s += "struct SpecConds {\n    static constexpr uint32_t n_strpred = " + std::to_string(n_pred_bits) + "u;\n";
+    s += "    static constexpr uint32_t kStrRec = " + std::to_string(str_halves) + "u;   // U4 per string record (BatchView::strrec), 0: no pre-pass\n";
     s += std::string("    static constexpr int kForm = ") + (n_uconds <= 31 ? "CB_UC_FORM_MASK32" : n_uconds <= 63 ? "CB_UC_FORM_MASK64" : "CB_UC_FORM_INDEX") + ";   // how the rows name their conditions\n";
     s += "    static constexpr uint32_t kScopeRows = " + std::to_string(scope_rows) + "u;   // rows the walk visits per scope (cb::uc_walk)\n";
     s += "    static constexpr uint32_t kDenyRows = " + std::to_string(deny_rows) + "u, kAllowRows = " + std::to_string(allow_rows) +
@@ -734,6 +763,10 @@
     s += "    template <typename Cols>\n    CB_HD SpecRegs load(const TableView t, const BatchView &b, const Cols &c) const {\n        SpecRegs r;\n        r.g.b = c.b; r.g.n = c.n;\n";
     for (uint32_t v = 0; v < ns; v++)
         if (reg(v)) s += "        r.s" + std::to_string(v) + " = c.slot(" + std::to_string(v) + "u);\n";
+    for (uint32_t v = 0; v < ns; v++)
+        if (rec_slot[v]) s += "        r.q" + std::to_string(v) + " = str_rec(t, b, r.s" + std::to_string(v) + ", kStrRec);\n";
+    for (uint32_t q = 0; q < terms.size(); q++)
+        if (form[q] == 'R' && !pair_match(q, true).empty()) s += "        r.m" + std::to_string(q) + " = " + pair_match(q, true) + ";\n";
     if (typed) {
         std::string guard;
         for (uint32_t v = 0; v < ns; v++) {
@@ -803,7 +836,7 @@
             const std::string A = std::to_string(a);
             if (atom_pred[a] >= 0) {
                 const std::string P = std::to_string(atom_pred[a]), V = sl(atoms.only_slot[a]);
-                atom_src += "        bool a" + A + ";\n        {\n            const uint64_t x = " + V + ";\n            const uint32_t w = v64_tag(x) == CB_V64_STRING && !v64_bad(x) ? ldg(b.strpred + (uint32_t)(x & 0xFFFFFFFFu)) >> " + P + " : 2u;\n";
+                atom_src += "        bool a" + A + ";\n        {\n            const uint64_t x = " + V + ";\n            const uint32_t w = v64_tag(x) == CB_V64_STRING && !v64_bad(x) ? str_rec(t, b, x, kStrRec).pred >> " + P + " : 2u;\n";
                 atom_src += "            if (w & 2u) { c.scr_used = 0; a" + A + " = uc_atom_" + A + "(c, cols); } else a" + A + " = (w & 1u) != 0;\n        }\n";
             } else {
                 atom_src += "        c.scr_used = 0; const bool a" + A + " = uc_atom_" + A + "(c, cols);\n";
@@ -856,6 +889,7 @@
     s += "        return val;\n    }\n};\n}  // namespace cb\n";
     out.src = s;
     out.n_strpred = n_pred_bits;
+    out.str_rec = str_halves;
     out.n_atoms = (uint32_t)atoms.src.size();
     return out;
 }
diff --git a/cerbos_b200/csrc/cerbos_b200.cu b/cerbos_b200/csrc/cerbos_b200.cu
--- a/cerbos_b200/csrc/cerbos_b200.cu
+++ b/cerbos_b200/csrc/cerbos_b200.cu
@@ -350,7 +350,7 @@
     bool col_tiles = false;
     bool cluster = false;
     bool spec = false;
-    bool strpred = false;
+    uint32_t str_rec = 0;
     bool merge_rows = false;
     bool serialise = false;
 };
@@ -393,7 +393,7 @@
         uint32_t *cells = nullptr;
         struct Bufs {
             LaneBuf<uint32_t> list;
-            LaneBuf<uint32_t> strpred;
+            LaneBuf<cb::U4> strrec;
             LaneBuf<cb::U4> pk;
         } q[4];
     };
@@ -450,7 +450,7 @@
     cudaLibrary_t spec_lib = nullptr;
     cudaKernel_t spec_tiles = nullptr, spec_direct = nullptr, spec_uc = nullptr, spec_uc_global = nullptr, spec_strpred = nullptr;
     cudaKernel_t spec_uc_meta = nullptr, spec_uc_meta_global = nullptr;
-    uint32_t spec_n_strpred = 0;
+    uint32_t spec_str_rec = 0;
     std::string spec_note;
     uint64_t sec_len[cbhost::kMaxSec]{};
     std::vector<cgpu_table *> peer_tables;
@@ -542,10 +542,11 @@
     "    cbk::check_uc_body<cb::SpecConds, cb::GlobalCols, false>(td, bv, nullptr, effects, nullptr, nullptr, cbk::UcMeta{action_meta, req_meta, side});\n"
     "}\n";
 const char kSpecUcStrpred[] =
-    "\nextern \"C\" __global__ void __launch_bounds__(256) cb_spec_strpred(const __grid_constant__ cbk::TableDesc td, const __grid_constant__ cb::BatchView bv, uint32_t *out, const uint32_t n) {\n"
+    "\nextern \"C\" __global__ void __launch_bounds__(256) cb_spec_strpred(const __grid_constant__ cbk::TableDesc td, const __grid_constant__ cb::BatchView bv, cb::U4 *out, const uint32_t n) {\n"
     "    const uint32_t id = blockIdx.x * 256u + threadIdx.x;\n"
     "    cb::TableView tv; tv.base = td.base; tv.L = &td.lay;\n"
-    "    if (id < n) out[id] = cb::SpecConds().strpred(tv, bv, id);\n"
+    "    constexpr uint32_t K = cb::SpecConds::kStrRec;\n"
+    "    if (K && id < n) cb::str_rec_store(out + (size_t)id * K, cb::str_rec_make(tv, bv, id, cb::SpecConds().strpred(tv, bv, id)), K);\n"
     "}\n";
 
 uint64_t fnv1a(const void *p, size_t n, uint64_t h = 1469598103934665603ull) {
@@ -593,9 +594,9 @@
 uint64_t uc_smem_bytes(const cbuc::Image &uc, uint64_t n_pk) { return (((uint64_t)uc.lay.image_bytes + 127) & ~127ull) + 16 * n_pk; }
 bool uc_stageable(const cbuc::Image &uc, uint64_t n_pk = 1) { return uc_smem_bytes(uc, n_pk) <= kUcMaxSmem; }
 
-SpecForm spec_generate(const uint8_t *image, const cb::TableLayout &lay, const uint32_t *meta, const cbuc::Image &uc, std::string *gen, std::string *why, uint32_t *n_strpred,
+SpecForm spec_generate(const uint8_t *image, const cb::TableLayout &lay, const uint32_t *meta, const cbuc::Image &uc, std::string *gen, std::string *why, uint32_t *str_rec,
                        uint32_t *n_atoms = nullptr) {
-    *n_strpred = 0;
+    *str_rec = 0;
     if (n_atoms) *n_atoms = 0;
     if (!cbhost::lean_table(lay, meta)) {
         *why = "table is not lean-eligible (principal / role policies, parent roles or resource globs): general kernel only";
@@ -608,7 +609,7 @@
     if (uc.ok) {
         cbspec::UcSource us = cbspec::generate_uc(uc.bytes.data(), uc.lay.off, uc.lay.uc_conds_off, uc.n_uconds, lay.n_slots, meta[CB_META_N_CONSTS]);
         *gen = us.src;
-        *n_strpred = us.n_strpred;
+        *str_rec = us.str_rec;
         if (n_atoms) *n_atoms = us.n_atoms;
         if (!gen->empty()) return SPEC_UC;
     }
@@ -617,10 +618,10 @@
     return SPEC_NONE;
 }
 
-SpecForm spec_compile(const uint8_t *image, const cb::TableLayout &lay, const uint32_t *meta, const cbuc::Image &uc, std::vector<char> *cubin, std::string *why, uint32_t *n_strpred) {
+SpecForm spec_compile(const uint8_t *image, const cb::TableLayout &lay, const uint32_t *meta, const cbuc::Image &uc, std::vector<char> *cubin, std::string *why, uint32_t *str_rec) {
     std::string gen;
     uint32_t n_atoms = 0;
-    const SpecForm form = spec_generate(image, lay, meta, uc, &gen, why, n_strpred, &n_atoms);
+    const SpecForm form = spec_generate(image, lay, meta, uc, &gen, why, str_rec, &n_atoms);
     if (form == SPEC_NONE) return SPEC_NONE;
     std::string src = kSpecPrelude;
     if (n_atoms) src += "#define CB_SPEC_PROGRAMS 1\n";
@@ -689,7 +690,7 @@
     if (ctx->force_no_jit) return give_up("disabled (CERBOS_B200_NO_JIT)");
     std::vector<char> cubin;
     std::string why;
-    const SpecForm form = spec_compile(t->host_image.data(), t->desc.lay, t->meta, t->uc, &cubin, &why, &t->spec_n_strpred);
+    const SpecForm form = spec_compile(t->host_image.data(), t->desc.lay, t->meta, t->uc, &cubin, &why, &t->spec_str_rec);
     if (form == SPEC_NONE) return give_up(why);
     if (cudaLibraryLoadData(&t->spec_lib, cubin.data(), nullptr, nullptr, 0, nullptr, nullptr, 0) != cudaSuccess) { cudaGetLastError(); return give_up("cudaLibraryLoadData failed"); }
     bool got = form == SPEC_UC ? (!uc_stageable(t->uc) || (cudaLibraryGetKernel(&t->spec_uc, t->spec_lib, "cb_spec_uc") == cudaSuccess &&
@@ -748,7 +749,7 @@
     return CGPU_OK;
 }
 
-int acquire_defer(cgpu_ctx *ctx, cudaStream_t stream, uint64_t count, uint32_t **list, uint32_t **cell, size_t n_strpred, uint32_t **strpred,
+int acquire_defer(cgpu_ctx *ctx, cudaStream_t stream, uint64_t count, uint32_t **list, uint32_t **cell, size_t n_strrec, cb::U4 **strrec,
                   size_t n_pk, cb::U4 **pk) {
     std::lock_guard<std::mutex> g(ctx->defer_mu);
     cgpu_ctx::DeferLane &ln = ctx->defer_lanes[stream];
@@ -759,11 +760,11 @@
     const uint32_t q = ln.seq++ & 3;
     cgpu_ctx::DeferLane::Bufs &b = ln.q[q];
     CUDA_TRY(b.list.fit(count, 1024, stream));
-    if (n_strpred) CUDA_TRY(b.strpred.fit(n_strpred, 4096, stream));
+    if (n_strrec) CUDA_TRY(b.strrec.fit(n_strrec, 4096, stream));
     if (n_pk) CUDA_TRY(b.pk.fit(n_pk, 4096, stream));
     *list = b.list.ptr;
     *cell = ln.cells + 4 * q;
-    *strpred = n_strpred ? b.strpred.ptr : nullptr;
+    *strrec = n_strrec ? b.strrec.ptr : nullptr;
     *pk = n_pk ? b.pk.ptr : nullptr;
     return CGPU_OK;
 }
@@ -797,7 +798,7 @@
     p.smem = p.uc ? (p.uc_staged ? (uint32_t)uc_smem_bytes(t.uc, n_pk) : 0) : p.col_tiles ? tiles_smem : p.stage ? lay.image_bytes : 0;
     p.last_arg = p.col_tiles ? lay.n_slots : p.stage ? 1u : 0u;
     p.serialise = p.spec && !p.uc && !ctx.profiling;
-    p.strpred = p.uc && p.spec && t.spec_n_strpred;
+    p.str_rec = p.uc && p.spec ? t.spec_str_rec : 0;
     p.merge_rows = p.uc && !p.uc_staged && n_pk <= (1u << 19);
     return p;
 }
@@ -882,11 +883,11 @@
     uint32_t last_arg = plan.last_arg;
     uint32_t *defer = nullptr;
     if (plan.lean) {
-        uint32_t *cell = nullptr, *strpred = nullptr;
-        cb::U4 *pk = nullptr;
+        uint32_t *cell = nullptr;
+        cb::U4 *strrec = nullptr, *pk = nullptr;
         const uint32_t n_str = lay.nT + bv.n_bstr;
         const uint64_t n_pk = (uint64_t)bv.n_asets * t->uc.lay.uc_n_rows;
-        int rc = acquire_defer(ctx, stream, bv.count, &defer, &cell, plan.strpred ? (size_t)n_str + 1 : 0, &strpred, plan.merge_rows ? (size_t)n_pk : 0, &pk);
+        int rc = acquire_defer(ctx, stream, bv.count, &defer, &cell, (size_t)plan.str_rec * (n_str + 1), &strrec, plan.merge_rows ? (size_t)n_pk : 0, &pk);
         if (rc != CGPU_OK) return rc;
         if (plan.merge_rows) {
             uc_merge_rows<<<(unsigned)((n_pk + kThreads - 1) / kThreads), kThreads, 0, stream>>>(t->uc_desc, bvv, pk, (uint32_t)n_pk);
@@ -897,14 +898,14 @@
         bvv.defer_count = cell;
         bvv.tile_counter = plan.col_tiles ? cell + 2 : nullptr;
         bvv.defer_list = defer;
-        if (plan.strpred && n_str) {
+        if (plan.str_rec && n_str) {
             TableDesc ptd = t->uc_desc;
             uint32_t n_arg = n_str;
-            void *pargs[] = {&ptd, &bvv, &strpred, &n_arg};
+            void *pargs[] = {&ptd, &bvv, &strrec, &n_arg};
             CUDA_TRY(cudaLaunchKernel((const void *)t->spec_strpred, dim3((n_str + 255) / 256), dim3(256), pargs, 0, stream));
             ctx->launches.fetch_add(1, std::memory_order_relaxed);
         }
-        bvv.strpred = strpred;
+        bvv.strrec = strrec;
     }
     const void *fn = kernel_fn(*t, plan.kernel);
     void *args[] = {&td, &bvv, &d_bitmap, &d_effects, &d_status, &last_arg};
@@ -1044,7 +1045,7 @@
     }
     if (ctx->d_status) cudaFree(ctx->d_status);
     for (auto &kv : ctx->defer_lanes) {
-        for (auto &b : kv.second.q) { cudaFree(b.list.ptr); cudaFree(b.strpred.ptr); cudaFree(b.pk.ptr); }
+        for (auto &b : kv.second.q) { cudaFree(b.list.ptr); cudaFree(b.strrec.ptr); cudaFree(b.pk.ptr); }
         if (kv.second.cells) cudaFree(kv.second.cells);
     }
     if (ctx->copy_stream) cudaStreamDestroy(ctx->copy_stream);
@@ -1131,8 +1132,8 @@
     const cbuc::Image uc = cbuc::build(static_cast<const uint8_t *>(blob), lay.off, sec_len, meta, lay);
     std::vector<char> cubin;
     std::string why;
-    uint32_t n_strpred = 0;
-    const SpecForm form = spec_compile(static_cast<const uint8_t *>(blob), lay, meta, uc, &cubin, &why, &n_strpred);
+    uint32_t str_rec = 0;
+    const SpecForm form = spec_compile(static_cast<const uint8_t *>(blob), lay, meta, uc, &cubin, &why, &str_rec);
     if (form == SPEC_NONE) {
         g_err = why;
         return why.rfind("NVRTC compile failed", 0) == 0 ? CGPU_ERR_CUDA : CGPU_OK;
```

Result: faster. 91.29 billion, median of 6 (+1.8%).
